# wangheda/youtube-8m

Measured on AMD Instinct MI355X. Metric: training videos/sec, higher is better.
Workload: dtype f32; 1 GPU; BASELINE configs[3]: LstmModel (2 x BasicLSTMCell(1024), dynamic_rnn over F=300) on raw uint8 [B,300,1152] frames + MoeModel head (2 mixtures, V=4716), fp32 training step (fwd+bwd+clip+Adam); per_gpu_batch=128, global_batch=128, frames=300, parallelism=dp1, params=113902808

## Files before the change

### include/yt8m_hip.h

```cpp
#ifndef YT8M_HIP_H
#define YT8M_HIP_H
#include <stdint.h>

#ifdef __cplusplus
extern "C" {
#endif

typedef void* yt8m_stream_t;

enum yt8m_status { YT8M_OK = 0, YT8M_E_BADARG = -1, YT8M_E_SHAPE = -2, YT8M_E_HIP = -3, YT8M_E_RCCL = -4 };
enum yt8m_label_dtype { YT8M_LABEL_U8 = 0, YT8M_LABEL_F32 = 1 };

int yt8m_abi_version(void);
const char* yt8m_last_error(void);
const char* yt8m_built_arch(void);

int yt8m_prof_enable(int on);
int yt8m_prof_reset(void);
int yt8m_prof_get(int family, int64_t* launches, double* total_ms);
int yt8m_prof_get_flops(int family, double* flops);
int yt8m_prof_get_bytes(int family, double* bytes);

int yt8m_probe_mfma_f32(int iters, int blocks, float* sink, yt8m_stream_t stream);
int yt8m_probe_mfma_bf16(int iters, int blocks, int random_operands, float* sink, yt8m_stream_t stream);
// ... 293 lines not shown
int64_t yt8m_wimg_count(void);
int yt8m_wimg_watch(const void* lo, const void* hi, int on);
int yt8m_wimg_note_demand(const float* src, int64_t R, int64_t C, int64_t ld, int trans, int planes, float scale);
int64_t yt8m_wimg_demands(yt8m_wimg_demand* out, int64_t max);
int64_t yt8m_wimg_demand_generation(const void* lo, const void* hi);
typedef struct yt8m_wimg_spec {
  void* plain;
  void* trans;
  int64_t row0, rows;
  float scale;
  int32_t planes;
} yt8m_wimg_spec;
typedef struct yt8m_wimg_job {
  int64_t offset;
  int64_t R, C;
  int32_t tensor;
  int32_t nspec;
  int64_t tile_base;
  yt8m_wimg_spec spec[4];
} yt8m_wimg_job;
int64_t yt8m_wimg_jobs_layout(yt8m_wimg_job* jobs_host, int64_t njobs);
int yt8m_adam_tiles(float* w, float* m, float* v, const float* g, const yt8m_wimg_job* jobs, int64_t njobs, int64_t tile0,
                    int64_t ntiles, const float* l2, float gscale, const float* norms, float clip, float lr_t, float beta1,
                    float beta2, float eps, int do_adam, yt8m_stream_t stream);
int yt8m_adam_multi_ex(float* w, float* m, float* v, const float* g, const int32_t* chunks, int64_t nchunks,
                       const float* l2, float gscale, const float* norms, float clip, float lr_t, float beta1, float beta2,
                       float eps, const uint8_t* skip_tensor, yt8m_stream_t stream);

int yt8m_lstm_gates_fwd(float* z, const float* c_prev, const float* h_prev, float* c_new, float* h_new,
                        float* out, const int32_t* num_frames, int32_t t, int64_t B, int64_t H,
                        float forget_bias, yt8m_stream_t stream);
int yt8m_lstm_gates_bwd(const float* gates, const float* c_prev, const float* c_new, const float* dh,
                        const float* dc, const float* dout, float* dz, float* dc_prev, float* dh_prev,
                        const int32_t* num_frames, int32_t t, int64_t B, int64_t H, yt8m_stream_t stream);

int yt8m_lstm_layer_fwd(float* z, const float* Wh, int64_t ldw, float* cs, float* hs, float* out,
                        const int32_t* num_frames, int64_t F, int64_t B, int64_t H, float forget_bias,
                        void* gemm_workspace, int64_t gemm_workspace_bytes, yt8m_stream_t stream);
int yt8m_lstm_layer_bwd(const float* gates, const float* Wh, int64_t ldw, const float* cs, const float* dout,
                        const float* dc_final, const float* dh_final, float* dz, float* work,
                        const int32_t* num_frames, int64_t F, int64_t B, int64_t H,
                        void* gemm_workspace, int64_t gemm_workspace_bytes, yt8m_stream_t stream);

int yt8m_lstm_persist_supported(int64_t B, int64_t H);
int64_t yt8m_lstm_persist_workspace_bytes(int64_t B, int64_t H);
int64_t yt8m_lstm_persist_workspace_bytes_steps(int64_t B, int64_t H, int64_t T);
int yt8m_lstm_persist_fwd_on_bf16_pipe(int64_t B, int64_t H);
int yt8m_lstm_persist_set_cus(int fwd_cus, int bwd_cus);
int yt8m_lstm_persist_get_cus(int* fwd_cus, int* bwd_cus);
int yt8m_lstm_persist_set_tape_prefetch(int mode);
int yt8m_lstm_persist_tape_prefetch_launches(int64_t* with_prefetch, int64_t* without_prefetch);
int yt8m_lstm_persist_reserve_cus(int cus, int* previous);
int yt8m_lstm_persist_status(const void* workspace, yt8m_stream_t stream);
int yt8m_lstm_persist_debug_fault(void* workspace, yt8m_stream_t stream);
int yt8m_lstm_persist_placement_stats(int64_t* launches, int64_t* workgroups, int64_t* off_xcd, int reset);
int yt8m_lstm_persist_fwd(float* z, const float* Wh, int64_t ldw, float* cs, float* hs, float* out,
                          const int32_t* num_frames, int64_t t0, int64_t T, int64_t B, int64_t H, float forget_bias,
                          void* workspace, int64_t workspace_bytes, yt8m_stream_t stream);
int yt8m_lstm_persist_fwd_bf16(float* z, const float* Wh, int64_t ldw, float* cs, float* hs, float* out,
                               const int32_t* num_frames, int64_t t0, int64_t T, int64_t B, int64_t H, float forget_bias,
                               void* workspace, int64_t workspace_bytes, yt8m_stream_t stream);
int yt8m_lstm_persist_fwd_h2(float* z, const float* Wh, int64_t ldw, float* cs, float* hs, float* out, const int32_t* num_frames,
                             int64_t t0, int64_t T, int64_t B, int64_t H, float forget_bias, const void* wh_absmax, void* workspace,
                             int64_t workspace_bytes, yt8m_stream_t stream);
int yt8m_lstm_persist_bwd_supported(int64_t B, int64_t H);
int yt8m_lstm_persist_bwd(const float* gates, const float* Wh, int64_t ldw, const float* cs, const float* dout, float* dz,
                          float* work, int phase, float* dbias_rows, const int32_t* num_frames, int64_t t0, int64_t T,
                          int64_t B, int64_t H, void* workspace, int64_t workspace_bytes, yt8m_stream_t stream);
int yt8m_lstm_persist_bwd_bf16(const float* gates, const float* Wh, int64_t ldw, const float* cs, const float* dout, float* dz,
                               float* work, int phase, float* dbias_rows, const int32_t* num_frames, int64_t t0, int64_t T,
                               int64_t B, int64_t H, void* workspace, int64_t workspace_bytes, yt8m_stream_t stream);
int yt8m_lstm_persist_bwd_h2(const float* gates, const float* Wh, int64_t ldw, const float* cs, const float* dout, float* dz,
                             float* work, int phase, float* dbias_rows, const int32_t* num_frames, int64_t t0, int64_t T,
                             int64_t B, int64_t H, const void* wh_absmax, void* workspace, int64_t workspace_bytes, yt8m_stream_t stream);
int yt8m_lstm_persist_bwd_on_f16_pipe(int64_t B, int64_t H);
int yt8m_gru_persist_supported(int64_t B, int64_t H);
int64_t yt8m_gru_persist_workspace_bytes(int64_t B, int64_t H, int64_t T);
int yt8m_gru_persist_fwd(float* zg, float* zc, const float* Wg_h, int64_t ldg, const float* Wc_h, int64_t ldc, float* hs, float* rh,
                         float* out, const int32_t* num_frames, int64_t t0, int64_t T, int64_t B, int64_t H, void* workspace,
                         int64_t workspace_bytes, yt8m_stream_t stream);
int yt8m_lstm_persist_bwd_ex(const float* gates, const float* Wh, int64_t ldw, const float* cs, const float* dout, float* dz, float* work,
                             int phase, const int32_t* num_frames, int64_t t0, int64_t T, int64_t B, int64_t H, const void* wh_absmax,
                             void* rowmax, void* partmax, void* workspace, int64_t workspace_bytes, yt8m_stream_t stream);
typedef struct yt8m_persist_bwd_images {
  void* plain;
  void* trans;
  void* trans_scaled;
  const float* rowscale;
  float* colpart;
  float* colpart_scaled;
} yt8m_persist_bwd_images;
int yt8m_lstm_persist_bwd_images_rows(int64_t B, int64_t H);
int yt8m_lstm_persist_bwd_images(const float* gates, const float* Wh, int64_t ldw, const float* cs, const float* dout, float* dz,
                                 float* work, int phase, const int32_t* num_frames, int64_t t0, int64_t T, int64_t B, int64_t H,
                                 void* workspace, int64_t workspace_bytes, const yt8m_persist_bwd_images* images, yt8m_stream_t stream);

typedef struct yt8m_lstm_stack_desc {
  int64_t B, F, D, H;
  int32_t L;
  int32_t input_u8;
  float forget_bias;
  int32_t fwd_chunks;
  int32_t bwd_chunks;
  int32_t need_dx;
  float input_keep_prob;
  int32_t reserved0;
  uint64_t dropout_seed[8];
} yt8m_lstm_stack_desc;
int yt8m_lstm_stack_supported(const yt8m_lstm_stack_desc* desc);
int64_t yt8m_lstm_stack_tape_bytes(const yt8m_lstm_stack_desc* desc);
int64_t yt8m_lstm_stack_scratch_bytes(const yt8m_lstm_stack_desc* desc);
int yt8m_lstm_stack_partition(const yt8m_lstm_stack_desc* desc, int* fwd_chunks, int* bwd_chunks);
int yt8m_lstm_stack_streams(int L, yt8m_stream_t* layer_streams, yt8m_stream_t* wgrad_stream);
int yt8m_lstm_stack_fwd(const yt8m_lstm_stack_desc* desc, const void* x, const int32_t* num_frames, const float* const* W,
                        const float* const* b, void* tape, int64_t tape_bytes, void* scratch, int64_t scratch_bytes,
                        yt8m_stream_t stream);
int yt8m_lstm_stack_view(const yt8m_lstm_stack_desc* desc, void* tape, int layer, int which, float** out);
int yt8m_lstm_stack_bwd(const yt8m_lstm_stack_desc* desc, const void* x, const int32_t* num_frames, const float* const* W, void* tape,
                        int64_t tape_bytes, void* scratch, int64_t scratch_bytes, const float* dout_top,
                        const float* const* dc_final, const float* const* dh_final, float* const* dW, float* const* db,
                        const float* beta_W, const float* beta_b, float* dx, yt8m_stream_t stream);
int yt8m_lstm_stack_status(const yt8m_lstm_stack_desc* desc, void* scratch, yt8m_stream_t stream);
int yt8m_lstm_stack_layer_done_wait(int layer, yt8m_stream_t stream);
int yt8m_lstm_stack_use_streams(int set, int* previous);
typedef void (*yt8m_stream_hook)(void* user, yt8m_stream_t stream);
int yt8m_lstm_stack_set_prep_hook(yt8m_stream_hook hook, void* user);
typedef struct yt8m_opt_ranges {
  float* w;
  float* m;
  float* v;
  const float* g;
  const int32_t* chunks;
  const int32_t* tensor_chunk_start;
  const int32_t* tensor_chunk_start_host;
  const float* l2;
  float* partial;
  float* norms;
  const uint8_t* skip_tensor;
  const yt8m_wimg_job* jobs;
  const int32_t* job_tensor_host;
  const int64_t* job_tile_base_host;
  int32_t njobs;
  int32_t nranges;
  int32_t range_lo[8], range_hi[8];
  float gscale, clip, lr_t, beta1, beta2, eps;
  yt8m_stream_t after_stream;
} yt8m_opt_ranges;
int yt8m_optimizer_ranges(const yt8m_opt_ranges* opt, yt8m_stream_t stream);
int yt8m_lstm_stack_set_early_optimizer(const yt8m_opt_ranges* opt);

int64_t yt8m_lstm_packed_floats(int64_t B, int64_t H);
int yt8m_lstm_pack(const float* Wh, int64_t ldw, int64_t H, float* Wp, float* Wq, yt8m_stream_t stream);
int yt8m_lstm_steps_fwd(float* z, const float* Wh, int64_t ldw, const float* Wp, float* cs, float* hs, float* out,
                        const int32_t* num_frames, int64_t t0, int64_t T, int64_t B, int64_t H, float forget_bias,
                        void* gemm_workspace, int64_t gemm_workspace_bytes, yt8m_stream_t stream);
int yt8m_lstm_steps_bwd(const float* gates, const float* Wh, int64_t ldw, const float* Wq, const float* cs,
                        const float* dout, float* dz, float* work, int phase, const int32_t* num_frames, int64_t t0,
                        int64_t T, int64_t B, int64_t H, void* gemm_workspace, int64_t gemm_workspace_bytes,
                        yt8m_stream_t stream);

int yt8m_graph_cache_stats(int64_t* hits, int64_t* captures, int64_t* fallbacks, int64_t* entries);
int yt8m_graph_cache_clear(void);

int yt8m_reverse_sequence_u8(const uint8_t* x, const int32_t* num_frames, uint8_t* y, int64_t B, int64_t F, int64_t D,
                             yt8m_stream_t stream);
int yt8m_reverse_sequence_f32_tm(const float* x, int64_t ldx, const int32_t* num_frames, float* y, int64_t ldy, int64_t y_col0,
// ... 166 lines not shown
```

### youtube-8m_amd/_lib.py

```python
import ctypes
import os

_HERE = os.path.dirname(os.path.abspath(__file__))
LIB_PATH = os.environ.get("YT8M_LIB", os.path.join(_HERE, "libyt8m_hip.so"))

c_void_p, c_int, c_int64, c_float, c_double = ctypes.c_void_p, ctypes.c_int, ctypes.c_int64, ctypes.c_float, ctypes.c_double
P = c_void_p

class GemmProblem(ctypes.Structure):
    _fields_ = [("M", c_int64), ("N", c_int64), ("K", c_int64), ("A", c_void_p), ("lda", c_int64), ("B", c_void_p),
                ("ldb", c_int64), ("C", c_void_p), ("ldc", c_int64), ("bias", c_void_p), ("beta", c_float)]


STREAM_HOOK = ctypes.CFUNCTYPE(None, ctypes.c_void_p, ctypes.c_void_p)


class PersistBwdImages(ctypes.Structure):
    _fields_ = [("plain", ctypes.c_void_p), ("trans", ctypes.c_void_p), ("trans_scaled", ctypes.c_void_p), ("rowscale", ctypes.c_void_p),
                ("colpart", ctypes.c_void_p), ("colpart_scaled", ctypes.c_void_p)]


class LstmStackDesc(ctypes.Structure):
    _fields_ = [("B", c_int64), ("F", c_int64), ("D", c_int64), ("H", c_int64), ("L", ctypes.c_int32), ("input_u8", ctypes.c_int32),
                ("forget_bias", c_float), ("fwd_chunks", ctypes.c_int32), ("bwd_chunks", ctypes.c_int32), ("need_dx", ctypes.c_int32),
# ... 114 lines not shown
    "yt8m_skinny_fwd_u8": (c_int, [P, c_int64, P, c_int64, P, P, P, P, c_int64, c_int64, c_int64, c_int64, c_float, P]),
    "yt8m_skinny_dw_u8": (c_int, [P, c_int64, P, c_int64, P, P, c_int64, c_int64, c_int64, c_int64, c_float, P, c_int64, P]),
    "yt8m_attn_pool_fwd_u8": (c_int, [P, P, P, P, c_int64, c_int64, c_int64, c_int64, P]),
    "yt8m_attn_pool_dw_u8": (c_int, [P, P, P, P, P, c_int64, c_int64, c_int64, c_int64, P]),
    "yt8m_attn_pool_supported": (c_int, [c_int64, c_int64, c_int64, c_int64]),
    "yt8m_attn_pool_fwd": (c_int, [P, P, P, c_int64, c_int64, c_int64, c_int64, P]),
    "yt8m_attn_pool_bwd": (c_int, [P, P, P, P, P, c_int64, c_int64, c_int64, c_int64, P]),
    "yt8m_gru_layer_fwd": (c_int, [P, P, P, c_int64, P, c_int64, P, P, P, P, c_int64, c_int64, c_int64, P, c_int64, P]),
    "yt8m_gru_layer_bwd": (c_int, [P, P, P, c_int64, P, c_int64, P, P, P, P, P, P, P, c_int64, c_int64, c_int64, P, c_int64, P]),
    "yt8m_lnlstm_layer_fwd": (c_int, [P, P, c_int64, P, P, P, P, P, P, P, c_int64, c_int64, c_int64, c_float, c_float,
                                      ctypes.c_uint64, P, c_int64, P]),
    "yt8m_lnlstm_layer_bwd": (c_int, [P, P, c_int64, P, P, P, P, P, P, P, P, P, P, P, P, c_int64, c_int64, c_int64, c_float,
                                      c_float, ctypes.c_uint64, P, c_int64, P]),
    "yt8m_gate_lstm_supported": (c_int, [c_int64, c_int64]),
    "yt8m_gate_lstm_layer_fwd": (c_int, [P, P, c_int64, P, c_int64, P, P, P, P, P, c_int64, c_int64, c_int64, P, c_int64, P]),
    "yt8m_gate_lstm_layer_bwd": (c_int, [P, P, c_int64, P, c_int64, P, P, P, P, P, P, P, P, P, c_int64, c_int64, c_int64, P, c_int64,
                                         P]),
    "yt8m_glu_lstm_supported": (c_int, [c_int64, c_int64, c_int64]),
    "yt8m_glu_lstm_layer_fwd": (c_int, [P, P, c_int64, P, c_int64, P, c_int64] + [P] * 12 + [c_int64] * 4 + [P, c_int64, P]),
    "yt8m_glu_lstm_layer_bwd": (c_int, [P, P, c_int64, P, c_int64, P, c_int64] + [P] * 14 + [c_int64] + [P] * 4 + [c_int64] * 4 +
                                        [P, c_int64, P]),
    "yt8m_dropout_f32": (c_int, [P, P, c_int64, c_float, ctypes.c_uint64, c_int64, P]),
    "yt8m_add_noise_f32": (c_int, [P, P, c_int64, c_float, ctypes.c_uint64, c_int64, P]),
    "yt8m_moe_mix_bwd_bf16_partial_rows": (c_int64, [c_int64]),
    "yt8m_moe_mix_bwd_bf16": (c_int, [P, P, P, P, c_int, c_int64, c_int64, c_int, c_float, c_float, P, P, c_int64, P, c_int64,
                                      P, c_int64, P, c_int64, P, P]),
    "yt8m_moe_mix_bwd_bf16_images": (c_int, [P, P, P, P, c_int, c_int64, c_int64, c_int, c_float, c_float, P, P, c_int64, P, c_int64,
                                      P, c_int64, P, c_int64, P, P]),
    "yt8m_moe_mix_bwd_bf16_images_z16": (c_int, [P, P, P, P, c_int, c_int64, c_int64, c_int, c_float, c_float, P, P, c_int64, P, c_int64,
                                      P, c_int64, P, c_int64, P, P]),
    "yt8m_moe_mix_fwd_bf16z": (c_int, [P, P, P, c_int64, c_int64, c_int, P]),
    "yt8m_act_fwd_f32": (c_int, [c_int, P, P, c_int64, P]),
    "yt8m_act_bwd_f32": (c_int, [c_int, P, P, P, c_int64, P]),
    "yt8m_chain_link_fwd": (c_int, [c_int, P, P, P, c_int64, c_int64, c_float, c_float, ctypes.c_uint64, c_int64, P]),
    "yt8m_chain_link_bwd": (c_int, [c_int, P, P, P, P, P, c_int64, c_int64, c_float, P]),
    "yt8m_memory_link_fwd": (c_int, [c_int, P, P, c_int, P, P, c_int64, c_float, P]),
    "yt8m_memory_link_bwd": (c_int, [c_int, P, c_int, P, P, P, P, c_int64, c_float, P]),
    "yt8m_frame_pyramid_u8": (c_int, [P, P, c_int64, c_int64, c_int64, c_int, c_int, P, P, P, c_float, P]),
    "yt8m_frame_pyramid_supported": (c_int, [c_int64, c_int, P, c_int]),
    "yt8m_colsum_workspace_bytes": (c_int64, [c_int64, c_int64]),
    "yt8m_colsum_f32": (c_int, [P, c_int64, c_int64, c_int64, P, c_float, P, c_int64, P]),
    "yt8m_rank1_add_rows_f32": (c_int, [P, c_int64, c_int64, c_int64, P, c_float, P]),
    "yt8m_colsum_weighted_f32": (c_int, [P, c_int64, c_int64, c_int64, P, P, c_float, P, P, c_int64, P]),
    "yt8m_xent_workspace_bytes": (c_int64, [c_int64, c_int64]),
    "yt8m_xent_fwd_bwd": (c_int, [P, P, c_int, P, P, P, c_int64, c_int64, c_float, c_float, P, P]),
    "yt8m_xent_bwd": (c_int, [P, P, c_int, P, P, P, c_int64, c_int64, c_float, c_float, P]),
    "yt8m_batch_agreement_workspace_bytes": (c_int64, [c_int64, c_int64]),
    "yt8m_batch_agreement_fwd": (c_int, [P, P, c_int, P, P, c_int64, c_int64, c_float, c_float, c_float, P, P]),
    "yt8m_batch_agreement_bwd": (c_int, [P, P, c_int, P, P, P, c_int64, c_int64, c_float, c_float, P]),
    "yt8m_topk_batch_agreement_fwd": (c_int, [P, P, c_int, P, P, c_int64, c_int64, c_float, c_float, P, P]),
    "yt8m_topk_batch_agreement_bwd": (c_int, [P, P, c_int, P, P, P, c_int64, c_int64, c_float, c_float, c_float, P]),
    "yt8m_pointwise_loss_workspace_bytes": (c_int64, [c_int64, c_int64]),
    "yt8m_pointwise_loss_fwd_bwd": (c_int, [c_int, P, P, c_int, P, P, c_int64, c_int64, c_float, c_float, c_float, c_float, P, P]),
    "yt8m_pointwise_loss_bwd": (c_int, [c_int, P, P, c_int, P, P, c_int64, c_int64, c_float, c_float, c_float, c_float, P]),
    "yt8m_sqnorm_multi": (c_int, [P, P, P, c_int64, P, c_float, P, P, c_int64, c_int64, P, c_int64, P]),
    "yt8m_adam_multi": (c_int, [P, P, P, P, P, c_int64, P, c_float, P, c_float, c_float, c_float, c_float, c_float, P]),
    "yt8m_lstm_gates_fwd": (c_int, [P, P, P, P, P, P, P, ctypes.c_int32, c_int64, c_int64, c_float, P]),
    "yt8m_lstm_gates_bwd": (c_int, [P, P, P, P, P, P, P, P, P, P, ctypes.c_int32, c_int64, c_int64, P]),
    "yt8m_lstm_layer_fwd": (c_int, [P, P, c_int64, P, P, P, P, c_int64, c_int64, c_int64, c_float, P, c_int64, P]),
    "yt8m_graph_cache_stats": (c_int, [ctypes.POINTER(c_int64), ctypes.POINTER(c_int64), ctypes.POINTER(c_int64),
                                       ctypes.POINTER(c_int64)]),
    "yt8m_graph_cache_clear": (c_int, []),
    "yt8m_lstm_persist_supported": (c_int, [c_int64, c_int64]),
    "yt8m_lstm_persist_workspace_bytes": (c_int64, [c_int64, c_int64]),
    "yt8m_lstm_persist_workspace_bytes_steps": (c_int64, [c_int64, c_int64, c_int64]),
    "yt8m_lstm_persist_placement_stats": (c_int, [ctypes.POINTER(c_int64), ctypes.POINTER(c_int64), ctypes.POINTER(c_int64), c_int]),
    "yt8m_lstm_persist_fwd_on_bf16_pipe": (c_int, [c_int64, c_int64]),
    "yt8m_lstm_persist_set_cus": (c_int, [c_int, c_int]),
    "yt8m_lstm_persist_get_cus": (c_int, [ctypes.POINTER(c_int), ctypes.POINTER(c_int)]),
    "yt8m_lstm_persist_set_tape_prefetch": (c_int, [c_int]),
    "yt8m_lstm_persist_tape_prefetch_launches": (c_int, [ctypes.POINTER(c_int64), ctypes.POINTER(c_int64)]),
    "yt8m_lstm_persist_status": (c_int, [P, P]),
    "yt8m_lstm_persist_reserve_cus": (c_int, [c_int, ctypes.POINTER(c_int)]),
    "yt8m_lstm_persist_debug_fault": (c_int, [P, P]),
    "yt8m_lstm_persist_fwd": (c_int, [P, P, c_int64, P, P, P, P, c_int64, c_int64, c_int64, c_int64, c_float, P, c_int64, P]),
    "yt8m_lstm_persist_fwd_bf16": (c_int, [P, P, c_int64, P, P, P, P, c_int64, c_int64, c_int64, c_int64, c_float, P, c_int64, P]),
    "yt8m_lstm_persist_bwd_supported": (c_int, [c_int64, c_int64]),
    "yt8m_lstm_persist_bwd": (c_int, [P, P, c_int64, P, P, P, P, c_int, P, P, c_int64, c_int64, c_int64, c_int64, P, c_int64, P]),
    "yt8m_lstm_persist_bwd_bf16": (c_int, [P, P, c_int64, P, P, P, P, c_int, P, P, c_int64, c_int64, c_int64, c_int64, P, c_int64, P]),
    "yt8m_lstm_persist_fwd_h2": (c_int, [P, P, c_int64, P, P, P, P, c_int64, c_int64, c_int64, c_int64, c_float, P, P, c_int64, P]),
    "yt8m_lstm_persist_bwd_h2": (c_int, [P, P, c_int64, P, P, P, P, c_int, P, P, c_int64, c_int64, c_int64, c_int64, P, P, c_int64, P]),
    "yt8m_lstm_persist_bwd_on_f16_pipe": (c_int, [c_int64, c_int64]),
    "yt8m_lstm_persist_bwd_ex": (c_int, [P, P, c_int64, P, P, P, P, c_int, P, c_int64, c_int64, c_int64, c_int64, P, P, P, P, c_int64, P]),
    "yt8m_h2_split_rowmax": (c_int, [P, c_int64, c_int64, c_int64, P, P, P, P]),
    "yt8m_lstm_persist_bwd_images_rows": (c_int, [c_int64, c_int64]),
    "yt8m_lstm_persist_bwd_images": (c_int, [P, P, c_int64, P, P, P, P, c_int, P, c_int64, c_int64, c_int64, c_int64, P, c_int64, P, P]),
    "yt8m_lstm_packed_floats": (c_int64, [c_int64, c_int64]),
    "yt8m_lstm_pack": (c_int, [P, c_int64, c_int64, P, P, P]),
    "yt8m_lstm_steps_fwd": (c_int, [P, P, c_int64, P, P, P, P, P, c_int64, c_int64, c_int64, c_int64, c_float, P, c_int64, P]),
    "yt8m_lstm_steps_bwd": (c_int, [P, P, c_int64, P, P, P, P, P, c_int, P, c_int64, c_int64, c_int64, c_int64, P, c_int64, P]),
    "yt8m_lstm_layer_bwd": (c_int, [P, P, c_int64, P, P, P, P, P, P, P, c_int64, c_int64, c_int64, P, c_int64, P]),
    "yt8m_attn_softmax_fwd": (c_int, [P, P, P, c_int64, c_int64, c_int64, P]),
    "yt8m_attn_softmax_bwd": (c_int, [P, P, P, P, c_int64, c_int64, c_int64, P]),
    "yt8m_softmax_rows_fwd": (c_int, [P, P, P, c_int64, c_int64, c_int64, P]),
    "yt8m_softmax_rows_bwd": (c_int, [P, P, P, P, c_int64, c_int64, c_int64, P]),
    "yt8m_netvlad_supported": (c_int, [c_int64, c_int64, c_int64, c_int64]),
    "yt8m_netvlad_single_pass": (c_int, [c_int64, c_int64, c_int64, c_int64]),
    "yt8m_netvlad_set_single": (c_int, [c_int]),
    "yt8m_netvlad_workspace_bytes": (c_int64, [c_int64, c_int64, c_int64, c_int64]),
    "yt8m_netvlad_fwd_u8": (c_int, [P, P, P, P, c_int64, c_int64, c_int64, c_int64, c_int, c_float, P, P, P, P, c_int64, P]),
    "yt8m_netvlad_bwd_u8": (c_int, [P, P, P, P, P, c_int64, c_int64, c_int64, c_int64, c_int, c_float, P, c_float, P, c_float,
                                    P, c_int64, P]),
    "yt8m_vlad_finish_fwd": (c_int, [P, P, P, P, P, c_int64, c_int64, c_int64, c_int64, c_float, P]),
    "yt8m_vlad_finish_bwd": (c_int, [P, P, P, P, P, P, P, c_float, c_int64, c_int64, c_int64, c_float, P]),
    "yt8m_vlad_finish_q_supported": (c_int, [c_int64]),
    "yt8m_vlad_finish_q_fwd": (c_int, [P, P, P, P, P, P, c_int64, c_int64, c_int64, c_int64, c_float, P]),
    "yt8m_vlad_finish_q_bwd": (c_int, [P, P, P, P, P, P, P, P, c_float, c_int64, c_int64, c_int64, c_float, P]),
    "yt8m_crc32c": (ctypes.c_uint32, [P, c_int64]),
    "yt8m_crc32c_masked": (ctypes.c_uint32, [P, c_int64]),
    "yt8m_prefetch_open": (c_int, [ctypes.POINTER(ctypes.c_char_p), c_int, c_int, ctypes.POINTER(ctypes.c_char_p),
                                   ctypes.POINTER(ctypes.c_int32), c_int, c_int64, c_int64, c_int64, c_int, c_int, c_int,
                                   ctypes.POINTER(c_void_p)]),
    "yt8m_prefetch_acquire": (c_int, [P, ctypes.POINTER(c_void_p), ctypes.POINTER(c_void_p), ctypes.POINTER(c_void_p),
                                      ctypes.POINTER(c_void_p), ctypes.POINTER(c_int64), ctypes.POINTER(c_int64),
                                      ctypes.POINTER(c_int)]),
    "yt8m_prefetch_close": (c_int, [P]),
    "yt8m_tfrecord_write_predictions": (c_int, [ctypes.c_char_p, c_int64, P, c_int64, P, P, c_int64, ctypes.c_char_p]),
    "yt8m_tfrecord_open": (c_int, [ctypes.c_char_p, c_int, ctypes.POINTER(c_void_p)]),
    "yt8m_tfrecord_close": (c_int, [P]),
    "yt8m_tfrecord_read_frame_batch": (c_int, [P, ctypes.POINTER(ctypes.c_char_p), ctypes.POINTER(ctypes.c_int32), c_int, c_int64,
                                               c_int64, c_int64, P, P, P, P, c_int64, ctypes.POINTER(c_int64)]),
    "yt8m_tfrecord_read_video_batch": (c_int, [P, ctypes.POINTER(ctypes.c_char_p), ctypes.POINTER(ctypes.c_int32), c_int, c_int64,
                                               c_int64, P, P, P, c_int64, ctypes.POINTER(c_int64)]),
    "yt8m_comm_unique_id": (c_int, [P]),
    "yt8m_comm_init": (c_int, [c_int, c_int, P, ctypes.POINTER(c_void_p)]),
    "yt8m_comm_size": (c_int, [P, ctypes.POINTER(c_int), ctypes.POINTER(c_int)]),
    "yt8m_comm_allreduce_f32": (c_int, [P, P, c_int64, c_int, P]),
    "yt8m_comm_allreduce_mean": (c_int, [P, P, c_int64, P]),
    "yt8m_comm_allreduce_rsag_f32": (c_int, [P, P, c_int64, c_int, c_int, P]),
    "yt8m_comm_broadcast_f32": (c_int, [P, P, c_int64, c_int, P]),
    "yt8m_comm_destroy": (c_int, [P]),
    "yt8m_u8_proj_supported": (c_int, [c_int64]),
    "yt8m_u8_frames_to_bf16_tm": (c_int, [P, P, c_int64, c_int64, c_int64, c_float, c_int, P, c_int64, P, P, P]),
    "yt8m_split3_bf16_t": (c_int, [P, c_int64, c_int64, c_int64, c_float, P, c_int64, P]),
    "yt8m_rowscale_bias_f32": (c_int, [P, c_int64, c_int64, c_int64, P, P, c_float, P, P]),
    "yt8m_sample_frames_f32": (c_int, [P, P, c_int64, c_int64, c_int64, c_int64, c_int, ctypes.c_uint64, P, P, P]),
    "yt8m_sample_frames_u8": (c_int, [P, P, c_int64, c_int64, c_int64, c_int64, c_int, ctypes.c_uint64, P, P, P]),
    "yt8m_frame_pool_fwd": (c_int, [P, c_int64, c_int64, c_int64, c_int, P, P]),
    "yt8m_frame_pool_bwd": (c_int, [P, P, P, c_int64, c_int64, c_int64, c_int, P, P]),
    "yt8m_batchnorm_fwd": (c_int, [P, c_int64, c_int64, P, P, P, P, c_int, c_float, c_float, P, P, P, P]),
    "yt8m_batchnorm_workspace_bytes": (c_int64, [c_int64]),
    "yt8m_batchnorm_bwd": (c_int, [P, P, c_int64, c_int64, P, P, P, c_int, P, P, c_float, P, c_float, P, c_int64, P]),
    "yt8m_wimg_register": (c_int, [P, c_int64, c_int64, c_int64, c_int, c_int, c_float, P]),
    "yt8m_wimg_unregister": (c_int64, [P, P]),
    "yt8m_wimg_lookup": (c_void_p, [P, c_int64, c_int64, c_int64, c_int, c_int, c_float]),
    "yt8m_wimg_count": (c_int64, []),
    "yt8m_wimg_watch": (c_int, [P, P, c_int]),
    "yt8m_wimg_note_demand": (c_int, [P, c_int64, c_int64, c_int64, c_int, c_int, c_float]),
    "yt8m_wimg_demands": (c_int64, [ctypes.POINTER(WimgDemand), c_int64]),
    "yt8m_wimg_demand_generation": (c_int64, [P, P]),
    "yt8m_wimg_jobs_layout": (c_int64, [ctypes.POINTER(WimgJob), c_int64]),
    "yt8m_adam_tiles": (c_int, [P, P, P, P, P, c_int64, c_int64, c_int64, P, c_float, P, c_float, c_float, c_float, c_float, c_float,
                                c_int, P]),
    "yt8m_adam_multi_ex": (c_int, [P, P, P, P, P, c_int64, P, c_float, P, c_float, c_float, c_float, c_float, c_float, P, P]),
    "yt8m_optimizer_ranges": (c_int, [ctypes.POINTER(OptRanges), P]),
    "yt8m_lstm_stack_set_early_optimizer": (c_int, [ctypes.POINTER(OptRanges)]),
    "yt8m_h2_split": (c_int, [P, c_int64, c_int64, c_int64, c_float, P, P, P, P, P]),
    "yt8m_h2_absmax": (c_int, [P, c_int64, c_int64, c_int64, P, P]),
    "yt8m_h2_degraded": (c_int, [ctypes.POINTER(ctypes.c_uint64), c_int, P]),
    "yt8m_clip_by_norm_f32": (c_int, [P, P, c_int64, c_float, P, P]),
    "yt8m_gru_persist_supported": (c_int, [c_int64, c_int64]),
    "yt8m_gru_persist_workspace_bytes": (c_int64, [c_int64, c_int64, c_int64]),
    "yt8m_gru_persist_fwd": (c_int, [P, P, P, c_int64, P, c_int64, P, P, P, P, c_int64, c_int64, c_int64, c_int64, P, c_int64, P]),
    "yt8m_h2_split_dropout": (c_int, [P, c_int64, c_int64, c_float, P, P, P, c_float, ctypes.c_uint64, c_int64, P]),
    "yt8m_h2_split_ex": (c_int, [P, c_int64, c_int64, c_int64, c_float, P, P, P, P, P, P, P, P]),
    "yt8m_gemm_h1x2_nt_ex": (c_int, [c_int64, c_int64, c_int64, P, c_int64, P, c_int64, P, c_int64, P, c_float, P, P, P, c_float, c_float, P,
# ... 88 lines not shown
```

### youtube-8m_amd/csrc/lstm_persist.hip

```cpp
#include <algorithm>
#include <atomic>
#include <mutex>
#include "common.h"
#include "x3_image.h"

namespace {

typedef float f32x4 __attribute__((ext_vector_type(4)));
typedef unsigned int u32x4 __attribute__((ext_vector_type(4)));

constexpr int FWD_POLLQ = 2;
constexpr int EPI_PRIO = 3;
constexpr int AUX_STORE = 17, AUX_LOAD = 17;
constexpr long long SPIN_TIMEOUT = 300000000;
constexpr int CTL_HDR = 32;
constexpr int CTL_STICKY = 32;
constexpr int NSH = 8;

struct PersistFwdArgs {
  float* z;
  const float* Wh;
  long long ldw;
  float* cs;
  float* hs;
  float* out;
  const int32_t* nf;
  float* hx;
  unsigned* ctl;
  unsigned* stats;
  int t0, T, B, H;
  float fb;
  int NU, RB, NT16, per, pf;
  int nimg;
  const unsigned* wword;
  unsigned long long* dbg;
};

#ifdef YT8M_PERSIST_TIMING
#define STAMP(slot)                                                                                            \
  do {                                                                                                         \
    if (blockIdx.x == 0 && (w == 0 || w == 8) && lane == 0 && k < 256)                                          \
      a.dbg[((w >> 3) * 256 + k) * 8 + (slot)] = __builtin_readcyclecounter();                                 \
  } while (0)
#else
#define STAMP(slot) do {} while (0)
#endif

__device__ __forceinline__ __amdgpu_buffer_rsrc_t make_rsrc(const void* p, unsigned bytes) {
  return __builtin_amdgcn_make_buffer_rsrc(const_cast<void*>(p), 0, (int)bytes, 0x00020000);
}

__device__ __forceinline__ float4 as_f4(u32x4 v) {
  return make_float4(__uint_as_float(v.x), __uint_as_float(v.y), __uint_as_float(v.z), __uint_as_float(v.w));
}

__device__ __forceinline__ unsigned placement_offset() {
  unsigned xcc;
  asm volatile("s_getreg_b32 %0, hwreg(HW_REG_XCC_ID)" : "=s"(xcc));
  return ((xcc & 7u) - (blockIdx.x & 7u)) & 7u;
}
__device__ __forceinline__ void note_placement(unsigned* ctl) {
  if (threadIdx.x == 0 && blockIdx.x == 0) __hip_atomic_store(ctl + 2, placement_offset() + 1u, __ATOMIC_RELAXED, __HIP_MEMORY_SCOPE_AGENT);
}
__device__ __forceinline__ void check_placement(unsigned* ctl, unsigned* stats) {
  if (!stats) return;
  const unsigned k0 = __hip_atomic_load(ctl + 2, __ATOMIC_RELAXED, __HIP_MEMORY_SCOPE_AGENT);
  if (k0 != 0u && k0 - 1u != placement_offset()) __hip_atomic_fetch_add(stats, 1u, __ATOMIC_RELAXED, __HIP_MEMORY_SCOPE_AGENT);
}

__device__ __forceinline__ void propagate_error(unsigned* ctl) {
  if (__hip_atomic_load(ctl, __ATOMIC_RELAXED, __HIP_MEMORY_SCOPE_AGENT) != 0u)
    __hip_atomic_store(ctl - CTL_STICKY, 1u, __ATOMIC_RELAXED, __HIP_MEMORY_SCOPE_AGENT);
}

__device__ __forceinline__ unsigned shard_sum(unsigned v) {
  unsigned tot = 0;
#pragma unroll
  for (int i = 0; i < NSH; ++i) tot += (unsigned)__builtin_amdgcn_readlane((int)v, i);
  return tot;
}

__device__ __forceinline__ void wait_tile(unsigned* ctl, int tile, unsigned target, int lane) {
  unsigned* c = ctl + CTL_HDR + (tile * NSH + (lane & (NSH - 1))) * 32;
  long long t_start = 0;
  for (unsigned spins = 0;; ++spins) {
    unsigned v = 0;
    if (lane < NSH) v = __hip_atomic_load(c, __ATOMIC_RELAXED, __HIP_MEMORY_SCOPE_AGENT);
    const unsigned tot = shard_sum(v);
    if (tot >= target) return;
    if (spins >= 16) {
      __builtin_amdgcn_s_sleep(1);
      if ((spins & 255) == 16) {
        if (__hip_atomic_load(ctl, __ATOMIC_RELAXED, __HIP_MEMORY_SCOPE_AGENT) != 0u) return;
        const long long now = wall_clock64();
        if (t_start == 0) t_start = now;
        else if (now - t_start > SPIN_TIMEOUT) {
          if (lane == 0) {
            __hip_atomic_store(ctl - CTL_STICKY, 1u, __ATOMIC_RELAXED, __HIP_MEMORY_SCOPE_AGENT);
            __hip_atomic_store(ctl, 1u, __ATOMIC_RELAXED, __HIP_MEMORY_SCOPE_AGENT);
          }
          return;
        }
      }
    }
  }
}

__global__ __launch_bounds__(256) void hx_pack_kernel(const float* __restrict__ h, float* __restrict__ hx, int B, int H, int NT16) {
  const long long n = (long long)NT16 * 16 * H;
  for (long long e = (long long)blockIdx.x * 256 + threadIdx.x; e < n; e += (long long)gridDim.x * 256) {
    const int j = (int)(e & 15), i = (int)((e >> 4) & 15);
    const long long blk = e >> 8;
    const int qg = (int)(blk % (H >> 4)), T = (int)(blk / (H >> 4));
    const int row = T * 16 + i;
    hx[e] = row < B ? h[(long long)row * H + qg * 16 + j] : 0.f;
  }
}

// ... 223 lines not shown
            v.x = __float_as_uint(hn[j]); v.y = __float_as_uint(h1); v.z = __float_as_uint(h2); v.w = __float_as_uint(h3);
            const int erow = 8 * j + (lane >> 3);
            const unsigned off = ((unsigned)(T * QH + (ug >> 1)) * 256u + (unsigned)(erow * 16 + (ug & 1) * 8 + eunit)) * 4u;
            __builtin_amdgcn_raw_buffer_store_b128(v, image(s + 1), (int)off, 0, AUX_STORE);
          }
        }
        STAMP(3);
        asm volatile("s_waitcnt vmcnt(0)" ::: "memory");
        if (lane == 0)
          __hip_atomic_fetch_add(a.ctl + CTL_HDR + (T * NSH + (blockIdx.x & (NSH - 1))) * 32, 1u, __ATOMIC_RELAXED, __HIP_MEMORY_SCOPE_AGENT);
        STAMP(4);
      }
#pragma unroll
      for (int j = 0; j < 2; ++j) {
        if (evalid[j]) {
          const int brow = T * 16 + 8 * j + (lane >> 3);
          const long long idx1 = ((long long)(t + 1) * B + brow) * H + ug * 8 + eunit;
          if (live[j]) {
            float* zr = a.z + ((long long)t * B + brow) * 4 * H + ug * 8 + eunit;
            zr[0] = gi[j]; zr[H] = gj[j]; zr[2 * H] = gf[j]; zr[3 * H] = go[j];
          }
          a.cs[idx1] = cn[j];
          a.hs[idx1] = hn[j];
          if (a.out) a.out[((long long)t * B + brow) * H + ug * 8 + eunit] = live[j] ? hn[j] : 0.f;
        }
      }
    }
  }
  if (ew == 0 && lane == 0) { check_placement(a.ctl, a.stats); propagate_error(a.ctl); }
}

typedef __bf16 bf16x8 __attribute__((ext_vector_type(8)));
typedef _Float16 f16x8 __attribute__((ext_vector_type(8)));
__device__ __forceinline__ u32x4 as_u4(float4 v) {
  u32x4 r;
  r.x = __float_as_uint(v.x); r.y = __float_as_uint(v.y); r.z = __float_as_uint(v.z); r.w = __float_as_uint(v.w);
  return r;
}
template <int N>
__device__ __forceinline__ float row_ror(float v) {
  return __int_as_float(__builtin_amdgcn_update_dpp(0, __float_as_int(v), 0x120 + N, 0xF, 0xF, true));
}

__device__ __forceinline__ unsigned bf16_rn_bits(float x) {
  const unsigned u = __float_as_uint(x);
  return (u + 0x7FFFu + ((u >> 16) & 1u)) >> 16;
}
__device__ __forceinline__ void split3_bits(float x, unsigned& h1, unsigned& h2, unsigned& h3) {
  h1 = bf16_rn_bits(x);
  const float r1 = x - __uint_as_float(h1 << 16);
  h2 = bf16_rn_bits(r1);
  h3 = bf16_rn_bits(r1 - __uint_as_float(h2 << 16));
}
template <int N>
__device__ __forceinline__ unsigned row_shl_u(unsigned v) {
  return (unsigned)__builtin_amdgcn_update_dpp(0, (int)v, 0x100 + N, 0xF, 0xF, true);
}

constexpr float FWD_H2_S = 8192.f;
template <int NP, bool F16 = false>
__global__ __launch_bounds__(256) void hx_pack_x3_kernel(const float* __restrict__ h, u32x4* __restrict__ img, int B, int H, int NT16) {
  const int KBH = H >> 5;
  const long long n = (long long)NT16 * KBH * NP * 64;
  for (long long e = (long long)blockIdx.x * 256 + threadIdx.x; e < n; e += (long long)gridDim.x * 256) {
    const int l = (int)(e & 63), p = (int)((e >> 6) % NP);
    const long long blk = e / (64 * NP);
    const int kbg = (int)(blk % KBH), T = (int)(blk / KBH);
    const int row = T * 16 + (l & 15), k0 = kbg * 32 + (l >> 4) * 8;
    unsigned hb[8];
#pragma unroll
    for (int j = 0; j < 8; ++j) {
      unsigned h1, h2, h3 = 0;
      const float hv = row < B ? h[(long long)row * H + k0 + j] : 0.f;
      if constexpr (F16) yt8m_x3::split_h2(hv * FWD_H2_S, h1, h2);
      else split3_bits(hv, h1, h2, h3);
      hb[j] = p == 0 ? h1 : (p == 1 ? h2 : h3);
    }
    u32x4 v;
    v.x = hb[0] | (hb[1] << 16); v.y = hb[2] | (hb[3] << 16); v.z = hb[4] | (hb[5] << 16); v.w = hb[6] | (hb[7] << 16);
    img[e] = v;
  }
}

template <int NKB, int NP = 3, bool F16 = false>
__global__ __launch_bounds__(768) void lstm_persist_fwd_x3_kernel(PersistFwdArgs a) {
  static_assert(!F16 || NP == 2, "the f16 form has two planes");
  constexpr int NS = 2;
  constexpr int EPW = 2;
  constexpr int NF = NKB * 2 * NP;
  constexpr int NREG = F16 ? NF : (NF < 10 ? NF : 10), NLDS = NF - NREG;
  constexpr int HK = NKB / 2;
  static_assert(NKB % 2 == 0, "half items");
  __shared__ __attribute__((aligned(16))) float red[NS][8][2][4][64];
  __shared__ __attribute__((aligned(16))) u32x4 Wl[8][NLDS > 0 ? NLDS : 1][64];
  __shared__ unsigned lds_cnt[NS], lds_free[NS];
  __shared__ unsigned lds_seen[MAX_LOCAL_TILES];
  __shared__ int lds_nf[MAX_LOCAL_TILES * 16];
  constexpr int CARRY_T = F16 ? 4 : 1;
  __shared__ float lds_ch[F16 ? 4 : 1][CARRY_T][2][2][64];
  const int tid = threadIdx.x, lane = tid & 63;
  const int w = __builtin_amdgcn_readfirstlane(tid >> 6);
  int ug, g;
  {
    const int b = blockIdx.x;
    if (a.per > 0 && (a.NU % (4 * a.per)) == 0) {
      const int x = b & 7, sl = b >> 3;
      g = x / a.per;
      ug = ((sl >> 2) * a.per + (x % a.per)) * 4 + (sl & 3);
    } else if (a.per > 0) { const int x = b & 7; g = x / a.per; ug = (b >> 3) * a.per + (x % a.per); }
    else { g = b / a.NU; ug = b % a.NU; }
  }
  const int H = a.H, B = a.B, NT16 = a.NT16, RB = a.RB;
  const int n_it = (NT16 - g + RB - 1) / RB;
  const int total = n_it * a.T;
  const int KBH = H >> 5;
  const long long img_f = (long long)NT16 * KBH * NP * 256;
  const unsigned img_bytes = (unsigned)(img_f * 4);
  auto image = [&](int s) -> __amdgpu_buffer_rsrc_t { return make_rsrc(a.hx + s * img_f, img_bytes); };
  const unsigned arrivals = (unsigned)a.NU * EPW;
  float f16_sw = 1.f;
  if constexpr (F16) f16_sw = yt8m_x3::pow2_scale_for(__uint_as_float(a.wword[0]), 14);
  const float f16_inv = F16 ? 1.0f / (f16_sw * FWD_H2_S) : 1.0f;
  auto w_frag = [&](int kb, int ct, int p) -> u32x4 {
    const int n16 = lane & 15, kg = lane >> 4;
    const long long k = (long long)(w * NKB + kb) * 32 + kg * 8;
    const long long col = (long long)(n16 & 3) * H + ug * 8 + ct * 4 + (n16 >> 2);
    const float* q = a.Wh + k * a.ldw + col;
    unsigned hb[8];
#pragma unroll
    for (int j = 0; j < 8; ++j) {
      unsigned h1, h2, h3 = 0;
      if constexpr (F16) yt8m_x3::split_h2(q[j * a.ldw] * f16_sw, h1, h2);
      else split3_bits(q[j * a.ldw], h1, h2, h3);
      hb[j] = p == 0 ? h1 : (p == 1 ? h2 : h3);
    }
    u32x4 v;
    v.x = hb[0] | (hb[1] << 16); v.y = hb[2] | (hb[3] << 16); v.z = hb[4] | (hb[5] << 16); v.w = hb[6] | (hb[7] << 16);
    return v;
  };
  note_placement(a.ctl);
  if (tid < NS) { lds_cnt[tid] = 0; lds_free[tid] = 0; }
  for (int i = tid; i < MAX_LOCAL_TILES; i += 768) lds_seen[i] = 0;
  for (int i = tid; i < n_it * 16; i += 768) {
    const int brow = (g + (i >> 4) * RB) * 16 + (i & 15);
    lds_nf[i] = (a.nf && brow < B) ? a.nf[brow] : 0x7fffffff;
  }
  if (w < 8) {
#pragma unroll
    for (int f = NREG; f < NF; ++f) Wl[w][f - NREG][lane] = w_frag(f / (2 * NP), (f / NP) & 1, f % NP);
  }
  __syncthreads();

  if (w < 8) {
    u32x4 Wr[NREG];
#pragma unroll
    for (int f = 0; f < NREG; ++f) Wr[f] = w_frag(f / (2 * NP), (f / NP) & 1, f % NP);
    const unsigned lane_off = (unsigned)lane * 16u + (unsigned)(w * NKB) * (NP * 1024u);
    auto load_half = [&](u32x4 (&Hh)[HK][NP], int s, int T, int half) {
      const __amdgpu_buffer_rsrc_t hxr = image(s);
      const unsigned base = (unsigned)(T * KBH) * (NP * 1024u) + lane_off + (unsigned)(half * HK) * (NP * 1024u);
#pragma unroll
      for (int kbl = 0; kbl < HK; ++kbl)
#pragma unroll
        for (int p = 0; p < NP; ++p)
          Hh[kbl][p] = __builtin_amdgcn_raw_buffer_load_b128(hxr, (int)(base + (unsigned)(kbl * NP + p) * 1024u), 0, 0);
    };
    u32x4 H0[HK][NP], H1[HK][NP], H2[HK][NP];
    load_half(H0, 0, g, 0);
    load_half(H1, 0, g, 1);
    int s_cur = 0, it_cur = 0;
    auto item = [&](u32x4 (&Ha)[HK][NP], u32x4 (&Hb)[HK][NP], u32x4 (&Hc)[HK][NP], int k) {
      const int s = s_cur, T = g + it_cur * RB;
      STAMP(0);
      int sr = s, itr = it_cur + 1;
      if (itr >= n_it) { itr -= n_it; ++sr; }
      const bool have = k + 1 < total;
      const int Tr = have ? g + itr * RB : T;
      itr = have ? itr : it_cur;
      sr = have ? sr : s;
      unsigned pv = 0;
      if (w == 0 && lane < NSH)
        pv = __hip_atomic_load(a.ctl + CTL_HDR + (Tr * NSH + lane) * 32, __ATOMIC_RELAXED, __HIP_MEMORY_SCOPE_AGENT);
      f32x4 acc[2][2] = {{{0.f, 0.f, 0.f, 0.f}, {0.f, 0.f, 0.f, 0.f}}, {{0.f, 0.f, 0.f, 0.f}, {0.f, 0.f, 0.f, 0.f}}};
      u32x4 ls[2][NP];
#pragma unroll
      for (int p = 0; p < NP; ++p)
        if (p >= NREG) ls[0][p] = Wl[w][p >= NREG ? p - NREG : 0][lane];
#pragma unroll
      for (int kb = 0; kb < NKB; ++kb) {
        if (kb == HK) {
          if (w == 0) {
            const unsigned tot = shard_sum(pv);
            if (tot < (unsigned)sr * arrivals) wait_tile(a.ctl, Tr, (unsigned)sr * arrivals, lane);
            if (lane == 0) __hip_atomic_store(&lds_seen[itr], (unsigned)sr * arrivals, __ATOMIC_RELAXED, __HIP_MEMORY_SCOPE_WORKGROUP);
          } else {
            lds_wait_ge(&lds_seen[itr], (unsigned)sr * arrivals, a.ctl);
          }
          STAMP(1);
        }
        u32x4 av[NP];
#pragma unroll
        for (int p = 0; p < NP; ++p) av[p] = kb < HK ? Ha[kb < HK ? kb : 0][p] : Hb[kb >= HK ? kb - HK : 0][p];
#pragma unroll
        for (int ct = 0; ct < 2; ++ct) {
          const int gi = kb * 2 + ct;
          if (kb >= HK) {
            const __amdgpu_buffer_rsrc_t hxr = image(sr);
            const unsigned base = (unsigned)(Tr * KBH) * (NP * 1024u) + lane_off;
#pragma unroll
            for (int j = NP * (gi - NKB); j < NP * (gi - NKB) + NP; ++j) {
              const int kbl = (j % (NP * HK)) / NP, pl = j % NP;
              const u32x4 v = __builtin_amdgcn_raw_buffer_load_b128(hxr, (int)(base + (unsigned)j * 1024u), 0, 0);
              if (j < NP * HK) Hc[kbl][pl] = v; else Ha[kbl][pl] = v;
            }
          }
          if (gi + 1 < 2 * NKB) {
#pragma unroll
            for (int p = 0; p < NP; ++p) {
              const int f = (gi + 1) * NP + p;
              if (f >= NREG) ls[(gi + 1) & 1][p] = Wl[w][f >= NREG ? f - NREG : 0][lane];
            }
          }
          __builtin_amdgcn_sched_barrier(0);
          u32x4 bv[NP];
#pragma unroll
          for (int p = 0; p < NP; ++p) {
            const int f = gi * NP + p;
            bv[p] = f < NREG ? Wr[f < NREG ? f : 0] : ls[gi & 1][p];
          }
          auto mm = [&](const u32x4& x, const u32x4& y, f32x4 c) -> f32x4 {
            if constexpr (F16) return __builtin_amdgcn_mfma_f32_16x16x32_f16(__builtin_bit_cast(f16x8, x), __builtin_bit_cast(f16x8, y), c, 0, 0, 0);
            else return __builtin_amdgcn_mfma_f32_16x16x32_bf16(__builtin_bit_cast(bf16x8, x), __builtin_bit_cast(bf16x8, y), c, 0, 0, 0);
          };
          if constexpr (NP == 3) {
            acc[ct][0] = mm(av[0], bv[0], acc[ct][0]);
            acc[ct][1] = mm(av[0], bv[1], acc[ct][1]);
            acc[ct][0] = mm(av[1], bv[0], acc[ct][0]);
            acc[ct][1] = mm(av[0], bv[2], acc[ct][1]);
            acc[ct][0] = mm(av[1], bv[1], acc[ct][0]);
// ... 93 lines not shown
        hn[j] = live[j] ? h1 : hpre[j];
        if (!evalid[j]) hn[j] = 0.f;
        if (carry) { lds_ch[F16 ? ew : 0][li][0][j][lane] = cn[j]; lds_ch[F16 ? ew : 0][li][1][j][lane] = hn[j]; }
      }
      if (s + 1 < a.T) {
        const __amdgpu_buffer_rsrc_t hxr = image(s + 1);
#pragma unroll
        for (int jj = 0; jj < JP; ++jj) {
          const int j = ew & 1;
          unsigned hb[3];
          if constexpr (F16) yt8m_x3::split_h2(hn[jj] * FWD_H2_S, hb[0], hb[1]);
          else if constexpr (NP == 3) split3_bits(hn[jj], hb[0], hb[1], hb[2]);
          else hb[0] = bf16_rn_bits(hn[jj]);
          const int erow = 8 * j + (lane >> 3);
#pragma unroll
          for (int p = 0; p < NP; ++p) {
            const unsigned d = hb[p] | (row_shl_u<1>(hb[p]) << 16);
            const unsigned d2 = row_shl_u<2>(d), d4 = row_shl_u<4>(d), d6 = row_shl_u<6>(d);
            if (eunit == 0) {
              u32x4 v;
              v.x = d; v.y = d2; v.z = d4; v.w = d6;
              const unsigned off = ((unsigned)((T * KBH + (ug >> 2)) * NP + p) * 256u + (unsigned)(((ug & 3) * 16 + erow) * 4)) * 4u;
              __builtin_amdgcn_raw_buffer_store_b128(v, hxr, (int)off, 0, AUX_STORE);
            }
          }
        }
        STAMP(3);
        asm volatile("s_waitcnt vmcnt(0)" ::: "memory");
        if (lane == 0)
          __hip_atomic_fetch_add(a.ctl + CTL_HDR + (T * NSH + ((blockIdx.x * EPW + (ew & (EPW - 1))) & (NSH - 1))) * 32, 1u,
                                 __ATOMIC_RELAXED, __HIP_MEMORY_SCOPE_AGENT);
        STAMP(4);
      }
#pragma unroll
      for (int jj = 0; jj < JP; ++jj) {
        const int j = ew & 1;
        if (evalid[jj]) {
          const int brow = T * 16 + 8 * j + (lane >> 3);
          const long long idx1 = ((long long)(t + 1) * B + brow) * H + ug * 8 + eunit;
          if (live[jj]) {
            float* zr = a.z + ((long long)t * B + brow) * 4 * H + ug * 8 + eunit;
            zr[0] = gi[jj]; zr[H] = gj[jj]; zr[2 * H] = gf[jj]; zr[3 * H] = go[jj];
          }
          a.cs[idx1] = cn[jj];
          a.hs[idx1] = hn[jj];
          if (a.out) a.out[((long long)t * B + brow) * H + ug * 8 + eunit] = live[jj] ? hn[jj] : 0.f;
        }
      }
    }
  }
  if (ew == 0 && lane == 0) { check_placement(a.ctl, a.stats); propagate_error(a.ctl); }
}

struct PersistBwdArgs {
  const float* gates;
  const float* Wh;
  long long ldw;
  const float* cs;
  const float* dout;
  float* dz;
  float* work;
  float* dbrows;
  const int32_t* nf;
  float* dzx;
  unsigned* ctl;
  unsigned* stats;
  int t0, T, B, H, phase;
  int NUB, RB, NT16, per, pf;
  int nimg;
  int bf;
  int h2;
  const unsigned* wword;
  unsigned* sc;
  unsigned sc_bytes;
  unsigned* rowmax;
  unsigned* partmax;
  unsigned long long* dbg;
  float* img_plain;
  float* img_trans;
  float* img_trans_s;
  const float* rowscale;
  float* colpart;
  float* colpart_s;
};

constexpr int NSLOT_B = 3;

constexpr int PF_DIST = 1;
constexpr int PF_ROWS = 4;
typedef const __attribute__((address_space(4))) unsigned* tape_kptr;
__device__ __forceinline__ unsigned tape_touch(const float* base, unsigned off) {
  const unsigned long long u = reinterpret_cast<unsigned long long>(base);
  const unsigned lo = __builtin_amdgcn_readfirstlane((unsigned)u), hi = __builtin_amdgcn_readfirstlane((unsigned)(u >> 32));
  return *reinterpret_cast<tape_kptr>((((unsigned long long)hi << 32) | lo) + off);
}
__device__ __forceinline__ void tape_discard(unsigned v) { asm volatile("" ::"s"(v)); }

__device__ __forceinline__ unsigned p_bf16_rn_bits(float x) {
  const unsigned u = __float_as_uint(x);
  return (u + 0x7FFFu + ((u >> 16) & 1u)) >> 16;
}
__device__ __forceinline__ void p_split3(float x, unsigned& h1, unsigned& h2, unsigned& h3) {
  h1 = p_bf16_rn_bits(x);
  const float r1 = x - __uint_as_float(h1 << 16);
  h2 = p_bf16_rn_bits(r1);
  const float r2 = r1 - __uint_as_float(h2 << 16);
  h3 = p_bf16_rn_bits(r2);
  if ((__float_as_uint(x) & 0x7F800000u) == 0x7F800000u) {
    h1 = __float_as_uint(x) >> 16;
    h2 = h3 = 0;
  }
}


template <int NQB, bool PF, bool SH, bool ROT, bool IMG = false, bool BF = false, bool H2 = false, bool TPF = false>
__global__ __launch_bounds__(768) void lstm_persist_bwd_kernel(PersistBwdArgs a) {
  static_assert(!TPF || H2, "the tape prefetch belongs to the two-half-plane form");
  static_assert(!IMG || ROT, "the operand images are written by the rotated epilogue");
  static_assert(!BF || (PF && SH && ROT && !IMG && (NQB % 4) == 0), "the bf16-operand form: prefetching, one image per step, rotated epilogue");
  static_assert(!H2 || (PF && SH && ROT && !IMG && !BF && (NQB % 8) == 0), "the two-half-plane form: prefetching, one image per step, rotated epilogue");
  constexpr int HALF = NQB / 2;
  constexpr unsigned EPW = ROT ? 1u : 4u;
  __shared__ __attribute__((aligned(16))) float4 Wl[8][BF ? 1 : HALF][64];
  __shared__ __attribute__((aligned(16))) float red[NSLOT_B][8][4][64];
  __shared__ unsigned lds_cnt[NSLOT_B], lds_free[NSLOT_B];
  __shared__ unsigned lds_seen[MAX_LOCAL_TILES];
  __shared__ int lds_nf[ROT ? MAX_LOCAL_TILES * 16 : 1];
  const int tid = threadIdx.x, lane = tid & 63;
  const int w = __builtin_amdgcn_readfirstlane(tid >> 6);
  int ub, g;
  {
    const int b = blockIdx.x;
    if (a.per > 0 && (a.NUB % (2 * a.per)) == 0) {
      const int x = b & 7, sl = b >> 3;
      g = x / a.per;
      ub = ((sl >> 1) * a.per + (x % a.per)) * 2 + (sl & 1);
    } else if (a.per > 0) { const int x = b & 7; g = x / a.per; ub = (b >> 3) * a.per + (x % a.per); }
    else { g = b / a.NUB; ub = b % a.NUB; }
  }
  const int H = a.H, B = a.B, NT16 = a.NT16, RB = a.RB;
  const int n_it = (NT16 - g + RB - 1) / RB;
  const int total = n_it * a.T;
  const int QH4 = H >> 2;
  const unsigned img_bytes = (unsigned)NT16 * (unsigned)H * (BF ? 32u : 64u) * 4u;
  const long long img_f = (long long)NT16 * H * (BF ? 32 : 64);
  auto image = [&](int s) -> __amdgpu_buffer_rsrc_t { return make_rsrc(a.dzx + (SH ? s : (s & 1)) * img_f, img_bytes); };
  constexpr int AUX_LD = SH ? 0 : AUX_LOAD;
  const unsigned arrivals = (unsigned)a.NUB * EPW;
  const int i16 = lane & 15, kq = lane >> 4;
  note_placement(a.ctl);
  if (tid < NSLOT_B) { lds_cnt[tid] = 0; lds_free[tid] = 0; }
  for (int i = tid; i < MAX_LOCAL_TILES; i += 768) lds_seen[i] = 0;
  if constexpr (ROT) {
    for (int i = tid; i < n_it * 16; i += 768) {
      const int brow = (g + (i >> 4) * RB) * 16 + (i & 15);
      lds_nf[i] = (a.nf && brow < B) ? a.nf[brow] : 0x7fffffff;
    }
  }
  float h2_sw = 1.f;
  if constexpr (H2) h2_sw = yt8m_x3::pow2_scale_for(__uint_as_float(a.wword[0]), 14);
  auto w_frag_h2 = [&](int kbl, u32x4& fhi, u32x4& flo) {
    const int kbp = w * (NQB / 2) + kbl;
    const int urow = ub * 16 + i16;
    const float* q = a.Wh + (long long)urow * a.ldw + 16 * (kbp >> 1) + 8 * (kbp & 1) + 2 * kq;
    unsigned hb[8], lb[8];
#pragma unroll
    for (int j = 0; j < 8; ++j) yt8m_x3::split_h2(q[(long long)(j & 3) * H + (j >> 2)] * h2_sw, hb[j], lb[j]);
    fhi.x = hb[0] | (hb[1] << 16); fhi.y = hb[2] | (hb[3] << 16); fhi.z = hb[4] | (hb[5] << 16); fhi.w = hb[6] | (hb[7] << 16);
    flo.x = lb[0] | (lb[1] << 16); flo.y = lb[2] | (lb[3] << 16); flo.z = lb[4] | (lb[5] << 16); flo.w = lb[6] | (lb[7] << 16);
  };
  if constexpr (H2) {
    if (w < 8) {
#pragma unroll
      for (int kbl = 0; kbl < HALF; ++kbl) {
        u32x4 fhi, flo;
        w_frag_h2(kbl, fhi, flo);
        Wl[w][kbl][lane] = as_f4(flo);
      }
    }
  }
  if (!BF && !H2 && w < 8) {
    const float* wrow = a.Wh + (long long)(ub * 16 + i16) * a.ldw + (long long)(w * NQB) * 16 + kq * 4;
#pragma unroll
    for (int qq = 0; qq < HALF; ++qq) Wl[w][qq][lane] = *reinterpret_cast<const float4*>(wrow + (HALF + qq) * 16);
  }
  __syncthreads();

  if constexpr (BF) {
    if (w < 8) {
      constexpr int KBW = NQB / 2, HB = KBW / 2;
      const float* wrow = a.Wh + (long long)(ub * 16 + i16) * a.ldw + (long long)(w * KBW) * 32 + kq * 8;
      u32x4 Wb[KBW];
#pragma unroll
      for (int kb = 0; kb < KBW; ++kb) {
        const float4 lo = *reinterpret_cast<const float4*>(wrow + kb * 32), hi = *reinterpret_cast<const float4*>(wrow + kb * 32 + 4);
        Wb[kb].x = p_bf16_rn_bits(lo.x) | (p_bf16_rn_bits(lo.y) << 16);
        Wb[kb].y = p_bf16_rn_bits(lo.z) | (p_bf16_rn_bits(lo.w) << 16);
        Wb[kb].z = p_bf16_rn_bits(hi.x) | (p_bf16_rn_bits(hi.y) << 16);
        Wb[kb].w = p_bf16_rn_bits(hi.z) | (p_bf16_rn_bits(hi.w) << 16);
      }
      const int QB = H >> 3;
      const unsigned lane_off = (unsigned)lane * 16u + (unsigned)(w * KBW) * 1024u;
      auto blk = [&](int T) -> unsigned { return (unsigned)(T * QB) * 1024u + lane_off; };
      u32x4 ring[HB];
      int s_cur = 0, it_cur = 0, slot = 0, gen = 0;
      {
        if (w == 0) {
          wait_tile(a.ctl, g, arrivals, lane);
          if (lane == 0) __hip_atomic_store(&lds_seen[0], arrivals, __ATOMIC_RELAXED, __HIP_MEMORY_SCOPE_WORKGROUP);
        } else {
          lds_wait_ge(&lds_seen[0], arrivals, a.ctl);
        }
        const unsigned b0 = blk(g);
        const __amdgpu_buffer_rsrc_t dx0 = image(0);
#pragma unroll
        for (int kb = 0; kb < HB; ++kb) ring[kb] = __builtin_amdgcn_raw_buffer_load_b128(dx0, (int)(b0 + (unsigned)kb * 1024u), 0, 0);
      }
      for (int k = 0; k < total; ++k) {
        const int s = s_cur, T = g + it_cur * RB;
        int s1 = s, it1 = it_cur + 1;
        if (it1 == n_it) { it1 = 0; ++s1; }
        const bool have1 = k + 1 < total;
        const int T1 = have1 ? g + it1 * RB : T;
        s1 = have1 ? s1 : s;
        unsigned pv = 0;
        const unsigned bcur = blk(T);
        const __amdgpu_buffer_rsrc_t dxr = image(s);
        if (w == 0 && lane < NSH)
          pv = __hip_atomic_load(a.ctl + CTL_HDR + (T1 * NSH + lane) * 32, __ATOMIC_RELAXED, __HIP_MEMORY_SCOPE_AGENT);
        f32x4 acc0 = {0.f, 0.f, 0.f, 0.f}, acc1 = {0.f, 0.f, 0.f, 0.f};
#pragma unroll
        for (int kb = 0; kb < HB; ++kb) {
          const bf16x8 av = __builtin_bit_cast(bf16x8, ring[kb]), bv = __builtin_bit_cast(bf16x8, Wb[kb]);
          ring[kb] = __builtin_amdgcn_raw_buffer_load_b128(dxr, (int)(bcur + (unsigned)(HB + kb) * 1024u), 0, 0);
          __builtin_amdgcn_sched_barrier(0);
          if (kb & 1) acc1 = __builtin_amdgcn_mfma_f32_16x16x32_bf16(av, bv, acc1, 0, 0, 0);
          else acc0 = __builtin_amdgcn_mfma_f32_16x16x32_bf16(av, bv, acc0, 0, 0, 0);
          __builtin_amdgcn_sched_barrier(0);
        }
        const int it1l = have1 ? it1 : it_cur;
        if (w == 0) {
          const unsigned tot = shard_sum(pv);
          if (tot < (unsigned)(s1 + 1) * arrivals) wait_tile(a.ctl, T1, (unsigned)(s1 + 1) * arrivals, lane);
          if (lane == 0) __hip_atomic_store(&lds_seen[it1l], (unsigned)(s1 + 1) * arrivals, __ATOMIC_RELAXED, __HIP_MEMORY_SCOPE_WORKGROUP);
        } else {
          lds_wait_ge(&lds_seen[it1l], (unsigned)(s1 + 1) * arrivals, a.ctl);
        }
        const unsigned bnext = blk(T1);
        const __amdgpu_buffer_rsrc_t dxn = image(s1);
#pragma unroll
        for (int kb = 0; kb < HB; ++kb) {
          const bf16x8 av = __builtin_bit_cast(bf16x8, ring[kb]), bv = __builtin_bit_cast(bf16x8, Wb[HB + kb]);
          if (kb & 1) acc1 = __builtin_amdgcn_mfma_f32_16x16x32_bf16(av, bv, acc1, 0, 0, 0);
          else acc0 = __builtin_amdgcn_mfma_f32_16x16x32_bf16(av, bv, acc0, 0, 0, 0);
          if (kb >= 1) {
            __builtin_amdgcn_sched_barrier(0);
            ring[kb - 1] = __builtin_amdgcn_raw_buffer_load_b128(dxn, (int)(bnext + (unsigned)(kb - 1) * 1024u), 0, 0);
            __builtin_amdgcn_sched_barrier(0);
          }
        }
        ring[HB - 1] = __builtin_amdgcn_raw_buffer_load_b128(dxn, (int)(bnext + (unsigned)(HB - 1) * 1024u), 0, 0);
        if (gen > 0) lds_wait_ge(&lds_free[slot], EPW * (unsigned)gen, a.ctl);
        float* rw = &red[slot][w][0][lane];
#pragma unroll
        for (int r = 0; r < 4; ++r) rw[r * 64] = acc0[r] + acc1[r];
        if (lane == 0) __hip_atomic_fetch_add(&lds_cnt[slot], 1u, __ATOMIC_RELAXED, __HIP_MEMORY_SCOPE_WORKGROUP);
        if (++slot == NSLOT_B) { slot = 0; ++gen; }
        if (++it_cur == n_it) { it_cur = 0; ++s_cur; }
      }
      return;
    }
  } else if constexpr (H2) {
    if (w < 8) {
      constexpr int NPW = NQB / 4, PH = NPW / 2;
      u32x4 Wh_[HALF];
#pragma unroll
      for (int kbl = 0; kbl < HALF; ++kbl) { u32x4 flo; w_frag_h2(kbl, Wh_[kbl], flo); }
      const float inv_sw = 1.0f / h2_sw;
      const int lane_off = lane * 16;
      auto blk = [&](int T) -> int { return __builtin_amdgcn_readfirstlane((T * QH4 + w * NQB) * 1024); };
      const __amdgpu_buffer_rsrc_t scr = make_rsrc(a.sc, a.sc_bytes);
      const int kq_off = kq * 4;
      auto sc_off = [&](int s, int T, int pl) -> int { return __builtin_amdgcn_readfirstlane(((s * NT16 + T) * a.NUB + w * NPW + pl) * 16); };
      u32x4 ring[HALF];
      unsigned sc[PH];
      int s_cur = 0, it_cur = 0, slot = 0, gen = 0;
      auto seen_wait = [&](int it, int T, unsigned target) {
        if (w == 0) {
          wait_tile(a.ctl, T, target, lane);
          if (lane == 0) __hip_atomic_store(&lds_seen[it], target, __ATOMIC_RELAXED, __HIP_MEMORY_SCOPE_WORKGROUP);
        } else {
          lds_wait_ge(&lds_seen[it], target, a.ctl);
        }
      };
      {
        seen_wait(0, g, arrivals);
        const int b0 = blk(g);
        const __amdgpu_buffer_rsrc_t dx0 = image(0);
#pragma unroll
        for (int q = 0; q < HALF; ++q) ring[q] = __builtin_amdgcn_raw_buffer_load_b128(dx0, lane_off, b0 + (q) * 1024, 0);
#pragma unroll
        for (int pl = 0; pl < PH; ++pl) sc[pl] = __builtin_amdgcn_raw_buffer_load_b32(scr, kq_off, sc_off(0, g, pl), 0);
      }
      u32x4 wlb[2] = {as_u4(Wl[w][0][lane]), as_u4(Wl[w][1][lane])};
      auto rescale = [&](f32x4& acc, const f32x4& tmp, unsigned e4) {
#pragma unroll
        for (int r = 0; r < 4; ++r) acc[r] = __builtin_fmaf(tmp[r], __uint_as_float(((e4 >> (8 * r)) & 0xFFu) << 23), acc[r]);
        asm volatile("" : "+v"(acc[0]), "+v"(acc[1]), "+v"(acc[2]), "+v"(acc[3]));
      };
      for (int k = 0; k < total; ++k) {
        const int s = s_cur, T = g + it_cur * RB;
        STAMP(0);
        int s1 = s, it1 = it_cur + 1;
        if (it1 == n_it) { it1 = 0; ++s1; }
        const bool have1 = k + 1 < total;
        const int T1 = have1 ? g + it1 * RB : T;
        s1 = have1 ? s1 : s;
        unsigned pv = 0;
        const int bcur = blk(T);
        const __amdgpu_buffer_rsrc_t dxr = image(s);
        if (w == 0 && lane < NSH)
          pv = __hip_atomic_load(a.ctl + CTL_HDR + (T1 * NSH + lane) * 32, __ATOMIC_RELAXED, __HIP_MEMORY_SCOPE_AGENT);
        f32x4 acc = {0.f, 0.f, 0.f, 0.f};
        f32x4 tmp = {0.f, 0.f, 0.f, 0.f};
        unsigned e_cur = 0;
#pragma unroll
        for (int kb = 0; kb < HALF / 2; ++kb) {
          const int pl = kb >> 1;
          const f16x8 ah = __builtin_bit_cast(f16x8, ring[2 * kb]), al = __builtin_bit_cast(f16x8, ring[2 * kb + 1]);
          const f16x8 bh = __builtin_bit_cast(f16x8, Wh_[kb]), bl = __builtin_bit_cast(f16x8, wlb[kb & 1]);
          if ((kb & 1) == 0) e_cur = sc[pl];
          __builtin_amdgcn_sched_barrier(0);
          if ((kb & 1) == 0) tmp = __builtin_amdgcn_mfma_f32_16x16x32_f16(ah, bh, f32x4{0.f, 0.f, 0.f, 0.f}, 0, 0, 0);
          else tmp = __builtin_amdgcn_mfma_f32_16x16x32_f16(ah, bh, tmp, 0, 0, 0);
          tmp = __builtin_amdgcn_mfma_f32_16x16x32_f16(al, bh, tmp, 0, 0, 0);
          tmp = __builtin_amdgcn_mfma_f32_16x16x32_f16(ah, bl, tmp, 0, 0, 0);
          __builtin_amdgcn_sched_barrier(0);
          wlb[kb & 1] = as_u4(Wl[w][kb + 2][lane]);
          ring[2 * kb] = __builtin_amdgcn_raw_buffer_load_b128(dxr, lane_off, bcur + (HALF + 2 * kb) * 1024, 0);
          ring[2 * kb + 1] = __builtin_amdgcn_raw_buffer_load_b128(dxr, lane_off, bcur + (HALF + 2 * kb + 1) * 1024, 0);
          if ((kb & 1) == 0) sc[pl] = __builtin_amdgcn_raw_buffer_load_b32(scr, kq_off, sc_off(s, T, PH + pl), 0);
          if (kb & 1) rescale(acc, tmp, e_cur);
          __builtin_amdgcn_sched_barrier(0);
        }
        {
          const int it1l = have1 ? it1 : it_cur;
          if (w == 0) {
            const unsigned tot = shard_sum(pv);
            if (tot < (unsigned)(s1 + 1) * arrivals) wait_tile(a.ctl, T1, (unsigned)(s1 + 1) * arrivals, lane);
            if (lane == 0) __hip_atomic_store(&lds_seen[it1l], (unsigned)(s1 + 1) * arrivals, __ATOMIC_RELAXED, __HIP_MEMORY_SCOPE_WORKGROUP);
          } else {
            lds_wait_ge(&lds_seen[it1l], (unsigned)(s1 + 1) * arrivals, a.ctl);
          }
          STAMP(1);
        }
        const int bnext = blk(T1);
        const __amdgpu_buffer_rsrc_t dxn = image(s1);
#pragma unroll
        for (int kb = HALF / 2; kb < HALF; ++kb) {
          const int kr = kb - HALF / 2, plr = kr >> 1;
// ... 629 lines not shown
  }
  arrive();
  if (ew == 0 && lane == 0) { check_placement(a.ctl, a.stats); propagate_error(a.ctl); }
}

#include "gru_persist.inl"

struct PersistGate {
  std::mutex mu;
  static constexpr int R = 4;
  hipEvent_t ev[16][R];
  int cus[16][R];
  int head[16];
  bool init[16];
  PersistGate() { memset(cus, 0, sizeof(cus)); memset(head, 0, sizeof(head)); memset(init, 0, sizeof(init)); }
  int admit(int dev, int need, int total, hipStream_t s) {
    static const bool chain_all = getenv("YT8M_PERSIST_CHAIN") != nullptr;
    if (!init[dev]) {
      for (int i = 0; i < R; ++i) YT8M_HIP_CHECK(hipEventCreateWithFlags(&ev[dev][i], hipEventDisableTiming));
      init[dev] = true;
    }
    int room = chain_all ? 0 : total - need;
    for (int i = 0; i < R; ++i) {
      const int k = (head[dev] + R - 1 - i) % R;
      if (cus[dev][k] == 0) continue;
      const bool oldest = i == R - 1;
      if (!oldest && cus[dev][k] <= room) { room -= cus[dev][k]; continue; }
      room = 0;
      YT8M_HIP_CHECK(hipStreamWaitEvent(s, ev[dev][k], 0));
    }
    return YT8M_OK;
  }
  int done(int dev, int used, hipStream_t s) {
    const int k = head[dev];
    YT8M_HIP_CHECK(hipEventRecord(ev[dev][k], s));
    cus[dev][k] = used;
    head[dev] = (k + 1) % R;
    return YT8M_OK;
  }
};
PersistGate g_gate;

unsigned* g_stats[16] = {nullptr};
int64_t g_stat_launches[16] = {0}, g_stat_wgs[16] = {0};
unsigned* stats_ptr(int dev) {
  if (!g_stats[dev]) {
    if (hipMalloc(reinterpret_cast<void**>(&g_stats[dev]), 64) != hipSuccess) return nullptr;
    (void)hipMemset(g_stats[dev], 0, 64);
  }
  return g_stats[dev];
}

int g_cap_fwd = -1, g_cap_bwd = -1;
int g_reserved_cus = getenv("YT8M_PERSIST_RESERVED_CUS") ? atoi(getenv("YT8M_PERSIST_RESERVED_CUS")) : 0;
int persist_cu_budget(int cus, bool bwd = false) {
  static const int cap = getenv("YT8M_PERSIST_CUS") ? atoi(getenv("YT8M_PERSIST_CUS")) : 0;
  static const int cap_b = getenv("YT8M_PERSIST_CUS_BWD") ? atoi(getenv("YT8M_PERSIST_CUS_BWD")) : 128;
  int c = bwd ? cap_b : cap;
  if (bwd && g_cap_bwd >= 0) c = g_cap_bwd;
  if (!bwd && g_cap_fwd >= 0) c = g_cap_fwd;
  return (c > 0 && c < cus) ? c : cus;
}

int device_cus(int* dev_out) {
  static int cus[16] = {0};
  int dev = 0;
  if (hipGetDevice(&dev) != hipSuccess || dev < 0 || dev >= 16) return 0;
  if (!cus[dev]) {
    int n = 0;
    if (hipDeviceGetAttribute(&n, hipDeviceAttributeMultiprocessorCount, dev) != hipSuccess) return 0;
    cus[dev] = n;
  }
  if (dev_out) *dev_out = dev;
  return cus[dev];
}

std::atomic<long long> g_tpf_launches[2] = {{0}, {0}};
thread_local int g_tape_prefetch_mode = 0;
bool tape_prefetch_on() {
  static const bool env_off = getenv("YT8M_PERSIST_TAPE_PREFETCH") != nullptr && atoi(getenv("YT8M_PERSIST_TAPE_PREFETCH")) == 0;
  return g_tape_prefetch_mode == 1 || (g_tape_prefetch_mode == 0 && !env_off);
}

struct Geometry { int NQ, NU, RB, NT16, per, pf; };

bool persist_geometry(int64_t B, int64_t H, Geometry* geo) {
  static const bool off = getenv("YT8M_NO_PERSIST") != nullptr;
  if (off || B < 1 || H < 128 || (H % 128) != 0 || H > 1024) return false;
  const int NQ = (int)(H / 128);
  if (!(NQ == 1 || NQ == 2 || NQ == 4 || NQ == 6 || NQ == 8)) return false;
  int dev = 0;
  const int cus = device_cus(&dev);
  const int NU = (int)(H / 8);
  if (cus < NU) return false;
  const int NT16 = (int)((B + 15) / 16);
  int RB = persist_cu_budget(cus) / NU;
  if (RB > NT16) RB = NT16;
  if (RB > NT16 / 4) RB = NT16 / 4;
  if (RB < 1) RB = 1;
  if ((NT16 + RB - 1) / RB > MAX_LOCAL_TILES) return false;
  const int nit_min = NT16 / RB;
  int per = 0;
  if (RB <= 8 && (8 % RB) == 0 && (NU % (8 / RB)) == 0) per = 8 / RB;
  if (geo) *geo = {NQ, NU, RB, NT16, per, nit_min >= 8 ? 2 : (nit_min >= 2 ? 1 : 0)};
  return true;
}

template <int NQ, bool SH>
int launch_fwd_sh(const PersistFwdArgs& a, unsigned grid, hipStream_t s) {
  if (a.pf >= 2) hipLaunchKernelGGL((lstm_persist_fwd_kernel<NQ, 2, SH>), dim3(grid), dim3(768), 0, s, a);
  else if (a.pf == 1) hipLaunchKernelGGL((lstm_persist_fwd_kernel<NQ, 1, SH>), dim3(grid), dim3(768), 0, s, a);
  else hipLaunchKernelGGL((lstm_persist_fwd_kernel<NQ, 0, SH>), dim3(grid), dim3(768), 0, s, a);
  return yt8m::launch_status("lstm_persist_fwd_kernel");
}
template <int NQ>
int launch_fwd(const PersistFwdArgs& a, unsigned grid, hipStream_t s) {
  return a.nimg >= a.T ? launch_fwd_sh<NQ, true>(a, grid, s) : launch_fwd_sh<NQ, false>(a, grid, s);
}

constexpr int64_t DBG_BYTES = 65536;
constexpr int64_t STICKY_BYTES = CTL_STICKY * 4;
int64_t ctl_bytes(int NT16) { return (int64_t)(CTL_HDR + NT16 * NSH * 32) * 4; }
int64_t ctl_padded(int NT16) { return ((STICKY_BYTES + ctl_bytes(NT16) + 255) / 256) * 256; }
int images_in(int64_t workspace_bytes, int NT16, int64_t width) {
  const int64_t n = (workspace_bytes - ctl_padded(NT16) - DBG_BYTES) / ((int64_t)NT16 * 16 * width * 4);
  return (int)std::min<int64_t>(n, 1 << 20);
}

}

using namespace yt8m;

extern "C" int yt8m_lstm_persist_set_cus(int fwd_cus, int bwd_cus) {
  YT8M_REQUIRE(fwd_cus >= -1 && bwd_cus >= -1, YT8M_E_BADARG, "CU counts must be >= -1");
  g_cap_fwd = fwd_cus;
  g_cap_bwd = bwd_cus;
  return YT8M_OK;
}

extern "C" int yt8m_lstm_persist_get_cus(int* fwd_cus, int* bwd_cus) {
  if (fwd_cus) *fwd_cus = g_cap_fwd;
  if (bwd_cus) *bwd_cus = g_cap_bwd;
  return YT8M_OK;
}

extern "C" int yt8m_lstm_persist_reserve_cus(int cus, int* previous) {
  YT8M_REQUIRE(cus >= 0 && cus <= 4096, YT8M_E_BADARG, "CU count out of range");
  std::lock_guard<std::mutex> lk(g_gate.mu);
  if (previous) *previous = g_reserved_cus;
  g_reserved_cus = cus;
  return YT8M_OK;
}

extern "C" int yt8m_lstm_persist_set_tape_prefetch(int mode) {
  YT8M_REQUIRE(mode >= 0 && mode <= 2, YT8M_E_BADARG, "mode must be 0 (default), 1 (on) or 2 (off)");
  g_tape_prefetch_mode = mode;
  return YT8M_OK;
}

extern "C" int yt8m_lstm_persist_tape_prefetch_launches(int64_t* with_prefetch, int64_t* without_prefetch) {
  if (with_prefetch) *with_prefetch = g_tpf_launches[1].load();
  if (without_prefetch) *without_prefetch = g_tpf_launches[0].load();
  return YT8M_OK;
}

extern "C" int yt8m_lstm_persist_supported(int64_t B, int64_t H) { return persist_geometry(B, H, nullptr) ? 1 : 0; }

namespace {
bool fwd_x3_shape(int64_t H, int pf) {
  static const bool x3_off = getenv("YT8M_PERSIST_X3") != nullptr && atoi(getenv("YT8M_PERSIST_X3")) == 0;
  return !x3_off && (H == 512 || H == 1024) && pf >= 1;
}
}

extern "C" int yt8m_lstm_persist_fwd_on_bf16_pipe(int64_t B, int64_t H) {
  Geometry geo;
  return (persist_geometry(B, H, &geo) && fwd_x3_shape(H, geo.pf)) ? 1 : 0;
}

extern "C" int64_t yt8m_lstm_persist_workspace_bytes(int64_t B, int64_t H) {
  Geometry geo;
  if (!persist_geometry(B, H, &geo)) return 0;
  return ctl_padded(geo.NT16) + (int64_t)2 * geo.NT16 * 16 * 4 * H * 4 + DBG_BYTES;
}

extern "C" int64_t yt8m_lstm_persist_workspace_bytes_steps(int64_t B, int64_t H, int64_t T) {
  Geometry geo;
  if (!persist_geometry(B, H, &geo)) return 0;
  return ctl_padded(geo.NT16) + std::max<int64_t>(T, 2) * geo.NT16 * 16 * 4 * H * 4 + ((std::max<int64_t>(T, 2) * geo.NT16 * (H / 16) * 16 + 255) / 256) * 256 +
         (int64_t)2 * geo.NT16 * (H / 16) * 2048 + DBG_BYTES;
}

extern "C" int yt8m_lstm_persist_placement_stats(int64_t* launches, int64_t* workgroups, int64_t* off_xcd, int reset) {
  int dev = 0;
  device_cus(&dev);
  unsigned v = 0;
  if (g_stats[dev]) YT8M_HIP_CHECK(hipMemcpy(&v, g_stats[dev], 4, hipMemcpyDeviceToHost));
  if (launches) *launches = g_stat_launches[dev];
  if (workgroups) *workgroups = g_stat_wgs[dev];
  if (off_xcd) *off_xcd = v;
  if (reset) {
    if (g_stats[dev]) YT8M_HIP_CHECK(hipMemset(g_stats[dev], 0, 64));
    g_stat_launches[dev] = 0;
    g_stat_wgs[dev] = 0;
  }
  return YT8M_OK;
}

extern "C" int yt8m_lstm_persist_status(const void* workspace, yt8m_stream_t stream) {
  YT8M_REQUIRE(workspace, YT8M_E_BADARG, "null workspace");
  unsigned err = 0;
  YT8M_HIP_CHECK(hipMemcpyAsync(&err, workspace, 4, hipMemcpyDeviceToHost, as_stream(stream)));
  YT8M_HIP_CHECK(hipStreamSynchronize(as_stream(stream)));
  if (err != 0) {
    YT8M_HIP_CHECK(hipMemsetAsync(const_cast<void*>(workspace), 0, 4, as_stream(stream)));
    return fail(YT8M_E_HIP, "a persistent LSTM launch on this workspace timed out waiting for a tile since the last status call%s", "");
  }
  return YT8M_OK;
}

namespace {
__global__ void persist_fault_kernel(unsigned* ctl) {
  __hip_atomic_store(ctl, 1u, __ATOMIC_RELAXED, __HIP_MEMORY_SCOPE_AGENT);
  propagate_error(ctl);
}
}

extern "C" int yt8m_lstm_persist_debug_fault(void* workspace, yt8m_stream_t stream) {
  YT8M_REQUIRE(workspace, YT8M_E_BADARG, "null workspace");
  hipLaunchKernelGGL(persist_fault_kernel, dim3(1), dim3(1), 0, as_stream(stream), static_cast<unsigned*>(workspace) + CTL_STICKY);
  return launch_status("persist_fault_kernel");
}

namespace {
int persist_fwd_impl(float* z, const float* Wh, int64_t ldw, float* cs, float* hs, float* out, const int32_t* num_frames, int64_t t0,
                     int64_t T, int64_t B, int64_t H, float forget_bias, void* workspace, int64_t workspace_bytes, yt8m_stream_t stream,
                     bool bf16, const void* h2_wword = nullptr);
}
extern "C" int yt8m_lstm_persist_fwd_h2(float* z, const float* Wh, int64_t ldw, float* cs, float* hs, float* out,
                                        const int32_t* num_frames, int64_t t0, int64_t T, int64_t B, int64_t H, float forget_bias,
                                        const void* wh_absmax, void* workspace, int64_t workspace_bytes, yt8m_stream_t stream) {
  YT8M_REQUIRE(wh_absmax, YT8M_E_BADARG, "null absmax word");
  static const bool off = getenv("YT8M_PERSIST_FWD_H2") != nullptr && atoi(getenv("YT8M_PERSIST_FWD_H2")) == 0;
  return persist_fwd_impl(z, Wh, ldw, cs, hs, out, num_frames, t0, T, B, H, forget_bias, workspace, workspace_bytes, stream, false,
                          off ? nullptr : wh_absmax);
}
extern "C" int yt8m_lstm_persist_fwd(float* z, const float* Wh, int64_t ldw, float* cs, float* hs, float* out,
                                     const int32_t* num_frames, int64_t t0, int64_t T, int64_t B, int64_t H, float forget_bias,
                                     void* workspace, int64_t workspace_bytes, yt8m_stream_t stream) {
  return persist_fwd_impl(z, Wh, ldw, cs, hs, out, num_frames, t0, T, B, H, forget_bias, workspace, workspace_bytes, stream, false);
}
extern "C" int yt8m_lstm_persist_fwd_bf16(float* z, const float* Wh, int64_t ldw, float* cs, float* hs, float* out,
                                          const int32_t* num_frames, int64_t t0, int64_t T, int64_t B, int64_t H, float forget_bias,
                                          void* workspace, int64_t workspace_bytes, yt8m_stream_t stream) {
  return persist_fwd_impl(z, Wh, ldw, cs, hs, out, num_frames, t0, T, B, H, forget_bias, workspace, workspace_bytes, stream, true);
}
namespace {
int persist_fwd_impl(float* z, const float* Wh, int64_t ldw, float* cs, float* hs, float* out, const int32_t* num_frames, int64_t t0,
                     int64_t T, int64_t B, int64_t H, float forget_bias, void* workspace, int64_t workspace_bytes, yt8m_stream_t stream,
                     bool bf16, const void* h2_wword) {
  using namespace yt8m;
  YT8M_REQUIRE(t0 >= 0 && T >= 0 && B >= 0 && H >= 0, YT8M_E_SHAPE, "negative dimension");
  if (T * B * H == 0) return YT8M_OK;
  YT8M_REQUIRE(z && Wh && cs && hs && workspace, YT8M_E_BADARG, "null operand");
  YT8M_REQUIRE(ldw >= 4 * H, YT8M_E_SHAPE, "ldw < 4H");
  Geometry geo;
  YT8M_REQUIRE(persist_geometry(B, H, &geo), YT8M_E_SHAPE, "shape not supported by the persistent recurrence (see yt8m_lstm_persist_supported)");
  YT8M_REQUIRE(workspace_bytes >= yt8m_lstm_persist_workspace_bytes(B, H), YT8M_E_SHAPE, "workspace too small");
  YT8M_REQUIRE(T < (1 << 20), YT8M_E_SHAPE, "T too large");
  hipStream_t s = as_stream(stream);
  const int64_t cb = ctl_padded(geo.NT16);
  PersistFwdArgs a;
  a.z = z; a.Wh = Wh; a.ldw = ldw; a.cs = cs; a.hs = hs; a.out = out; a.nf = num_frames;
  a.ctl = static_cast<unsigned*>(workspace) + CTL_STICKY;
  a.hx = reinterpret_cast<float*>(static_cast<char*>(workspace) + cb);
  a.t0 = (int)t0; a.T = (int)T; a.B = (int)B; a.H = (int)H; a.fb = forget_bias;
  a.NU = geo.NU; a.RB = geo.RB; a.NT16 = geo.NT16; a.per = geo.per; a.pf = geo.pf;
  a.nimg = images_in(workspace_bytes, geo.NT16, H);
  a.dbg = reinterpret_cast<unsigned long long*>(static_cast<char*>(workspace) + workspace_bytes - DBG_BYTES);
  const unsigned grid = (unsigned)(geo.NU * geo.RB);
  int dev = 0;
  device_cus(&dev);
  a.stats = stats_ptr(dev);
  ++g_stat_launches[dev];
  g_stat_wgs[dev] += grid;
  ProfScope prof(F_LSTM, s, 2.0 * (double)T * (double)B * (double)H * 4.0 * (double)H);
  std::lock_guard<std::mutex> lk(g_gate.mu);
  const int total_cus = device_cus(nullptr);
  int grc = g_gate.admit(dev, (int)grid, std::max(0, total_cus - g_reserved_cus), s);
  if (grc != YT8M_OK) return grc;
  YT8M_HIP_CHECK(hipMemsetAsync(a.ctl, 0, (size_t)ctl_bytes(geo.NT16), s));
  const bool x3 = fwd_x3_shape(H, geo.pf) && images_in(workspace_bytes, geo.NT16, H + H / 2) >= T;
  int rc;
  a.wword = static_cast<const unsigned*>(h2_wword);
  if (x3 && !bf16 && h2_wword) {
    hipLaunchKernelGGL((hx_pack_x3_kernel<2, true>), dim3(256), dim3(256), 0, s, hs + t0 * B * H, reinterpret_cast<u32x4*>(a.hx), (int)B, (int)H,
                       geo.NT16);
    rc = launch_status("hx_pack_x3_kernel");
    if (rc != YT8M_OK) return rc;
    if (H == 1024) hipLaunchKernelGGL((lstm_persist_fwd_x3_kernel<4, 2, true>), dim3(grid), dim3(768), 0, s, a);
    else hipLaunchKernelGGL((lstm_persist_fwd_x3_kernel<2, 2, true>), dim3(grid), dim3(768), 0, s, a);
    rc = launch_status("lstm_persist_fwd_x3_kernel");
  } else if (x3 && bf16) {
    hipLaunchKernelGGL(hx_pack_x3_kernel<1>, dim3(256), dim3(256), 0, s, hs + t0 * B * H, reinterpret_cast<u32x4*>(a.hx), (int)B, (int)H,
                       geo.NT16);
    rc = launch_status("hx_pack_x3_kernel");
    if (rc != YT8M_OK) return rc;
    if (H == 1024) hipLaunchKernelGGL((lstm_persist_fwd_x3_kernel<4, 1>), dim3(grid), dim3(768), 0, s, a);
    else hipLaunchKernelGGL((lstm_persist_fwd_x3_kernel<2, 1>), dim3(grid), dim3(768), 0, s, a);
    rc = launch_status("lstm_persist_fwd_x3_kernel");
  } else if (x3) {
    hipLaunchKernelGGL(hx_pack_x3_kernel<3>, dim3(256), dim3(256), 0, s, hs + t0 * B * H, reinterpret_cast<u32x4*>(a.hx), (int)B, (int)H,
                       geo.NT16);
    rc = launch_status("hx_pack_x3_kernel");
    if (rc != YT8M_OK) return rc;
    if (H == 1024) hipLaunchKernelGGL((lstm_persist_fwd_x3_kernel<4>), dim3(grid), dim3(768), 0, s, a);
    else hipLaunchKernelGGL((lstm_persist_fwd_x3_kernel<2>), dim3(grid), dim3(768), 0, s, a);
    rc = launch_status("lstm_persist_fwd_x3_kernel");
  } else {
    hipLaunchKernelGGL(hx_pack_kernel, dim3(256), dim3(256), 0, s, hs + t0 * B * H, a.hx, (int)B, (int)H, geo.NT16);
    rc = launch_status("hx_pack_kernel");
    if (rc != YT8M_OK) return rc;
    switch (geo.NQ) {
      case 1: rc = launch_fwd<1>(a, grid, s); break;
      case 2: rc = launch_fwd<2>(a, grid, s); break;
      case 4: rc = launch_fwd<4>(a, grid, s); break;
      case 6: rc = launch_fwd<6>(a, grid, s); break;
      default: rc = launch_fwd<8>(a, grid, s); break;
    }
  }
  if (rc != YT8M_OK) return rc;
  return g_gate.done(dev, (int)grid, s);
}
}

namespace {
struct GeometryB { int NQB, NUB, RB, NT16, per, pf; };

bool persist_geometry_bwd(int64_t B, int64_t H, GeometryB* geo) {
  static const bool off = getenv("YT8M_NO_PERSIST") != nullptr || getenv("YT8M_NO_PERSIST_BWD") != nullptr;
  if (off || B < 1 || H > 1024 || !(H == 128 || (H >= 256 && (H % 256) == 0))) return false;
  const int NQB = (int)(H / 32);
  if (!(NQB == 4 || NQB == 8 || NQB == 16 || NQB == 24 || NQB == 32)) return false;
  int dev = 0;
  const int cus = device_cus(&dev);
  const int NUB = (int)(H / 16);
  if (cus < NUB) return false;
  const int NT16 = (int)((B + 15) / 16);
  int RB = persist_cu_budget(cus, true) / NUB;
  if (RB > NT16 / 2) RB = NT16 / 2;
  if (RB < 1) RB = 1;
  if ((NT16 + RB - 1) / RB > MAX_LOCAL_TILES) return false;
  const int nit_min = NT16 / RB;
  int per = 0;
  if (RB <= 8 && (8 % RB) == 0 && (NUB % (8 / RB)) == 0) per = 8 / RB;
  if (geo) *geo = {NQB, NUB, RB, NT16, per, nit_min >= 2 ? 1 : 0};
  return true;
}

bool bwd_rot_off() {
  static const bool off = getenv("YT8M_BWD_ROT") != nullptr && atoi(getenv("YT8M_BWD_ROT")) == 0;
  return off;
}
bool bwd_rot(int pf, int NT16, int RB) { return !bwd_rot_off() && pf && (NT16 % (4 * RB)) == 0; }

template <int NQB, bool SH>
int launch_bwd_sh(const PersistBwdArgs& a, unsigned grid, hipStream_t s) {
  const bool rot = bwd_rot(a.pf, a.NT16, a.RB);
  const bool img = a.img_plain || a.img_trans || a.img_trans_s || a.colpart || a.colpart_s;
  if (img) {
    if constexpr (SH) {
      if (!rot) return yt8m::fail(YT8M_E_SHAPE, "operand images need the rotated backward epilogue%s", "");
      hipLaunchKernelGGL((lstm_persist_bwd_kernel<NQB, true, true, true, true>), dim3(grid), dim3(768), 0, s, a);
      return yt8m::launch_status("lstm_persist_bwd_kernel");
    } else {
      return yt8m::fail(YT8M_E_SHAPE, "operand images need one exchange image per step%s", "");
    }
  }
  if constexpr (SH && (NQB == 16 || NQB == 32)) {
    if (a.bf && rot) {
      hipLaunchKernelGGL((lstm_persist_bwd_kernel<NQB, true, true, true, false, true>), dim3(grid), dim3(768), 0, s, a);
      return yt8m::launch_status("lstm_persist_bwd_kernel");
    }
  }
  if constexpr (SH && (NQB == 16 || NQB == 32)) {
    if (a.h2 && rot) {
      const bool tpf = tape_prefetch_on();
      ++g_tpf_launches[tpf ? 1 : 0];
      if (tpf) hipLaunchKernelGGL((lstm_persist_bwd_kernel<NQB, true, true, true, false, false, true, true>), dim3(grid), dim3(768), 0, s, a);
      else hipLaunchKernelGGL((lstm_persist_bwd_kernel<NQB, true, true, true, false, false, true>), dim3(grid), dim3(768), 0, s, a);
      return yt8m::launch_status("lstm_persist_bwd_kernel");
    }
  }
  if (rot) hipLaunchKernelGGL((lstm_persist_bwd_kernel<NQB, true, SH, true>), dim3(grid), dim3(768), 0, s, a);
  else if (a.pf) hipLaunchKernelGGL((lstm_persist_bwd_kernel<NQB, true, SH, false>), dim3(grid), dim3(768), 0, s, a);
  else hipLaunchKernelGGL((lstm_persist_bwd_kernel<NQB, false, SH, false>), dim3(grid), dim3(768), 0, s, a);
  return yt8m::launch_status("lstm_persist_bwd_kernel");
}
template <int NQB>
int launch_bwd(const PersistBwdArgs& a, unsigned grid, hipStream_t s) {
  return a.nimg >= a.T ? launch_bwd_sh<NQB, true>(a, grid, s) : launch_bwd_sh<NQB, false>(a, grid, s);
}
}

extern "C" int yt8m_lstm_persist_bwd_supported(int64_t B, int64_t H) {
  return (persist_geometry(B, H, nullptr) && persist_geometry_bwd(B, H, nullptr)) ? 1 : 0;
}

extern "C" int yt8m_lstm_persist_bwd_images_rows(int64_t B, int64_t H) {
  GeometryB geo;
  if (!persist_geometry(B, H, nullptr) || !persist_geometry_bwd(B, H, &geo)) return 0;
  if ((B % 16) != 0 || !bwd_rot(geo.pf, geo.NT16, geo.RB)) return 0;
  return 4 * geo.RB;
}

namespace {
int persist_bwd_impl(const float* gates, const float* Wh, int64_t ldw, const float* cs, const float* dout, float* dz,
                     float* work, int phase, float* dbias_rows, const int32_t* num_frames, int64_t t0, int64_t T,
                     int64_t B, int64_t H, void* workspace, int64_t workspace_bytes, const yt8m_persist_bwd_images* img,
                     yt8m_stream_t stream, bool bf16 = false, const void* h2_wword = nullptr, void* rowmax = nullptr, void* partmax = nullptr);
int64_t h2_scale_bytes(int NT16, int64_t H, int64_t T) { return ((T * NT16 * (H / 16) * 16 + 255) / 256) * 256; }
}

extern "C" int yt8m_lstm_persist_bwd(const float* gates, const float* Wh, int64_t ldw, const float* cs, const float* dout, float* dz,
                                     float* work, int phase, float* dbias_rows, const int32_t* num_frames, int64_t t0, int64_t T,
                                     int64_t B, int64_t H, void* workspace, int64_t workspace_bytes, yt8m_stream_t stream) {
  return persist_bwd_impl(gates, Wh, ldw, cs, dout, dz, work, phase, dbias_rows, num_frames, t0, T, B, H, workspace, workspace_bytes,
                          nullptr, stream);
}

extern "C" int yt8m_lstm_persist_bwd_bf16(const float* gates, const float* Wh, int64_t ldw, const float* cs, const float* dout, float* dz,
                                          float* work, int phase, float* dbias_rows, const int32_t* num_frames, int64_t t0, int64_t T,
                                          int64_t B, int64_t H, void* workspace, int64_t workspace_bytes, yt8m_stream_t stream) {
  return persist_bwd_impl(gates, Wh, ldw, cs, dout, dz, work, phase, dbias_rows, num_frames, t0, T, B, H, workspace, workspace_bytes,
                          nullptr, stream, true);
}

extern "C" int yt8m_lstm_persist_bwd_h2(const float* gates, const float* Wh, int64_t ldw, const float* cs, const float* dout, float* dz,
                                        float* work, int phase, float* dbias_rows, const int32_t* num_frames, int64_t t0, int64_t T,
                                        int64_t B, int64_t H, const void* wh_absmax, void* workspace, int64_t workspace_bytes,
                                        yt8m_stream_t stream) {
  YT8M_REQUIRE(wh_absmax, YT8M_E_BADARG, "null absmax word");
  static const bool off = getenv("YT8M_PERSIST_BWD_H2") != nullptr && atoi(getenv("YT8M_PERSIST_BWD_H2")) == 0;
  return persist_bwd_impl(gates, Wh, ldw, cs, dout, dz, work, phase, dbias_rows, num_frames, t0, T, B, H, workspace, workspace_bytes,
                          nullptr, stream, false, off ? nullptr : wh_absmax);
}
extern "C" int yt8m_lstm_persist_bwd_ex(const float* gates, const float* Wh, int64_t ldw, const float* cs, const float* dout, float* dz,
                                        float* work, int phase, const int32_t* num_frames, int64_t t0, int64_t T, int64_t B, int64_t H,
                                        const void* wh_absmax, void* rowmax, void* partmax, void* workspace, int64_t workspace_bytes,
                                        yt8m_stream_t stream) {
  static const bool off = getenv("YT8M_PERSIST_BWD_H2") != nullptr && atoi(getenv("YT8M_PERSIST_BWD_H2")) == 0;
  return persist_bwd_impl(gates, Wh, ldw, cs, dout, dz, work, phase, nullptr, num_frames, t0, T, B, H, workspace, workspace_bytes,
                          nullptr, stream, false, off ? nullptr : wh_absmax, rowmax, partmax);
}
extern "C" int yt8m_lstm_persist_bwd_on_f16_pipe(int64_t B, int64_t H) {
  GeometryB geo;
  if (!persist_geometry(B, H, nullptr) || !persist_geometry_bwd(B, H, &geo)) return 0;
  return ((H == 512 || H == 1024) && bwd_rot(geo.pf, geo.NT16, geo.RB)) ? 1 : 0;
}

extern "C" int yt8m_lstm_persist_bwd_images(const float* gates, const float* Wh, int64_t ldw, const float* cs, const float* dout, float* dz,
                                            float* work, int phase, const int32_t* num_frames, int64_t t0, int64_t T, int64_t B,
                                            int64_t H, void* workspace, int64_t workspace_bytes, const yt8m_persist_bwd_images* images,
                                            yt8m_stream_t stream) {
  YT8M_REQUIRE(images, YT8M_E_BADARG, "null image description");
  YT8M_REQUIRE(yt8m_lstm_persist_bwd_images_rows(B, H) > 0, YT8M_E_SHAPE, "shape cannot take the operand images (yt8m_lstm_persist_bwd_images_rows)");
  YT8M_REQUIRE((images->rowscale != nullptr) == (images->trans_scaled != nullptr || images->colpart_scaled != nullptr), YT8M_E_BADARG,
               "rowscale comes with trans_scaled / colpart_scaled");
  YT8M_REQUIRE((((uintptr_t)images->plain | (uintptr_t)images->trans | (uintptr_t)images->trans_scaled) & 15) == 0, YT8M_E_BADARG,
               "images must be 16-byte aligned");
  return persist_bwd_impl(gates, Wh, ldw, cs, dout, dz, work, phase, nullptr, num_frames, t0, T, B, H, workspace, workspace_bytes, images,
                          stream);
}

namespace {
int persist_bwd_impl(const float* gates, const float* Wh, int64_t ldw, const float* cs, const float* dout, float* dz,
                     float* work, int phase, float* dbias_rows, const int32_t* num_frames, int64_t t0, int64_t T,
                     int64_t B, int64_t H, void* workspace, int64_t workspace_bytes, const yt8m_persist_bwd_images* img,
                     yt8m_stream_t stream, bool bf16, const void* h2_wword, void* rowmax, void* partmax) {
  using namespace yt8m;
  YT8M_REQUIRE(t0 >= 0 && T >= 0 && B >= 0 && H >= 0, YT8M_E_SHAPE, "negative dimension");
  YT8M_REQUIRE(phase == 0 || phase == 1, YT8M_E_BADARG, "phase must be 0 or 1");
  if (T * B * H == 0) return YT8M_OK;
  YT8M_REQUIRE(gates && Wh && cs && dz && work && workspace, YT8M_E_BADARG, "null operand");
  YT8M_REQUIRE(ldw >= 4 * H && (ldw % 4) == 0 && (reinterpret_cast<uintptr_t>(Wh) & 15) == 0, YT8M_E_SHAPE,
               "W_h rows must be 16-byte aligned (ldw % 4 == 0)");
  GeometryB geo;
  YT8M_REQUIRE(persist_geometry(B, H, nullptr) && persist_geometry_bwd(B, H, &geo), YT8M_E_SHAPE,
               "shape not supported by the persistent backward recurrence (see yt8m_lstm_persist_bwd_supported)");
  YT8M_REQUIRE(workspace_bytes >= yt8m_lstm_persist_workspace_bytes(B, H), YT8M_E_SHAPE, "workspace too small");
  YT8M_REQUIRE(T < (1 << 20), YT8M_E_SHAPE, "T too large");
  hipStream_t s = as_stream(stream);
  const int64_t cb = ctl_padded(geo.NT16);
  PersistBwdArgs a;
  a.gates = gates; a.Wh = Wh; a.ldw = ldw; a.cs = cs; a.dout = dout; a.dz = dz; a.work = work; a.nf = num_frames;
  a.dbrows = dbias_rows;
  a.img_plain = img ? static_cast<float*>(img->plain) : nullptr;
  a.img_trans = img ? static_cast<float*>(img->trans) : nullptr;
  a.img_trans_s = img ? static_cast<float*>(img->trans_scaled) : nullptr;
  a.rowscale = img ? img->rowscale : nullptr;
  a.colpart = img ? img->colpart : nullptr;
  a.colpart_s = img ? img->colpart_scaled : nullptr;
  a.ctl = static_cast<unsigned*>(workspace) + CTL_STICKY;
  a.dzx = reinterpret_cast<float*>(static_cast<char*>(workspace) + cb);
  a.t0 = (int)t0; a.T = (int)T; a.B = (int)B; a.H = (int)H; a.phase = phase;
  a.NUB = geo.NUB; a.RB = geo.RB; a.NT16 = geo.NT16; a.per = geo.per; a.pf = geo.pf;
  a.nimg = images_in(workspace_bytes, geo.NT16, 4 * H);
  a.bf = (bf16 && !img) ? 1 : 0;
  a.dbg = reinterpret_cast<unsigned long long*>(static_cast<char*>(workspace) + workspace_bytes - DBG_BYTES);
  a.rowmax = static_cast<unsigned*>(rowmax);
  a.partmax = static_cast<unsigned*>(partmax);
  YT8M_REQUIRE(!(rowmax || partmax) || (!img && images_in(workspace_bytes, geo.NT16, 4 * H) >= T && bwd_rot(geo.pf, geo.NT16, geo.RB)), YT8M_E_SHAPE,
               "row / launch maxima need the rotated backward epilogue on a per-step workspace (yt8m_lstm_persist_bwd_images_rows)");
  a.h2 = 0; a.wword = nullptr; a.sc = nullptr; a.sc_bytes = 0;
  if (h2_wword && !img && !bf16 && (H == 512 || H == 1024)) {
    const int64_t scb = h2_scale_bytes(geo.NT16, H, T);
    if (scb < (1LL << 31) && images_in(workspace_bytes - scb, geo.NT16, 4 * H) >= T) {
      a.h2 = 1;
      a.wword = static_cast<const unsigned*>(h2_wword);
      a.sc = reinterpret_cast<unsigned*>(static_cast<char*>(workspace) + workspace_bytes - DBG_BYTES - scb);
      a.sc_bytes = (unsigned)scb;
    }
  }
  const unsigned grid = (unsigned)(geo.NUB * geo.RB);
  int dev = 0;
  device_cus(&dev);
  a.stats = stats_ptr(dev);
  ++g_stat_launches[dev];
  g_stat_wgs[dev] += grid;
  ProfScope prof(F_LSTM_BWD, s, 2.0 * (double)T * (double)B * (double)H * 4.0 * (double)H);
  std::lock_guard<std::mutex> lk(g_gate.mu);
  const int total_cus = device_cus(nullptr);
  int grc = g_gate.admit(dev, (int)grid, std::max(0, total_cus - g_reserved_cus), s);
  if (grc != YT8M_OK) return grc;
  YT8M_HIP_CHECK(hipMemsetAsync(a.ctl, 0, (size_t)ctl_bytes(geo.NT16), s));
  int rc;
  switch (geo.NQB) {
    case 4: rc = launch_bwd<4>(a, grid, s); break;
    case 8: rc = launch_bwd<8>(a, grid, s); break;
    case 16: rc = launch_bwd<16>(a, grid, s); break;
    case 24: rc = launch_bwd<24>(a, grid, s); break;
    default: rc = launch_bwd<32>(a, grid, s); break;
  }
  if (rc != YT8M_OK) return rc;
  return g_gate.done(dev, (int)grid, s);
}
}


extern "C" int yt8m_gru_persist_supported(int64_t B, int64_t H) {
  static const bool off = getenv("YT8M_GRU_PERSIST") != nullptr && atoi(getenv("YT8M_GRU_PERSIST")) == 0;
  Geometry geo;
  return (!off && persist_geometry(B, H, &geo) && geo.NQ >= 2) ? 1 : 0;
}

extern "C" int64_t yt8m_gru_persist_workspace_bytes(int64_t B, int64_t H, int64_t T) {
  Geometry geo;
  if (!persist_geometry(B, H, &geo)) return 0;
  return ctl_padded(geo.NT16) + (3 * std::max<int64_t>(T, 1) + 3) * geo.NT16 * 16 * H * 4 + DBG_BYTES;
}

namespace {
template <int NQ>
int launch_gru_fwd(const GruFwdArgs& a, unsigned grid, hipStream_t s) {
  if (a.pf >= 2) hipLaunchKernelGGL((gru_persist_fwd_kernel<NQ, 2>), dim3(grid), dim3(768), 0, s, a);
  else if (a.pf == 1) hipLaunchKernelGGL((gru_persist_fwd_kernel<NQ, 1>), dim3(grid), dim3(768), 0, s, a);
  else hipLaunchKernelGGL((gru_persist_fwd_kernel<NQ, 0>), dim3(grid), dim3(768), 0, s, a);
  return yt8m::launch_status("gru_persist_fwd_kernel");
}
}

extern "C" int yt8m_gru_persist_fwd(float* zg, float* zc, const float* Wg_h, int64_t ldg, const float* Wc_h, int64_t ldc, float* hs,
                                    float* rh, float* out, const int32_t* num_frames, int64_t t0, int64_t T, int64_t B, int64_t H,
                                    void* workspace, int64_t workspace_bytes, yt8m_stream_t stream) {
  using namespace yt8m;
  YT8M_REQUIRE(t0 >= 0 && T >= 0 && B >= 0 && H >= 0, YT8M_E_SHAPE, "negative dimension");
  if (T * B * H == 0) return YT8M_OK;
  YT8M_REQUIRE(zg && zc && Wg_h && Wc_h && hs && rh && workspace, YT8M_E_BADARG, "null operand");
  YT8M_REQUIRE(ldg >= 2 * H && ldc >= H, YT8M_E_SHAPE, "leading dimension too small");
  Geometry geo;
  YT8M_REQUIRE(yt8m_gru_persist_supported(B, H) && persist_geometry(B, H, &geo), YT8M_E_SHAPE,
               "shape not supported by the persistent GRU recurrence (see yt8m_gru_persist_supported)");
  YT8M_REQUIRE(workspace_bytes >= yt8m_gru_persist_workspace_bytes(B, H, T), YT8M_E_SHAPE, "workspace too small");
  YT8M_REQUIRE(T < (1 << 19), YT8M_E_SHAPE, "T too large");
  hipStream_t s = as_stream(stream);
  GruFwdArgs a;
  a.zg = zg; a.zc = zc; a.Wg = Wg_h; a.Wc = Wc_h; a.ldg = ldg; a.ldc = ldc; a.hs = hs; a.rh = rh; a.out = out; a.nf = num_frames;
  a.ctl = static_cast<unsigned*>(workspace) + CTL_STICKY;
  a.hx = reinterpret_cast<float*>(static_cast<char*>(workspace) + ctl_padded(geo.NT16));
  a.t0 = (int)t0; a.T = (int)T; a.B = (int)B; a.H = (int)H;
  a.NU = geo.NU; a.RB = geo.RB; a.NT16 = geo.NT16; a.per = geo.per; a.pf = geo.pf;
  const unsigned grid = (unsigned)(geo.NU * geo.RB);
  int dev = 0;
  device_cus(&dev);
  a.stats = stats_ptr(dev);
  ++g_stat_launches[dev];
  g_stat_wgs[dev] += grid;
  ProfScope prof(F_LSTM, s, 2.0 * (double)T * (double)B * (double)H * 3.0 * (double)H);
  std::lock_guard<std::mutex> lk(g_gate.mu);
  const int total_cus = device_cus(nullptr);
  int grc = g_gate.admit(dev, (int)grid, std::max(0, total_cus - g_reserved_cus), s);
  if (grc != YT8M_OK) return grc;
  YT8M_HIP_CHECK(hipMemsetAsync(a.ctl, 0, (size_t)ctl_bytes(geo.NT16), s));
  hipLaunchKernelGGL(hx_pack_kernel, dim3(256), dim3(256), 0, s, hs + t0 * B * H, a.hx, (int)B, (int)H, geo.NT16);
// ... 12 lines not shown
```

### youtube-8m_amd/csrc/lstm_stack.hip

```cpp
#include <stdlib.h>
#include <algorithm>
#include <mutex>
#include <vector>
#include "common.h"

using namespace yt8m;

namespace {

constexpr int MAXL = 8, MAXP = 64;
constexpr int MAXBP = 62;
constexpr float U8_ALPHA = 4.0f / 255.0f;
constexpr float U8_BETA = 128.0f * (4.0f / 255.0f) + (4.0f / 512.0f - 2.0f);
constexpr int64_t X3_MIN_ROWS = 1024;
constexpr int64_t STEP_IMAGES_MAX_BYTES = 8LL << 30;
constexpr float H2_S = 8192.0f;

int64_t up256(int64_t v) { return (v + 255) / 256 * 256; }

int knob(const char* name, int dflt) { const char* v = getenv(name); return v ? atoi(v) : dflt; }

struct Part { int64_t t0, T; };
int chunks(int64_t F, int n, Part* out) {
  if (n < 1) n = 1;
  if (n > F) n = (int)F;
  if (n > MAXP) n = MAXP;
  const int64_t step = (F + n - 1) / n;
  int k = 0;
  for (int64_t t0 = 0; t0 < F; t0 += step) out[k++] = {t0, std::min(step, F - t0)};
  return k;
}

struct Plan {
  int64_t B, F, D, H, FB;
  int L, u8, need_dx;
  int bf16;
  int nf, nb;
  Part fp[MAXP], bp[MAXP];
  int64_t z[MAXL], cs[MAXL], hs[MAXL], out[MAXL], rrow, tape_bytes;
  int64_t pws[MAXL], pws_bytes;
  int64_t gws[MAXL + 1], gws_bytes;
  int64_t gwx[MAXL], gws2;
  int64_t qimg, w3t, wcs, wxt3[MAXL], xi[MAXL];
  int64_t dz[MAXL], dbuf[MAXL], work[MAXL];
  int64_t dz3[MAXL], wx3[MAXL], dzT3[MAXL], dzT3s, csr, dbdummy;
  int64_t xT[MAXL], hT[MAXL];
  int64_t cpart[MAXL], cparts;
  bool colparts;
  int img_rows;
  int h2;
  int64_t hsc;
  int64_t hx0;
  int64_t hrow, hrow_stride;
  float keep;
  uint64_t seed[MAXL];
  int emit_max;
  int64_t rmax, rmax_stride;
  int64_t cimg[MAXL], cimgs;
  int64_t scratch_bytes;
};

int64_t x3_bytes(int64_t rows, int64_t K) { return yt8m_x3_image_bytes(rows, K); }
int64_t x1_bytes(int64_t rows, int64_t K) { return ((rows + 31) / 32) * ((K + 15) / 16) * 1024; }

const char* plan(const yt8m_lstm_stack_desc* d, Plan* P) {
  if (!d) return "null description";
  if (d->L < 1 || d->L > MAXL) return "1..8 layers";
  if (d->B < 1 || d->F < 1 || d->D < 1 || d->H < 1) return "empty dimension";
  Plan& p = *P;
  p.B = d->B; p.F = d->F; p.D = d->D; p.H = d->H; p.L = d->L; p.u8 = (d->input_u8 & 1) != 0; p.need_dx = d->need_dx != 0;
  p.bf16 = (d->input_u8 & 2) != 0;
  p.FB = p.F * p.B;
  if (p.FB >= (1LL << 31) - 64) return "too many frame rows";
  if (!yt8m_lstm_persist_supported(p.B, p.H) || !yt8m_lstm_persist_bwd_supported(p.B, p.H))
    return "shape not covered by the persistent recurrence kernels";
  if (p.FB < X3_MIN_ROWS || p.H < 128) return "too small for the bf16-pipe products";
  if (p.u8 && (p.D % 16 != 0 || p.D > 2048)) return "uint8 input needs D % 16 == 0 and D <= 2048";
  if (p.u8 && p.need_dx) return "no gradient with respect to uint8 frames";
  if (p.FB % 16 != 0) return "F * B must be a multiple of 16 (K ranges of the transposed operand images)";
  p.nf = chunks(p.F, d->fwd_chunks > 0 ? d->fwd_chunks : 1, p.fp);
  p.nb = chunks(p.F, std::min(d->bwd_chunks > 0 ? d->bwd_chunks : 3, MAXBP), p.bp);
  static const char* dflt_parts = "2,2,1,1";
  const char* spec = getenv("YT8M_STACK_BWD_PARTS");
  if (!spec && d->bwd_chunks <= 0 && p.F >= 12) spec = dflt_parts;
  if (spec) {
    double w[MAXP], tot = 0;
    int n = 0;
    for (const char* q = spec; *q && n < MAXBP;) { w[n] = atof(q); tot += w[n++]; while (*q && *q != ',') ++q; if (*q) ++q; }
    if (n >= 1 && tot > 0) {
      int64_t t0 = 0; double acc = 0; int k = 0;
      Part pp[MAXP];
      for (int i = 0; i < n; ++i) {
        acc += w[i];
        int64_t t1 = i + 1 == n ? p.F : (int64_t)(p.F * acc / tot + 0.5);
        if (t1 > t0) { pp[k++] = {t0, t1 - t0}; t0 = t1; }
      }
      bool ok = k >= 1;
      for (int i = 0; i < k; ++i) ok = ok && (pp[i].t0 * p.B) % 16 == 0 && (pp[i].T * p.B) % 16 == 0;
      if (ok) { p.nb = k; for (int i = 0; i < k; ++i) p.bp[i] = pp[i]; }
    }
  }
  int64_t tmax = 0;
  for (int c = 0; c < p.nf; ++c) {
    if (p.u8 && (p.fp[c].t0 * p.B) % 32 != 0) return "a forward chunk does not start on a 32-row group of the frame image";
    tmax = std::max(tmax, p.fp[c].T);
  }
  for (int c = 0; c < p.nb; ++c) {
    if ((p.bp[c].t0 * p.B) % 16 != 0 || (p.bp[c].T * p.B) % 16 != 0) return "a backward part is not a multiple of 16 frame rows";
    tmax = std::max(tmax, p.bp[c].T);
  }
  const int64_t BH = p.B * p.H, FBH = p.FB * p.H;
  int64_t o = 0;
  for (int l = 0; l < p.L; ++l) {
    p.z[l] = o; o += up256(FBH * 4 * 4);
    p.cs[l] = o; o += up256((FBH + BH) * 4);
    p.hs[l] = o; o += up256((FBH + BH) * 4);
    p.out[l] = o; o += up256(FBH * 4);
  }
  p.rrow = o; o += up256(p.FB * 4);
  p.tape_bytes = o;
  int64_t pb = yt8m_lstm_persist_workspace_bytes_steps(p.B, p.H, tmax);
  const bool per_step = pb <= STEP_IMAGES_MAX_BYTES;
  if (!per_step) pb = yt8m_lstm_persist_workspace_bytes(p.B, p.H);
  p.pws_bytes = up256(pb);
  o = 0;
  for (int l = 0; l < p.L; ++l) { p.pws[l] = o; o += p.pws_bytes; }
  p.gws_bytes = up256(yt8m_gemm_workspace_bytes());
  for (int l = 0; l <= p.L; ++l) { p.gws[l] = o; o += p.gws_bytes; }
  for (int l = 0; l < p.L; ++l) { p.gwx[l] = o; o += p.gws_bytes; }
  p.gws2 = o; o += p.gws_bytes;
  auto ib = [&](int64_t rows, int64_t K) { return p.bf16 ? x1_bytes(rows, K) : x3_bytes(rows, K); };
  const int64_t H4 = 4 * p.H;
  p.qimg = o; o += p.u8 ? up256(x1_bytes(p.FB, p.D)) : 0;
  p.w3t = o; o += p.u8 ? up256(ib(H4, p.D)) : 0;
  p.wcs = o; o += up256(H4 * 4);
  int64_t fmax = 0, bmax = 0;
  for (int c = 0; c < p.nf; ++c) fmax = std::max(fmax, p.fp[c].T * p.B);
  for (int c = 0; c < p.nb; ++c) bmax = std::max(bmax, p.bp[c].T * p.B);
  for (int l = 0; l < p.L; ++l) {
    const int64_t Din = l ? p.H : p.D;
    const bool x1 = l == 0 && p.u8;
    p.wxt3[l] = o; o += x1 ? 0 : up256(ib(H4, Din));
    p.xi[l] = o; o += x1 ? 0 : up256(ib(fmax, Din));
    p.dz[l] = o; o += up256(FBH * 4 * 4);
    p.dbuf[l] = o; o += l + 1 < p.L ? up256(FBH * 4) : 0;
    p.work[l] = o; o += up256(4 * BH * 4);
    const bool dxl = l > 0 || p.need_dx;
    p.dz3[l] = o; o += dxl ? up256(ib(bmax, H4)) : 0;
    p.wx3[l] = o; o += dxl ? up256(ib(Din, H4)) : 0;
    p.xT[l] = o; o += x1 ? up256(x1_bytes(p.D, p.FB)) : up256(ib(Din, p.FB));
    p.hT[l] = o; o += up256(ib(p.H, p.FB));
  }
  p.h2 = (knob("YT8M_STACK_H2", 1) && !p.bf16) ? 1 : 0;
  p.keep = (d->input_keep_prob > 0.f && d->input_keep_prob < 1.f) ? d->input_keep_prob : 0.f;
  for (int l = 0; l < MAXL; ++l) p.seed[l] = d->dropout_seed[l];
  if (d->input_keep_prob < 0.f || d->input_keep_prob > 1.f) return "input_keep_prob must be in [0, 1]";
  if (p.keep > 0.f && (p.u8 || !p.h2 || p.keep < 0.3f || (p.D % 4) != 0 || (p.H % 4) != 0))
    return "input dropout: float input, f16 product forms (YT8M_STACK_H2), keep_prob >= 0.3, D % 4 == 0";
  p.img_rows = (knob("YT8M_STACK_FUSED_IMAGES", 0) && !p.bf16 && !p.h2) ? yt8m_lstm_persist_bwd_images_rows(p.B, p.H) : 0;
  const int64_t trows = p.img_rows ? p.FB : bmax;
  for (int l = 0; l < p.L; ++l) { p.dzT3[l] = o; o += up256(ib(H4, trows)); }
  p.dzT3s = o; o += p.u8 ? up256(ib(H4, trows)) : 0;
  const int64_t ci = p.img_rows ? up256((int64_t)p.img_rows * MAXP * 2 * H4 * 4) : 0;
  for (int l = 0; l < p.L; ++l) { p.cimg[l] = o; o += ci; }
  p.cimgs = o; o += p.u8 ? ci : 0;
  p.csr = o; o += up256(H4 * 4);
  p.dbdummy = o; o += up256(H4 * 4);
  p.hsc = o; o += 256 * MAXL;
  p.hx0 = o; o += 256;
  p.hrow_stride = up256(bmax * 4);
  p.hrow = o; o += p.h2 ? p.hrow_stride * 2 * MAXL : 0;
  p.emit_max = (p.h2 && knob("YT8M_STACK_DZ_MAXIMA", 1) && yt8m_lstm_persist_bwd_images_rows(p.B, p.H) > 0 && per_step && p.nb <= 61) ? 1 : 0;
  p.rmax_stride = up256(p.FB * 4);
  p.rmax = o; o += p.emit_max ? p.rmax_stride * p.L : 0;
  p.colparts = knob("YT8M_STACK_COLPARTS", 1) != 0;
  for (int c = 0; c < p.nb; ++c) p.colparts = p.colparts && (p.bp[c].t0 * p.B) % 64 == 0 && (p.bp[c].T * p.B) % 64 == 0;
  const int64_t cp = p.colparts ? up256(((p.FB + 63) / 64) * H4 * 4) : 0;
  for (int l = 0; l < p.L; ++l) { p.cpart[l] = o; o += cp; }
  p.cparts = o; o += p.u8 ? cp : 0;
  p.scratch_bytes = o;
  return nullptr;
}

struct DevState {
  hipStream_t rs[MAXL] = {nullptr};
  hipStream_t dxs[MAXL] = {nullptr};
  hipStream_t sw = nullptr, sw2 = nullptr;
  int prio = 0;
  bool prio_known = false;
  std::vector<hipEvent_t> ev[2];
  size_t used[2] = {0, 0};
  hipEvent_t layer_done[MAXL] = {nullptr};
  int layers_done = 0;
};
std::mutex g_mu;
constexpr int NSETS = 2;
DevState g_dev[NSETS][16];
thread_local int g_set = 0;
thread_local yt8m_stream_hook g_prep_hook = nullptr;
thread_local void* g_prep_user = nullptr;
struct EarlyOpt {
  bool set = false;
  yt8m_opt_ranges o;
  std::vector<int32_t> tcs, job_tensor;
  std::vector<int64_t> tile_base;
};
thread_local EarlyOpt g_early;

int high_stream(DevState& S, hipStream_t* s) {
  if (*s) return YT8M_OK;
  if (!S.prio_known) {
    int least = 0, greatest = 0;
    YT8M_HIP_CHECK(hipDeviceGetStreamPriorityRange(&least, &greatest));
    S.prio = greatest;
    S.prio_known = true;
  }
  YT8M_HIP_CHECK(hipStreamCreateWithPriority(s, hipStreamNonBlocking, S.prio));
  return YT8M_OK;
}
int plain_stream(hipStream_t* s) {
  if (*s) return YT8M_OK;
  YT8M_HIP_CHECK(hipStreamCreateWithFlags(s, hipStreamNonBlocking));
  return YT8M_OK;
}

int dev_state(int L, DevState** out) {
  int dev = 0;
  YT8M_HIP_CHECK(hipGetDevice(&dev));
  YT8M_REQUIRE(dev >= 0 && dev < 16, YT8M_E_BADARG, "device index out of range");
  DevState& S = g_dev[g_set][dev];
  for (int l = 0; l < L; ++l) { int rc = high_stream(S, &S.rs[l]); if (rc != YT8M_OK) return rc; }
  { int rc = plain_stream(&S.sw); if (rc != YT8M_OK) return rc; }
  if (knob("YT8M_STACK_DX_STREAM", 0))
    for (int l = 0; l < L; ++l) { int rc = high_stream(S, &S.dxs[l]); if (rc != YT8M_OK) return rc; }
  if (knob("YT8M_STACK_SW2", 0)) { int rc = plain_stream(&S.sw2); if (rc != YT8M_OK) return rc; }
  *out = &S;
  return YT8M_OK;
}

struct Ev {
  DevState& S;
  int dir;
  int rc = YT8M_OK;
  Ev(DevState& s, int d) : S(s), dir(d) { S.used[d] = 0; }
  hipEvent_t record(hipStream_t st) {
    if (S.used[dir] == S.ev[dir].size()) {
      hipEvent_t e;
      if (hipEventCreateWithFlags(&e, hipEventDisableTiming) != hipSuccess) { rc = fail(YT8M_E_HIP, "hipEventCreate failed%s", ""); return nullptr; }
      S.ev[dir].push_back(e);
    }
    hipEvent_t e = S.ev[dir][S.used[dir]++];
    if (hipEventRecord(e, st) != hipSuccess) rc = fail(YT8M_E_HIP, "hipEventRecord failed%s", "");
    return e;
  }
  void wait(hipStream_t st, hipEvent_t e) {
    if (e && hipStreamWaitEvent(st, e, 0) != hipSuccess) rc = fail(YT8M_E_HIP, "hipStreamWaitEvent failed%s", "");
  }
};

#define RC(expr) do { int _rc = (expr); if (_rc != YT8M_OK) return _rc; } while (0)

template <typename T> T* at(void* base, int64_t off) { return reinterpret_cast<T*>(static_cast<char*>(base) + off); }

}

extern "C" int yt8m_lstm_stack_supported(const yt8m_lstm_stack_desc* desc) {
  Plan P;
  const char* why = plan(desc, &P);
  if (why) { snprintf(g_err, sizeof(g_err), "yt8m_lstm_stack: %s", why); return 0; }
  return 1;
}
extern "C" int64_t yt8m_lstm_stack_tape_bytes(const yt8m_lstm_stack_desc* desc) {
  Plan P;
  return plan(desc, &P) ? 0 : P.tape_bytes;
}
extern "C" int64_t yt8m_lstm_stack_scratch_bytes(const yt8m_lstm_stack_desc* desc) {
  Plan P;
  return plan(desc, &P) ? 0 : P.scratch_bytes;
// ... 38 lines not shown
  }
  return YT8M_OK;
}

extern "C" int yt8m_lstm_stack_layer_done_wait(int layer, yt8m_stream_t stream) {
  int dev = 0;
  YT8M_HIP_CHECK(hipGetDevice(&dev));
  YT8M_REQUIRE(dev >= 0 && dev < 16, YT8M_E_BADARG, "device index out of range");
  std::lock_guard<std::mutex> lk(g_mu);
  DevState& S = g_dev[g_set][dev];
  YT8M_REQUIRE(layer >= 0 && layer < S.layers_done && S.layer_done[layer], YT8M_E_BADARG,
               "no backward call on this device has recorded that layer");
  YT8M_HIP_CHECK(hipStreamWaitEvent(as_stream(stream), S.layer_done[layer], 0));
  return YT8M_OK;
}

extern "C" int yt8m_lstm_stack_status(const yt8m_lstm_stack_desc* desc, void* scratch, yt8m_stream_t stream) {
  Plan P;
  const char* why = plan(desc, &P);
  YT8M_REQUIRE(!why, YT8M_E_SHAPE, why ? why : "");
  YT8M_REQUIRE(scratch, YT8M_E_BADARG, "null scratch");
  int rc = YT8M_OK;
  for (int l = 0; l < P.L; ++l) {
    const int r = yt8m_lstm_persist_status(at<char>(scratch, P.pws[l]), stream);
    if (r != YT8M_OK) rc = r;
  }
  return rc;
}

extern "C" int yt8m_lstm_stack_set_prep_hook(yt8m_stream_hook hook, void* user) {
  g_prep_hook = hook;
  g_prep_user = user;
  return YT8M_OK;
}

extern "C" int yt8m_lstm_stack_set_early_optimizer(const yt8m_opt_ranges* opt) {
  g_early.set = false;
  if (!opt) return YT8M_OK;
  YT8M_REQUIRE(opt->nranges >= 1 && opt->nranges <= 8 && opt->tensor_chunk_start_host, YT8M_E_BADARG, "1..8 ranges + the host chunk starts");
  int hi = 0;
  for (int r = 0; r < opt->nranges; ++r) {
    YT8M_REQUIRE(opt->range_lo[r] >= 0 && opt->range_hi[r] >= opt->range_lo[r], YT8M_E_BADARG, "bad tensor range");
    hi = std::max(hi, (int)opt->range_hi[r]);
  }
  YT8M_REQUIRE(opt->njobs >= 0 && (opt->njobs == 0 || (opt->job_tensor_host && opt->job_tile_base_host)), YT8M_E_BADARG, "job tables");
  g_early.o = *opt;
  g_early.tcs.assign(opt->tensor_chunk_start_host, opt->tensor_chunk_start_host + hi + 1);
  g_early.o.tensor_chunk_start_host = g_early.tcs.data();
  g_early.job_tensor.clear();
  g_early.tile_base.clear();
  if (opt->njobs) {
    g_early.job_tensor.assign(opt->job_tensor_host, opt->job_tensor_host + opt->njobs);
    g_early.tile_base.assign(opt->job_tile_base_host, opt->job_tile_base_host + opt->njobs + 1);
    g_early.o.job_tensor_host = g_early.job_tensor.data();
    g_early.o.job_tile_base_host = g_early.tile_base.data();
  }
  g_early.set = true;
  return YT8M_OK;
}

extern "C" int yt8m_lstm_stack_fwd(const yt8m_lstm_stack_desc* desc, const void* x, const int32_t* num_frames, const float* const* W,
                                   const float* const* b, void* tape, int64_t tape_bytes, void* scratch, int64_t scratch_bytes,
                                   yt8m_stream_t stream) {
  Plan P;
  const char* why = plan(desc, &P);
  YT8M_REQUIRE(!why, YT8M_E_SHAPE, why ? why : "");
  YT8M_REQUIRE(x && W && b && tape && scratch, YT8M_E_BADARG, "null operand");
  YT8M_REQUIRE(tape_bytes >= P.tape_bytes && scratch_bytes >= P.scratch_bytes, YT8M_E_BADARG, "tape / scratch too small");
  YT8M_REQUIRE(((reinterpret_cast<uintptr_t>(tape) | reinterpret_cast<uintptr_t>(scratch)) & 255) == 0, YT8M_E_BADARG,
               "tape and scratch must be 256-byte aligned");
  for (int l = 0; l < P.L; ++l) YT8M_REQUIRE(W[l] && b[l], YT8M_E_BADARG, "null weights");
  std::lock_guard<std::mutex> lk(g_mu);
  DevState* S = nullptr;
  RC(dev_state(P.L, &S));
  Ev ev(*S, 0);
  hipStream_t main = as_stream(stream);
  const int64_t B = P.B, D = P.D, H = P.H, H4 = 4 * H, BH = B * H;
  const bool bf = P.bf16 != 0;
  auto split = [&](const float* src, int64_t R, int64_t C, int64_t ld, float scale, void* plain, void* trans, hipStream_t st) {
    return bf ? yt8m_bf16_image(src, R, C, ld, scale, plain, trans, (yt8m_stream_t)st) : yt8m_x3_split(src, R, C, ld, scale, plain, trans, (yt8m_stream_t)st);
  };
  hipEvent_t start = ev.record(main);
  for (int l = 0; l < P.L; ++l) ev.wait(S->rs[l], start);
  const void* wxt_img[MAXL] = {nullptr};
  for (int l = 0; l < P.L; ++l) {
    hipStream_t s = S->rs[l];
    const int64_t Din = l ? H : D;
    YT8M_HIP_CHECK(hipMemsetAsync(at<char>(tape, P.cs[l]), 0, (size_t)BH * 4, s));
    YT8M_HIP_CHECK(hipMemsetAsync(at<char>(tape, P.hs[l]), 0, (size_t)BH * 4, s));
    if (!bf) {
      YT8M_HIP_CHECK(hipMemsetAsync(at<char>(scratch, P.hsc + 256 * l + 252), 0, 4, s));
      RC(yt8m_h2_absmax(W[l] + Din * H4, H, H4, H4, at<char>(scratch, P.hsc + 256 * l + 252), (yt8m_stream_t)s));
    }
    if (l == 0 && P.u8) {
      if (P.h2) {
        RC(yt8m_u8_frames_image_f16(static_cast<const uint8_t*>(x), num_frames, B, P.F, D, 1e-12f, at<char>(scratch, P.qimg), nullptr,
                                    at<float>(tape, P.rrow), s));
        float* word = at<float>(scratch, P.hsc);
        YT8M_HIP_CHECK(hipMemsetAsync(word, 0, 4, s));
        RC(yt8m_h2_absmax(W[0], D, H4, H4, word, (yt8m_stream_t)s));
        RC(yt8m_h2_split(W[0], D, H4, H4, U8_ALPHA, word, nullptr, at<char>(scratch, P.w3t), nullptr, (yt8m_stream_t)s));
        wxt_img[0] = at<char>(scratch, P.w3t);
      } else {
      RC(yt8m_u8_frames_image(static_cast<const uint8_t*>(x), num_frames, B, P.F, D, 1e-12f, at<char>(scratch, P.qimg), nullptr,
                              at<float>(tape, P.rrow), s));
      wxt_img[0] = yt8m_wimg_lookup(W[0], D, H4, H4, 1, bf ? 1 : 3, U8_ALPHA);
      if (!wxt_img[0]) {
        RC(split(W[0], D, H4, H4, U8_ALPHA, nullptr, at<char>(scratch, P.w3t), s));
        wxt_img[0] = at<char>(scratch, P.w3t);
      }
      }
      RC(yt8m_colsum_f32(W[0], D, H4, H4, at<float>(scratch, P.wcs), 0.f, at<char>(scratch, P.gws[0]), P.gws_bytes, s));
    } else {
      if (P.h2) {
        float* word = at<float>(scratch, P.hsc + 256 * l);
        YT8M_HIP_CHECK(hipMemsetAsync(word, 0, 4, s));
        RC(yt8m_h2_absmax(W[l], Din, H4, H4, word, (yt8m_stream_t)s));
        RC(yt8m_h2_split(W[l], Din, H4, H4, 1.0f, word, nullptr, at<char>(scratch, P.wxt3[l]), nullptr, (yt8m_stream_t)s));
        wxt_img[l] = at<char>(scratch, P.wxt3[l]);
        if (l == 0) {
          YT8M_HIP_CHECK(hipMemsetAsync(at<char>(scratch, P.hx0), 0, 4, s));
          RC(yt8m_h2_absmax(static_cast<const float*>(x), P.FB, D, D, at<char>(scratch, P.hx0), (yt8m_stream_t)s));
        }
        continue;
      }
      wxt_img[l] = yt8m_wimg_lookup(W[l], Din, H4, H4, 1, bf ? 1 : 3, 1.0f);
      if (!wxt_img[l]) {
        RC(split(W[l], Din, H4, H4, 1.0f, nullptr, at<char>(scratch, P.wxt3[l]), s));
        wxt_img[l] = at<char>(scratch, P.wxt3[l]);
      }
    }
  }
  std::vector<hipEvent_t> done((size_t)P.L * P.nf, nullptr);
  static const int fwd_half = knob("YT8M_STACK_FWD_HALF", 0);
  struct CapGuard {
    bool on;
    int fwd = -1, bwd = -1;
    explicit CapGuard(bool o) : on(o) {
      if (!on) return;
      yt8m_lstm_persist_get_cus(&fwd, &bwd);
      yt8m_lstm_persist_set_cus(fwd > 0 ? std::min(fwd, 128) : 128, bwd);
    }
    ~CapGuard() { if (on) yt8m_lstm_persist_set_cus(fwd, bwd); }
  } cap_guard(fwd_half != 0 && P.L >= 2 && P.nf >= 2);
  for (int c = 0; c < P.nf; ++c) {
    const int64_t t0 = P.fp[c].t0, T = P.fp[c].T, M = T * B;
    for (int l = 0; l < P.L; ++l) {
      hipStream_t s = S->rs[l];
      const int64_t Din = l ? H : D;
      if (l > 0) ev.wait(s, done[(size_t)(l - 1) * P.nf + c]);
      float* zc = at<float>(tape, P.z[l]) + t0 * B * H4;
      void* gw = at<char>(scratch, P.gws[l]);
      static const int chain_combine = knob("YT8M_STACK_CHAIN_COMBINE", 0);
      if (chain_combine) yt8m_x3_set_combine(1);
      if (l == 0 && P.u8) {
        const char* qi = at<char>(scratch, P.qimg) + (t0 * B / 32) * (D / 16) * 1024;
        const int prc = P.h2 ? yt8m_gemm_h1x2_nt_ex(M, H4, D, qi, 0, wxt_img[0], 0, zc, H4, b[0], 1.0f, at<float>(scratch, P.hsc),
                                                    at<float>(tape, P.rrow) + t0 * B, at<float>(scratch, P.wcs), U8_BETA, 0.f, gw, P.gws_bytes, s)
                           : bf ? yt8m_gemm_b1_nt_ex(M, H4, D, qi, 0, wxt_img[0], 0, zc, H4, b[0], 1.0f, at<float>(tape, P.rrow) + t0 * B,
                                                at<float>(scratch, P.wcs), U8_BETA, 0.f, gw, P.gws_bytes, s)
                           : yt8m_gemm_x1x3_nt(M, H4, D, qi, wxt_img[0], zc, H4, b[0], at<float>(tape, P.rrow) + t0 * B,
                                               at<float>(scratch, P.wcs), U8_BETA, gw, P.gws_bytes, s);
        yt8m_x3_set_combine(0);
        RC(prc);
      } else {
        const float* src = l ? at<float>(tape, P.out[l - 1]) + t0 * B * H : static_cast<const float*>(x) + t0 * B * D;
        yt8m_gemm_problem pr = {M, H4, Din, at<char>(scratch, P.xi[l]), 0, wxt_img[l], 0, zc, H4, b[l], 0.0f};
        int grc;
        if (P.h2 && l >= 1) {
          if (P.keep > 0.f)
            RC(yt8m_h2_split_dropout(src, M, Din, H2_S, nullptr, at<char>(scratch, P.xi[l]), nullptr, P.keep, P.seed[l], t0 * B * Din, (yt8m_stream_t)s));
          else
          RC(yt8m_h2_split(src, M, Din, Din, H2_S, nullptr, at<char>(scratch, P.xi[l]), nullptr, nullptr, (yt8m_stream_t)s));
          const float alpha = 1.0f / H2_S;
          const float* dsb = at<float>(scratch, P.hsc + 256 * l);
          grc = yt8m_gemm_h2_nt_grouped(1, &pr, &alpha, nullptr, &dsb, gw, P.gws_bytes, (yt8m_stream_t)s);
        } else if (P.h2) {
          const float* dsa = at<float>(scratch, P.hx0);
          const float* dsb = at<float>(scratch, P.hsc);
          if (P.keep > 0.f)
            RC(yt8m_h2_split_dropout(src, M, Din, 1.0f, dsa, at<char>(scratch, P.xi[0]), nullptr, P.keep, P.seed[0], t0 * B * Din, (yt8m_stream_t)s));
          else
          RC(yt8m_h2_split(src, M, Din, Din, 1.0f, dsa, at<char>(scratch, P.xi[0]), nullptr, nullptr, (yt8m_stream_t)s));
          const float alpha = 1.0f;
          grc = yt8m_gemm_h2_nt_grouped(1, &pr, &alpha, &dsa, &dsb, gw, P.gws_bytes, (yt8m_stream_t)s);
        } else {
          RC(split(src, M, Din, Din, 1.0f, at<char>(scratch, P.xi[l]), nullptr, s));
          grc = bf ? yt8m_gemm_b1_nt_grouped(1, &pr, gw, P.gws_bytes, s) : yt8m_gemm_x3_nt_grouped(1, &pr, gw, P.gws_bytes, s);
        }
        yt8m_x3_set_combine(0);
        RC(grc);
      }
      static const int bf_recur_f = knob("YT8M_STACK_BF16_RECUR", 1);
      static const int h2_recur_f_env = knob("YT8M_STACK_H2_RECUR_FWD", -1);
      const int h2_recur_f = h2_recur_f_env >= 0 ? h2_recur_f_env : P.h2;
      if (!bf && h2_recur_f)
        RC(yt8m_lstm_persist_fwd_h2(at<float>(tape, P.z[l]), W[l] + Din * H4, H4, at<float>(tape, P.cs[l]), at<float>(tape, P.hs[l]),
                                    at<float>(tape, P.out[l]), num_frames, t0, T, B, H, desc->forget_bias,
                                    at<char>(scratch, P.hsc + 256 * l + 252), at<char>(scratch, P.pws[l]), P.pws_bytes, s));
      else
      RC((bf && bf_recur_f ? yt8m_lstm_persist_fwd_bf16 : yt8m_lstm_persist_fwd)(
          at<float>(tape, P.z[l]), W[l] + Din * H4, H4, at<float>(tape, P.cs[l]), at<float>(tape, P.hs[l]), at<float>(tape, P.out[l]),
          num_frames, t0, T, B, H, desc->forget_bias, at<char>(scratch, P.pws[l]), P.pws_bytes, s));
      done[(size_t)l * P.nf + c] = ev.record(s);
    }
  }
  for (int l = 0; l < P.L; ++l) ev.wait(main, done[(size_t)l * P.nf + P.nf - 1]);
  return ev.rc;
}

extern "C" int yt8m_lstm_stack_bwd(const yt8m_lstm_stack_desc* desc, const void* x, const int32_t* num_frames, const float* const* W,
                                   void* tape, int64_t tape_bytes, void* scratch, int64_t scratch_bytes, const float* dout_top,
                                   const float* const* dc_final, const float* const* dh_final, float* const* dW, float* const* db,
                                   const float* beta_W, const float* beta_b, float* dx, yt8m_stream_t stream) {
  Plan P;
  const char* why = plan(desc, &P);
  YT8M_REQUIRE(!why, YT8M_E_SHAPE, why ? why : "");
  YT8M_REQUIRE(x && W && tape && scratch && dW && db, YT8M_E_BADARG, "null operand");
  YT8M_REQUIRE(tape_bytes >= P.tape_bytes && scratch_bytes >= P.scratch_bytes, YT8M_E_BADARG, "tape / scratch too small");
  YT8M_REQUIRE(!P.need_dx || dx, YT8M_E_BADARG, "need_dx is set but dx is NULL");
  for (int l = 0; l < P.L; ++l) {
    YT8M_REQUIRE(W[l], YT8M_E_BADARG, "null weights");
    YT8M_REQUIRE(!beta_W || beta_W[l] == 0.f || beta_W[l] == 1.f, YT8M_E_BADARG, "beta must be 0 or 1");
    YT8M_REQUIRE(!beta_b || beta_b[l] == 0.f || beta_b[l] == 1.f, YT8M_E_BADARG, "beta must be 0 or 1");
  }
  std::lock_guard<std::mutex> lk(g_mu);
  DevState* S = nullptr;
  RC(dev_state(P.L, &S));
  Ev ev(*S, 1);
  hipStream_t main = as_stream(stream), sw = S->sw;
  static const int dx_stream = knob("YT8M_STACK_DX_STREAM", 0), two_sw = knob("YT8M_STACK_SW2", 0);
  const int fuse_dz = P.h2 ? 0 : knob("YT8M_STACK_FUSE_DZ_SPLIT", 0);
  const int64_t B = P.B, D = P.D, H = P.H, H4 = 4 * H, BH = B * H, FB = P.FB;
  const int64_t KBtot = FB / 16;
  const bool bf = P.bf16 != 0;
  const int64_t KBB = bf ? 1024 : 3072;
  auto split = [&](const float* src, int64_t R, int64_t C, int64_t ld, float scale, void* plain, void* trans, hipStream_t st) {
    return bf ? yt8m_bf16_image(src, R, C, ld, scale, plain, trans, (yt8m_stream_t)st) : yt8m_x3_split(src, R, C, ld, scale, plain, trans, (yt8m_stream_t)st);
  };
  auto gemm = [&](int n, const yt8m_gemm_problem* pr, void* ws, int64_t wsb, hipStream_t st) {
    return bf ? yt8m_gemm_b1_nt_grouped(n, pr, ws, wsb, (yt8m_stream_t)st) : yt8m_gemm_x3_nt_grouped(n, pr, ws, wsb, (yt8m_stream_t)st);
  };
  hipEvent_t start = ev.record(main);
  ev.wait(sw, start);
  if (two_sw) ev.wait(S->sw2, start);
  for (int l = 0; l < P.L; ++l) { ev.wait(S->rs[l], start); if (dx_stream) ev.wait(S->dxs[l], start); }
  if (P.h2)
    for (int l = 0; l < P.L; ++l) {
      YT8M_HIP_CHECK(hipMemsetAsync(at<char>(scratch, P.hsc + 256 * l + 4), 0, 248, S->rs[l]));
      if (P.emit_max && l >= 1) YT8M_HIP_CHECK(hipMemsetAsync(at<char>(scratch, P.rmax + l * P.rmax_stride), 0, (size_t)FB * 4, S->rs[l]));
    }
  for (int l = 0; l < P.L; ++l) {
    if (!dW[l]) continue;
    if (l == 0 && P.u8) {
      if (P.h2) RC(yt8m_u8_frames_image_t_f16(static_cast<const uint8_t*>(x), num_frames, B, P.F, D, at<char>(scratch, P.xT[0]), sw));
      else RC(yt8m_u8_frames_image_t(static_cast<const uint8_t*>(x), num_frames, B, P.F, D, at<char>(scratch, P.xT[0]), sw));
    } else {
      const float* src = l ? at<float>(tape, P.out[l - 1]) : static_cast<const float*>(x);
      const int64_t Din = l ? H : D;
      if (P.h2 && P.keep > 0.f)
        RC(yt8m_h2_split_dropout(src, FB, Din, l ? H2_S : 1.0f, l ? nullptr : at<float>(scratch, P.hx0), nullptr, at<char>(scratch, P.xT[l]),
                                 P.keep, P.seed[l], 0, (yt8m_stream_t)sw));
      else if (P.h2 && l >= 1) RC(yt8m_h2_split(src, FB, Din, Din, H2_S, nullptr, nullptr, at<char>(scratch, P.xT[l]), nullptr, (yt8m_stream_t)sw));
      else if (P.h2) RC(yt8m_h2_split(src, FB, Din, Din, 1.0f, at<float>(scratch, P.hx0), nullptr, at<char>(scratch, P.xT[0]), nullptr, (yt8m_stream_t)sw));
      else RC(split(src, FB, Din, Din, 1.0f, nullptr, at<char>(scratch, P.xT[l]), sw));
    }
    if (P.h2) RC(yt8m_h2_split(at<float>(tape, P.hs[l]), FB, H, H, H2_S, nullptr, nullptr, at<char>(scratch, P.hT[l]), nullptr, (yt8m_stream_t)sw));
    else RC(split(at<float>(tape, P.hs[l]), FB, H, H, 1.0f, nullptr, at<char>(scratch, P.hT[l]), sw));
  }
  yt8m_stream_hook hook = g_prep_hook;
  void* hook_user = g_prep_user;
  g_prep_hook = nullptr;
  g_prep_user = nullptr;
  bool early = g_early.set;
  g_early.set = false;
  if (two_sw) ev.wait(S->sw2, ev.record(sw));
  int phase[MAXL];
  bool wx3_done[MAXL];
  const void* wx_img[MAXL] = {nullptr};
  hipEvent_t dzT_free[MAXL] = {nullptr};
  const bool fused_img = P.img_rows > 0 && !dx_stream && !fuse_dz;
  int64_t img_done_rows[MAXL] = {0};
  int img_launches[MAXL] = {0};
  for (int l = 0; l < P.L; ++l) {
    hipStream_t s = S->rs[l];
    float* work = at<float>(scratch, P.work[l]);
    const float* dh = dh_final ? dh_final[l] : nullptr;
    const float* dc = dc_final ? dc_final[l] : nullptr;
    if (dh) YT8M_HIP_CHECK(hipMemcpyAsync(work, dh, (size_t)BH * 4, hipMemcpyDeviceToDevice, s));
    else YT8M_HIP_CHECK(hipMemsetAsync(work, 0, (size_t)BH * 4, s));
    if (dc) YT8M_HIP_CHECK(hipMemcpyAsync(work + BH, dc, (size_t)BH * 4, hipMemcpyDeviceToDevice, s));
    else YT8M_HIP_CHECK(hipMemsetAsync(work + BH, 0, (size_t)BH * 4, s));
    phase[l] = 0;
    wx3_done[l] = false;
  }
  std::vector<hipEvent_t> last;
  int sub0[MAXP];
  for (int c = 0; c < P.nb; ++c) sub0[c] = (c == 0 && P.L > 1 && P.nb > 1 && !getenv("YT8M_STACK_SUB0")) ? std::max(1, knob("YT8M_STACK_SUB0_LAST", 1)) : 1;
  if (const char* spec = getenv("YT8M_STACK_SUB0")) {
    int n = 0;
    for (const char* q = spec; *q && n < P.nb;) { sub0[n++] = std::max(1, atoi(q)); while (*q && *q != ',') ++q; if (*q) ++q; }
  }
  for (int c = P.nb - 1; c >= 0; --c) {
    hipEvent_t dx_ev = nullptr;
    for (int l = P.L - 1; l >= 0; --l) {
     Part sp[MAXP];
     int nsub = (l == 0 && P.L > 1 && !P.emit_max) ? std::min(sub0[c], MAXP) : 1;
     if (nsub > 1) {
       const int64_t step = (P.bp[c].T + nsub - 1) / nsub;
       int k = 0;
       bool ok = (step * B) % (P.colparts ? 64 : 16) == 0;
       for (int64_t u = 0; ok && u < P.bp[c].T; u += step) sp[k++] = {P.bp[c].t0 + u, std::min(step, P.bp[c].T - u)};
       nsub = ok ? k : 1;
     }
     if (nsub == 1) sp[0] = P.bp[c];
     for (int j = nsub - 1; j >= 0; --j) {
      const int64_t t0 = sp[j].t0, T = sp[j].T, M = T * B;
      const int64_t kb0 = t0 * B / 16;
      const bool first = c == P.nb - 1 && j == nsub - 1;
      hipStream_t s = S->rs[l];
      const int64_t Din = l ? H : D;
      if (dx_ev && j == nsub - 1) ev.wait(s, dx_ev);
      const float* dout = l == P.L - 1 ? dout_top : at<float>(scratch, P.dbuf[l]);
      float* dz = at<float>(scratch, P.dz[l]);
      const int64_t toff = fused_img ? (H4 / 32) * (img_done_rows[l] / 16) * 3072 : 0;
      char* dzT_img = at<char>(scratch, P.dzT3[l]) + toff;
      char* dzTs_img = at<char>(scratch, P.dzT3s) + toff;
      if (fused_img && img_launches[l] < 2 * MAXP) {
        const bool dxl = l > 0 || P.need_dx;
        yt8m_persist_bwd_images im;
        im.plain = dxl ? at<char>(scratch, P.dz3[l]) : nullptr;
        im.trans = dW[l] ? dzT_img : nullptr;
        const bool sc = dW[l] && l == 0 && P.u8;
        im.trans_scaled = sc ? dzTs_img : nullptr;
        im.rowscale = sc ? at<float>(tape, P.rrow) : nullptr;
        im.colpart = at<float>(scratch, P.cimg[l]) + (int64_t)img_launches[l] * P.img_rows * H4;
        im.colpart_scaled = sc ? at<float>(scratch, P.cimgs) + (int64_t)img_launches[l] * P.img_rows * H4 : nullptr;
        RC(yt8m_lstm_persist_bwd_images(at<float>(tape, P.z[l]), W[l] + Din * H4, H4, at<float>(tape, P.cs[l]), dout, dz,
                                        at<float>(scratch, P.work[l]), phase[l], num_frames, t0, T, B, H, at<char>(scratch, P.pws[l]),
                                        P.pws_bytes, &im, s));
        img_done_rows[l] += M;
        ++img_launches[l];
      } else {
        YT8M_REQUIRE(!fused_img, YT8M_E_SHAPE, "YT8M_STACK_FUSED_IMAGES: more backward launches per layer than image slots (YT8M_STACK_SUB0)");
        static const int bf_recur = knob("YT8M_STACK_BF16_RECUR", 1);
        static const int h2_recur = knob("YT8M_STACK_H2_RECUR", 1);
        static const int h2_dx_rows = knob("YT8M_STACK_H2_DX", 1);
        if (P.emit_max)
          RC(yt8m_lstm_persist_bwd_ex(at<float>(tape, P.z[l]), W[l] + Din * H4, H4, at<float>(tape, P.cs[l]), dout, dz,
                                      at<float>(scratch, P.work[l]), phase[l], num_frames, t0, T, B, H,
                                      h2_recur ? at<char>(scratch, P.hsc + 256 * l + 252) : nullptr,
                                      (l >= 1 && h2_dx_rows) ? at<char>(scratch, P.rmax + l * P.rmax_stride) : nullptr,
                                      at<char>(scratch, P.hsc + 256 * l + 4 * (1 + c)), at<char>(scratch, P.pws[l]), P.pws_bytes, s));
        else if (!bf && h2_recur)
          RC(yt8m_lstm_persist_bwd_h2(at<float>(tape, P.z[l]), W[l] + Din * H4, H4, at<float>(tape, P.cs[l]), dout, dz,
                                      at<float>(scratch, P.work[l]), phase[l], nullptr, num_frames, t0, T, B, H,
                                      at<char>(scratch, P.hsc + 256 * l + 252), at<char>(scratch, P.pws[l]), P.pws_bytes, s));
        else
        RC((bf && bf_recur ? yt8m_lstm_persist_bwd_bf16 : yt8m_lstm_persist_bwd)(
            at<float>(tape, P.z[l]), W[l] + Din * H4, H4, at<float>(tape, P.cs[l]), dout, dz, at<float>(scratch, P.work[l]), phase[l],
            nullptr, num_frames, t0, T, B, H, at<char>(scratch, P.pws[l]), P.pws_bytes, s));
      }
      phase[l] = (int)((phase[l] + T) % 2);
      hipEvent_t rb = ev.record(s);
      if (hook) {
        hook(hook_user, (yt8m_stream_t)S->sw);
        hook = nullptr;
      }
      if (early) {
        early = false;
        RC(yt8m_optimizer_ranges(&g_early.o, (yt8m_stream_t)S->sw));
      }
      bool fused_t = false;
      const float* dzc = dz + t0 * B * H4;
      if (j == nsub - 1) dx_ev = nullptr;
      if (l > 0 || P.need_dx) {
        hipStream_t sx = dx_stream ? S->dxs[l] : s;
        if (dx_stream) ev.wait(sx, rb);
        fused_t = fuse_dz && dW[l] && !(l == 0 && P.u8);
        if (fused_t && dzT_free[l]) ev.wait(sx, dzT_free[l]);
        static const int h2_dx_knob = knob("YT8M_STACK_H2_DX", 1);
        const bool dx_h2 = P.h2 && l >= 1 && h2_dx_knob;
        if (dx_h2) {
          float* rS = at<float>(scratch, P.hrow + 2 * l * P.hrow_stride);
          float* rI = at<float>(scratch, P.hrow + (2 * l + 1) * P.hrow_stride);
          if (P.emit_max) {
            RC(yt8m_h2_split_rowmax(dzc, M, H4, H4, at<char>(scratch, P.rmax + l * P.rmax_stride + t0 * B * 4), rI, at<char>(scratch, P.dz3[l]),
                                    (yt8m_stream_t)sx));
          } else {
            RC(yt8m_h2_rowscales(dzc, M, H4, H4, rS, rI, (yt8m_stream_t)sx));
            RC(yt8m_h2_split_rows(dzc, M, H4, H4, rS, at<char>(scratch, P.dz3[l]), (yt8m_stream_t)sx));
          }
          const float* wword = at<float>(scratch, P.hsc + 256 * l);
          if (!wx3_done[l]) {
            RC(yt8m_h2_split(W[l], Din, H4, H4, 1.0f, wword, at<char>(scratch, P.wx3[l]), nullptr, nullptr, (yt8m_stream_t)sx));
            wx3_done[l] = true;
          }
          float* dst = at<float>(scratch, P.dbuf[l - 1]) + t0 * B * H;
          RC(yt8m_gemm_h2_nt_ex(M, Din, H4, at<char>(scratch, P.dz3[l]), 0, at<char>(scratch, P.wx3[l]), 0, dst, Din, nullptr, 1.0f, nullptr,
                                wword, rI, 0.0f, at<char>(scratch, dx_stream ? P.gwx[l] : P.gws[l]), P.gws_bytes, (yt8m_stream_t)sx));
          if (P.keep > 0.f)
            RC(yt8m_dropout_f32(dst, dst, M * Din, P.keep, P.seed[l], t0 * B * Din, (yt8m_stream_t)sx));
          dx_ev = ev.record(sx);
          if (c == 0 && j == 0) last.push_back(dx_ev);
        } else {
        if (!fused_img)
          RC(split(dzc, M, H4, H4, 1.0f, at<char>(scratch, P.dz3[l]), fused_t ? at<char>(scratch, P.dzT3[l]) : nullptr, sx));
        if (fused_t) rb = ev.record(sx);
        if (!wx3_done[l]) {
          wx_img[l] = yt8m_wimg_lookup(W[l], Din, H4, H4, 0, bf ? 1 : 3, 1.0f);
          if (!wx_img[l]) {
            RC(split(W[l], Din, H4, H4, 1.0f, at<char>(scratch, P.wx3[l]), nullptr, sx));
            wx_img[l] = at<char>(scratch, P.wx3[l]);
          }
          wx3_done[l] = true;
        }
        float* dst = l ? at<float>(scratch, P.dbuf[l - 1]) + t0 * B * H : dx + t0 * B * D;
        yt8m_gemm_problem pr = {M, Din, H4, at<char>(scratch, P.dz3[l]), 0, wx_img[l], 0, dst, Din, nullptr, 0.0f};
        static const int chain_combine_b = knob("YT8M_STACK_CHAIN_COMBINE", 0);
        if (chain_combine_b) yt8m_x3_set_combine(1);
        const int grc = gemm(1, &pr, at<char>(scratch, dx_stream ? P.gwx[l] : P.gws[l]), P.gws_bytes, sx);
        yt8m_x3_set_combine(0);
        RC(grc);
        if (P.keep > 0.f) RC(yt8m_dropout_f32(dst, dst, M * Din, P.keep, P.seed[l], t0 * B * Din, (yt8m_stream_t)sx));
        dx_ev = ev.record(sx);
        if (c == 0 && j == 0) last.push_back(dx_ev);
        }
      }
      hipStream_t sw = (two_sw && l == 0) ? S->sw2 : S->sw;
      ev.wait(sw, rb);
      void* gw = at<char>(scratch, (two_sw && l == 0) ? P.gws2 : P.gws[P.L]);
      const float bW = first ? (beta_W ? beta_W[l] : 0.f) : 1.f;
      const bool lastpart = c == 0 && j == 0;
      if (dW[l]) {
        if (l == 0 && P.u8 && P.h2) {
          const float* rr = at<float>(tape, P.rrow) + t0 * B;
          float* word = at<float>(scratch, P.hsc) + 1 + c;
          if (!P.emit_max) RC(yt8m_h2_absmax(dzc, M, H4, H4, word, (yt8m_stream_t)sw));
          float* cp = P.colparts ? at<float>(scratch, P.cpart[l]) + (t0 * B / 64) * H4 : nullptr;
          float* cps = P.colparts ? at<float>(scratch, P.cparts) + (t0 * B / 64) * H4 : nullptr;
// ... 93 lines not shown
```

Measured before the change: 8305 videos/s.

## Precompute split-f16 recurrent weight fragment images for persistent LSTM kernels

Adds kernels that convert the recurrent weight matrix into pre-scaled, split-half f16 MFMA fragment images once per step, one for forward and one for backward. The persistent forward and backward kernels then load their register and LDS weight fragments directly from these images instead of gathering and splitting fp32 weights inside each persistent block. The stack driver allocates the image scratch, builds the forward image on a neighbouring stream alongside the absmax pass, and builds the backward image after the forward recurrence. Event tracking keyed by buffer address orders image reuse. This adds extra conversion launches and scratch memory and makes the cross-stream synchronisation more complex.

```diff
diff --git a/include/yt8m_hip.h b/include/yt8m_hip.h
--- a/include/yt8m_hip.h
+++ b/include/yt8m_hip.h
@@ -399,6 +399,18 @@
 int yt8m_lstm_persist_bwd_ex(const float* gates, const float* Wh, int64_t ldw, const float* cs, const float* dout, float* dz, float* work,
                              int phase, const int32_t* num_frames, int64_t t0, int64_t T, int64_t B, int64_t H, const void* wh_absmax,
                              void* rowmax, void* partmax, void* workspace, int64_t workspace_bytes, yt8m_stream_t stream);
+int64_t yt8m_lstm_persist_wh_image_bytes(int64_t H, int direction);
+int yt8m_lstm_persist_wh_image(const float* Wh, int64_t ldw, int64_t H, const void* wh_absmax, int direction, void* image, yt8m_stream_t stream);
+int yt8m_lstm_persist_fwd_h2_img(float* z, const float* Wh, int64_t ldw, float* cs, float* hs, float* out, const int32_t* num_frames,
+                                 int64_t t0, int64_t T, int64_t B, int64_t H, float forget_bias, const void* wh_absmax, const void* wh_image,
+                                 void* workspace, int64_t workspace_bytes, yt8m_stream_t stream);
+int yt8m_lstm_persist_bwd_ex_img(const float* gates, const float* Wh, int64_t ldw, const float* cs, const float* dout, float* dz, float* work,
+                                 int phase, const int32_t* num_frames, int64_t t0, int64_t T, int64_t B, int64_t H, const void* wh_absmax,
+                                 const void* wh_image, void* rowmax, void* partmax, void* workspace, int64_t workspace_bytes,
+                                 yt8m_stream_t stream);
+int yt8m_lstm_persist_set_wh_image(int mode);
+int yt8m_lstm_persist_wh_image_on(void);
+int yt8m_lstm_persist_wh_image_launches(int64_t* fwd_with, int64_t* fwd_without, int64_t* bwd_with, int64_t* bwd_without);
 typedef struct yt8m_persist_bwd_images {
   void* plain;
   void* trans;
diff --git a/youtube-8m_amd/_lib.py b/youtube-8m_amd/_lib.py
--- a/youtube-8m_amd/_lib.py
+++ b/youtube-8m_amd/_lib.py
@@ -220,6 +220,13 @@
     "yt8m_lstm_persist_bwd_h2": (c_int, [P, P, c_int64, P, P, P, P, c_int, P, P, c_int64, c_int64, c_int64, c_int64, P, P, c_int64, P]),
     "yt8m_lstm_persist_bwd_on_f16_pipe": (c_int, [c_int64, c_int64]),
     "yt8m_lstm_persist_bwd_ex": (c_int, [P, P, c_int64, P, P, P, P, c_int, P, c_int64, c_int64, c_int64, c_int64, P, P, P, P, c_int64, P]),
+    "yt8m_lstm_persist_wh_image_bytes": (c_int64, [c_int64, c_int]),
+    "yt8m_lstm_persist_wh_image": (c_int, [P, c_int64, c_int64, P, c_int, P, P]),
+    "yt8m_lstm_persist_fwd_h2_img": (c_int, [P, P, c_int64, P, P, P, P, c_int64, c_int64, c_int64, c_int64, c_float, P, P, P, c_int64, P]),
+    "yt8m_lstm_persist_bwd_ex_img": (c_int, [P, P, c_int64, P, P, P, P, c_int, P, c_int64, c_int64, c_int64, c_int64, P, P, P, P, P, c_int64, P]),
+    "yt8m_lstm_persist_set_wh_image": (c_int, [c_int]),
+    "yt8m_lstm_persist_wh_image_on": (c_int, []),
+    "yt8m_lstm_persist_wh_image_launches": (c_int, [ctypes.POINTER(c_int64)] * 4),
     "yt8m_h2_split_rowmax": (c_int, [P, c_int64, c_int64, c_int64, P, P, P, P]),
     "yt8m_lstm_persist_bwd_images_rows": (c_int, [c_int64, c_int64]),
     "yt8m_lstm_persist_bwd_images": (c_int, [P, P, c_int64, P, P, P, P, c_int, P, c_int64, c_int64, c_int64, c_int64, P, c_int64, P, P]),
diff --git a/youtube-8m_amd/csrc/lstm_persist.hip b/youtube-8m_amd/csrc/lstm_persist.hip
--- a/youtube-8m_amd/csrc/lstm_persist.hip
+++ b/youtube-8m_amd/csrc/lstm_persist.hip
@@ -34,6 +34,7 @@
   int nimg;
   const unsigned* wword;
   unsigned long long* dbg;
+  const void* wimg;
 };
 
 #ifdef YT8M_PERSIST_TIMING
@@ -423,9 +424,10 @@
   }
 }
 
-template <int NKB, int NP = 3, bool F16 = false>
+template <int NKB, int NP = 3, bool F16 = false, bool WIMG = false>
 __global__ __launch_bounds__(768) void lstm_persist_fwd_x3_kernel(PersistFwdArgs a) {
   static_assert(!F16 || NP == 2, "the f16 form has two planes");
+  static_assert(!WIMG || F16, "the fragment image belongs to the f16 form");
   constexpr int NS = 2;
   constexpr int EPW = 2;
   constexpr int NF = NKB * 2 * NP;
@@ -494,8 +496,14 @@
 
   if (w < 8) {
     u32x4 Wr[NREG];
-#pragma unroll
-    for (int f = 0; f < NREG; ++f) Wr[f] = w_frag(f / (2 * NP), (f / NP) & 1, f % NP);
+    if constexpr (WIMG) {
+      const u32x4* wi = static_cast<const u32x4*>(a.wimg) + ((long long)(ug * 8 + w) * NF) * 64 + lane;
+#pragma unroll
+      for (int f = 0; f < NREG; ++f) Wr[f] = wi[f * 64];
+    } else {
+#pragma unroll
+      for (int f = 0; f < NREG; ++f) Wr[f] = w_frag(f / (2 * NP), (f / NP) & 1, f % NP);
+    }
     const unsigned lane_off = (unsigned)lane * 16u + (unsigned)(w * NKB) * (NP * 1024u);
     auto load_half = [&](u32x4 (&Hh)[HK][NP], int s, int T, int half) {
       const __amdgpu_buffer_rsrc_t hxr = image(s);
@@ -755,6 +763,7 @@
   const float* rowscale;
   float* colpart;
   float* colpart_s;
+  const void* wimg;
 };
 
 constexpr int NSLOT_B = 3;
@@ -786,9 +795,10 @@
 }
 
 
-template <int NQB, bool PF, bool SH, bool ROT, bool IMG = false, bool BF = false, bool H2 = false, bool TPF = false>
+template <int NQB, bool PF, bool SH, bool ROT, bool IMG = false, bool BF = false, bool H2 = false, bool TPF = false, bool WIMG = false>
 __global__ __launch_bounds__(768) void lstm_persist_bwd_kernel(PersistBwdArgs a) {
   static_assert(!TPF || H2, "the tape prefetch belongs to the two-half-plane form");
+  static_assert(!WIMG || H2, "the fragment image belongs to the two-half-plane form");
   static_assert(!IMG || ROT, "the operand images are written by the rotated epilogue");
   static_assert(!BF || (PF && SH && ROT && !IMG && (NQB % 4) == 0), "the bf16-operand form: prefetching, one image per step, rotated epilogue");
   static_assert(!H2 || (PF && SH && ROT && !IMG && !BF && (NQB % 8) == 0), "the two-half-plane form: prefetching, one image per step, rotated epilogue");
@@ -842,13 +852,19 @@
     fhi.x = hb[0] | (hb[1] << 16); fhi.y = hb[2] | (hb[3] << 16); fhi.z = hb[4] | (hb[5] << 16); fhi.w = hb[6] | (hb[7] << 16);
     flo.x = lb[0] | (lb[1] << 16); flo.y = lb[2] | (lb[3] << 16); flo.z = lb[4] | (lb[5] << 16); flo.w = lb[6] | (lb[7] << 16);
   };
+  const u32x4* wimg_w = WIMG ? static_cast<const u32x4*>(a.wimg) + ((long long)(ub * 8 + (w & 7)) * 2 * HALF) * 64 + lane : nullptr;
   if constexpr (H2) {
     if (w < 8) {
+      if constexpr (WIMG) {
+#pragma unroll
+        for (int kbl = 0; kbl < HALF; ++kbl) Wl[w][kbl][lane] = as_f4(wimg_w[(HALF + kbl) * 64]);
+      } else {
 #pragma unroll
       for (int kbl = 0; kbl < HALF; ++kbl) {
         u32x4 fhi, flo;
         w_frag_h2(kbl, fhi, flo);
         Wl[w][kbl][lane] = as_f4(flo);
+      }
       }
     }
   }
@@ -947,8 +963,13 @@
     if (w < 8) {
       constexpr int NPW = NQB / 4, PH = NPW / 2;
       u32x4 Wh_[HALF];
-#pragma unroll
-      for (int kbl = 0; kbl < HALF; ++kbl) { u32x4 flo; w_frag_h2(kbl, Wh_[kbl], flo); }
+      if constexpr (WIMG) {
+#pragma unroll
+        for (int kbl = 0; kbl < HALF; ++kbl) Wh_[kbl] = wimg_w[kbl * 64];
+      } else {
+#pragma unroll
+        for (int kbl = 0; kbl < HALF; ++kbl) { u32x4 flo; w_frag_h2(kbl, Wh_[kbl], flo); }
+      }
       const float inv_sw = 1.0f / h2_sw;
       const int lane_off = lane * 16;
       auto blk = [&](int T) -> int { return __builtin_amdgcn_readfirstlane((T * QH4 + w * NQB) * 1024); };
@@ -1744,6 +1765,75 @@
   return g_tape_prefetch_mode == 1 || (g_tape_prefetch_mode == 0 && !env_off);
 }
 
+std::atomic<long long> g_whimg_launches[2][2] = {{{0}, {0}}, {{0}, {0}}};
+thread_local int g_wh_image_mode = 0;
+bool wh_image_on() {
+  static const bool env_off = getenv("YT8M_PERSIST_WH_IMAGE") != nullptr && atoi(getenv("YT8M_PERSIST_WH_IMAGE")) == 0;
+  return g_wh_image_mode == 1 || (g_wh_image_mode == 0 && !env_off);
+}
+
+constexpr int FWD_UNITS = 8, BWD_UNITS = 16;
+bool h2_form_width(int64_t H) { return H == 512 || H == 1024; }
+int fwd_h2_nkb(int64_t H) { return (int)(H / 256); }
+int bwd_nqb(int64_t H) { return (int)(H / 32); }
+
+__device__ __forceinline__ u32x4 pack_halves(const unsigned (&hb)[8]) {
+  u32x4 v;
+  v.x = hb[0] | (hb[1] << 16); v.y = hb[2] | (hb[3] << 16); v.z = hb[4] | (hb[5] << 16); v.w = hb[6] | (hb[7] << 16);
+  return v;
+}
+template <int NKB>
+__global__ __launch_bounds__(256) void wh_image_fwd_kernel(const float* __restrict__ Wh, long long ldw, int H, const unsigned* __restrict__ wword,
+                                                           u32x4* __restrict__ img) {
+  __shared__ float tile[32][4][33];
+  const int kb = blockIdx.x % NKB, w = (blockIdx.x / NKB) & 7, ugq = blockIdx.x / (NKB * 8);
+  const long long k0 = (long long)(w * NKB + kb) * 32;
+  for (int e = threadIdx.x; e < 32 * 4 * 32; e += 256) {
+    const int c = e & 31, g4 = (e >> 5) & 3, r = e >> 7;
+    tile[r][g4][c] = Wh[(k0 + r) * ldw + (long long)g4 * H + ugq * 32 + c];
+  }
+  __syncthreads();
+  const float sw = yt8m_x3::pow2_scale_for(__uint_as_float(wword[0]), 14);
+  for (int o = threadIdx.x; o < 4 * 4 * 64; o += 256) {
+    const int lane = o & 63, p = (o >> 6) & 1, ct = (o >> 7) & 1, ugl = o >> 8;
+    const int n16 = lane & 15, kg = lane >> 4;
+    unsigned hb[8];
+#pragma unroll
+    for (int j = 0; j < 8; ++j) {
+      unsigned h1, h2;
+      yt8m_x3::split_h2(tile[kg * 8 + j][n16 & 3][ugl * 8 + ct * 4 + (n16 >> 2)] * sw, h1, h2);
+      hb[j] = p == 0 ? h1 : h2;
+    }
+    const int ug = ugq * 4 + ugl, f = kb * 4 + ct * 2 + p;
+    img[((long long)(ug * 8 + w) * (NKB * 4) + f) * 64 + lane] = pack_halves(hb);
+  }
+}
+template <int HALF>
+__global__ __launch_bounds__(256) void wh_image_bwd_kernel(const float* __restrict__ Wh, long long ldw, int H, const unsigned* __restrict__ wword,
+                                                           u32x4* __restrict__ img) {
+  constexpr int C = 8 * HALF;
+  __shared__ float tile[16][4][C + 1];
+  const int w = blockIdx.x & 7, ub = blockIdx.x >> 3;
+  for (int e = threadIdx.x; e < 16 * 4 * C; e += 256) {
+    const int c = e % C, g4 = (e / C) & 3, r = e / (4 * C);
+    tile[r][g4][c] = Wh[(long long)(ub * 16 + r) * ldw + (long long)g4 * H + w * C + c];
+  }
+  __syncthreads();
+  const float sw = yt8m_x3::pow2_scale_for(__uint_as_float(wword[0]), 14);
+  for (int o = threadIdx.x; o < 2 * HALF * 64; o += 256) {
+    const int lane = o & 63, kbl = (o >> 6) % HALF, pl = o / (64 * HALF);
+    const int i16 = lane & 15, kq = lane >> 4;
+    unsigned hb[8];
+#pragma unroll
+    for (int j = 0; j < 8; ++j) {
+      unsigned h1, h2;
+      yt8m_x3::split_h2(tile[i16][j & 3][8 * kbl + 2 * kq + (j >> 2)] * sw, h1, h2);
+      hb[j] = pl == 0 ? h1 : h2;
+    }
+    img[((long long)(ub * 8 + w) * 2 * HALF) * 64 + o] = pack_halves(hb);
+  }
+}
+
 struct Geometry { int NQ, NU, RB, NT16, per, pf; };
 
 bool persist_geometry(int64_t B, int64_t H, Geometry* geo) {
@@ -1753,7 +1843,7 @@
   if (!(NQ == 1 || NQ == 2 || NQ == 4 || NQ == 6 || NQ == 8)) return false;
   int dev = 0;
   const int cus = device_cus(&dev);
-  const int NU = (int)(H / 8);
+  const int NU = (int)(H / FWD_UNITS);
   if (cus < NU) return false;
   const int NT16 = (int)((B + 15) / 16);
   int RB = persist_cu_budget(cus) / NU;
@@ -1826,12 +1916,55 @@
   return YT8M_OK;
 }
 
+extern "C" int yt8m_lstm_persist_set_wh_image(int mode) {
+  YT8M_REQUIRE(mode >= 0 && mode <= 2, YT8M_E_BADARG, "mode must be 0 (default), 1 (on) or 2 (off)");
+  g_wh_image_mode = mode;
+  return YT8M_OK;
+}
+
+extern "C" int yt8m_lstm_persist_wh_image_on(void) { return wh_image_on() ? 1 : 0; }
+
+extern "C" int yt8m_lstm_persist_wh_image_launches(int64_t* fwd_with, int64_t* fwd_without, int64_t* bwd_with, int64_t* bwd_without) {
+  if (fwd_with) *fwd_with = g_whimg_launches[0][1].load();
+  if (fwd_without) *fwd_without = g_whimg_launches[0][0].load();
+  if (bwd_with) *bwd_with = g_whimg_launches[1][1].load();
+  if (bwd_without) *bwd_without = g_whimg_launches[1][0].load();
+  return YT8M_OK;
+}
+
+extern "C" int64_t yt8m_lstm_persist_wh_image_bytes(int64_t H, int direction) {
+  if ((direction != 0 && direction != 1) || !h2_form_width(H)) return 0;
+  return direction == 0 ? (H / FWD_UNITS) * 8 * (int64_t)(fwd_h2_nkb(H) * 4) * 1024 : (H / BWD_UNITS) * 8 * (int64_t)bwd_nqb(H) * 1024;
+}
+
+extern "C" int yt8m_lstm_persist_wh_image(const float* Wh, int64_t ldw, int64_t H, const void* wh_absmax, int direction, void* image,
+                                          yt8m_stream_t stream) {
+  YT8M_REQUIRE(Wh && wh_absmax && image, YT8M_E_BADARG, "null operand");
+  YT8M_REQUIRE(direction == 0 || direction == 1, YT8M_E_BADARG, "direction must be 0 (forward) or 1 (backward)");
+  YT8M_REQUIRE(yt8m_lstm_persist_wh_image_bytes(H, direction) > 0, YT8M_E_SHAPE, "no f16 form of the recurrence at this width");
+  YT8M_REQUIRE(ldw >= 4 * H, YT8M_E_SHAPE, "ldw < 4H");
+  YT8M_REQUIRE((reinterpret_cast<uintptr_t>(image) & 15) == 0, YT8M_E_BADARG, "the image must be 16-byte aligned");
+  hipStream_t s = as_stream(stream);
+  const unsigned* word = static_cast<const unsigned*>(wh_absmax);
+  u32x4* img = static_cast<u32x4*>(image);
+  if (direction == 0) {
+    const unsigned grid = (unsigned)((H / FWD_UNITS / 4) * 8 * fwd_h2_nkb(H));
+    if (fwd_h2_nkb(H) == 4) hipLaunchKernelGGL(wh_image_fwd_kernel<4>, dim3(grid), dim3(256), 0, s, Wh, (long long)ldw, (int)H, word, img);
+    else hipLaunchKernelGGL(wh_image_fwd_kernel<2>, dim3(grid), dim3(256), 0, s, Wh, (long long)ldw, (int)H, word, img);
+    return launch_status("wh_image_fwd_kernel");
+  }
+  const unsigned grid = (unsigned)((H / BWD_UNITS) * 8);
+  if (bwd_nqb(H) == 32) hipLaunchKernelGGL(wh_image_bwd_kernel<16>, dim3(grid), dim3(256), 0, s, Wh, (long long)ldw, (int)H, word, img);
+  else hipLaunchKernelGGL(wh_image_bwd_kernel<8>, dim3(grid), dim3(256), 0, s, Wh, (long long)ldw, (int)H, word, img);
+  return launch_status("wh_image_bwd_kernel");
+}
+
 extern "C" int yt8m_lstm_persist_supported(int64_t B, int64_t H) { return persist_geometry(B, H, nullptr) ? 1 : 0; }
 
 namespace {
 bool fwd_x3_shape(int64_t H, int pf) {
   static const bool x3_off = getenv("YT8M_PERSIST_X3") != nullptr && atoi(getenv("YT8M_PERSIST_X3")) == 0;
-  return !x3_off && (H == 512 || H == 1024) && pf >= 1;
+  return !x3_off && h2_form_width(H) && pf >= 1;
 }
 }
 
@@ -1897,7 +2030,7 @@
 namespace {
 int persist_fwd_impl(float* z, const float* Wh, int64_t ldw, float* cs, float* hs, float* out, const int32_t* num_frames, int64_t t0,
                      int64_t T, int64_t B, int64_t H, float forget_bias, void* workspace, int64_t workspace_bytes, yt8m_stream_t stream,
-                     bool bf16, const void* h2_wword = nullptr);
+                     bool bf16, const void* h2_wword = nullptr, const void* wimg = nullptr);
 }
 extern "C" int yt8m_lstm_persist_fwd_h2(float* z, const float* Wh, int64_t ldw, float* cs, float* hs, float* out,
                                         const int32_t* num_frames, int64_t t0, int64_t T, int64_t B, int64_t H, float forget_bias,
@@ -1907,6 +2040,16 @@
   return persist_fwd_impl(z, Wh, ldw, cs, hs, out, num_frames, t0, T, B, H, forget_bias, workspace, workspace_bytes, stream, false,
                           off ? nullptr : wh_absmax);
 }
+extern "C" int yt8m_lstm_persist_fwd_h2_img(float* z, const float* Wh, int64_t ldw, float* cs, float* hs, float* out,
+                                            const int32_t* num_frames, int64_t t0, int64_t T, int64_t B, int64_t H, float forget_bias,
+                                            const void* wh_absmax, const void* wh_image, void* workspace, int64_t workspace_bytes,
+                                            yt8m_stream_t stream) {
+  YT8M_REQUIRE(wh_absmax, YT8M_E_BADARG, "null absmax word");
+  YT8M_REQUIRE((reinterpret_cast<uintptr_t>(wh_image) & 15) == 0, YT8M_E_BADARG, "the image must be 16-byte aligned");
+  static const bool off = getenv("YT8M_PERSIST_FWD_H2") != nullptr && atoi(getenv("YT8M_PERSIST_FWD_H2")) == 0;
+  return persist_fwd_impl(z, Wh, ldw, cs, hs, out, num_frames, t0, T, B, H, forget_bias, workspace, workspace_bytes, stream, false,
+                          off ? nullptr : wh_absmax, wh_image);
+}
 extern "C" int yt8m_lstm_persist_fwd(float* z, const float* Wh, int64_t ldw, float* cs, float* hs, float* out,
                                      const int32_t* num_frames, int64_t t0, int64_t T, int64_t B, int64_t H, float forget_bias,
                                      void* workspace, int64_t workspace_bytes, yt8m_stream_t stream) {
@@ -1920,7 +2063,7 @@
 namespace {
 int persist_fwd_impl(float* z, const float* Wh, int64_t ldw, float* cs, float* hs, float* out, const int32_t* num_frames, int64_t t0,
                      int64_t T, int64_t B, int64_t H, float forget_bias, void* workspace, int64_t workspace_bytes, yt8m_stream_t stream,
-                     bool bf16, const void* h2_wword) {
+                     bool bf16, const void* h2_wword, const void* wimg) {
   using namespace yt8m;
   YT8M_REQUIRE(t0 >= 0 && T >= 0 && B >= 0 && H >= 0, YT8M_E_SHAPE, "negative dimension");
   if (T * B * H == 0) return YT8M_OK;
@@ -1955,12 +2098,18 @@
   const bool x3 = fwd_x3_shape(H, geo.pf) && images_in(workspace_bytes, geo.NT16, H + H / 2) >= T;
   int rc;
   a.wword = static_cast<const unsigned*>(h2_wword);
+  a.wimg = nullptr;
   if (x3 && !bf16 && h2_wword) {
     hipLaunchKernelGGL((hx_pack_x3_kernel<2, true>), dim3(256), dim3(256), 0, s, hs + t0 * B * H, reinterpret_cast<u32x4*>(a.hx), (int)B, (int)H,
                        geo.NT16);
     rc = launch_status("hx_pack_x3_kernel");
     if (rc != YT8M_OK) return rc;
-    if (H == 1024) hipLaunchKernelGGL((lstm_persist_fwd_x3_kernel<4, 2, true>), dim3(grid), dim3(768), 0, s, a);
+    a.wimg = wh_image_on() ? wimg : nullptr;
+    ++g_whimg_launches[0][a.wimg ? 1 : 0];
+    const int nkb = fwd_h2_nkb(H);
+    if (a.wimg && nkb == 4) hipLaunchKernelGGL((lstm_persist_fwd_x3_kernel<4, 2, true, true>), dim3(grid), dim3(768), 0, s, a);
+    else if (a.wimg) hipLaunchKernelGGL((lstm_persist_fwd_x3_kernel<2, 2, true, true>), dim3(grid), dim3(768), 0, s, a);
+    else if (nkb == 4) hipLaunchKernelGGL((lstm_persist_fwd_x3_kernel<4, 2, true>), dim3(grid), dim3(768), 0, s, a);
     else hipLaunchKernelGGL((lstm_persist_fwd_x3_kernel<2, 2, true>), dim3(grid), dim3(768), 0, s, a);
     rc = launch_status("lstm_persist_fwd_x3_kernel");
   } else if (x3 && bf16) {
@@ -2002,11 +2151,11 @@
 bool persist_geometry_bwd(int64_t B, int64_t H, GeometryB* geo) {
   static const bool off = getenv("YT8M_NO_PERSIST") != nullptr || getenv("YT8M_NO_PERSIST_BWD") != nullptr;
   if (off || B < 1 || H > 1024 || !(H == 128 || (H >= 256 && (H % 256) == 0))) return false;
-  const int NQB = (int)(H / 32);
+  const int NQB = bwd_nqb(H);
   if (!(NQB == 4 || NQB == 8 || NQB == 16 || NQB == 24 || NQB == 32)) return false;
   int dev = 0;
   const int cus = device_cus(&dev);
-  const int NUB = (int)(H / 16);
+  const int NUB = (int)(H / BWD_UNITS);
   if (cus < NUB) return false;
   const int NT16 = (int)((B + 15) / 16);
   int RB = persist_cu_budget(cus, true) / NUB;
@@ -2049,7 +2198,10 @@
     if (a.h2 && rot) {
       const bool tpf = tape_prefetch_on();
       ++g_tpf_launches[tpf ? 1 : 0];
-      if (tpf) hipLaunchKernelGGL((lstm_persist_bwd_kernel<NQB, true, true, true, false, false, true, true>), dim3(grid), dim3(768), 0, s, a);
+      ++g_whimg_launches[1][a.wimg ? 1 : 0];
+      if (a.wimg && tpf) hipLaunchKernelGGL((lstm_persist_bwd_kernel<NQB, true, true, true, false, false, true, true, true>), dim3(grid), dim3(768), 0, s, a);
+      else if (a.wimg) hipLaunchKernelGGL((lstm_persist_bwd_kernel<NQB, true, true, true, false, false, true, false, true>), dim3(grid), dim3(768), 0, s, a);
+      else if (tpf) hipLaunchKernelGGL((lstm_persist_bwd_kernel<NQB, true, true, true, false, false, true, true>), dim3(grid), dim3(768), 0, s, a);
       else hipLaunchKernelGGL((lstm_persist_bwd_kernel<NQB, true, true, true, false, false, true>), dim3(grid), dim3(768), 0, s, a);
       return yt8m::launch_status("lstm_persist_bwd_kernel");
     }
@@ -2080,7 +2232,8 @@
 int persist_bwd_impl(const float* gates, const float* Wh, int64_t ldw, const float* cs, const float* dout, float* dz,
                      float* work, int phase, float* dbias_rows, const int32_t* num_frames, int64_t t0, int64_t T,
                      int64_t B, int64_t H, void* workspace, int64_t workspace_bytes, const yt8m_persist_bwd_images* img,
-                     yt8m_stream_t stream, bool bf16 = false, const void* h2_wword = nullptr, void* rowmax = nullptr, void* partmax = nullptr);
+                     yt8m_stream_t stream, bool bf16 = false, const void* h2_wword = nullptr, void* rowmax = nullptr, void* partmax = nullptr,
+                     const void* wimg = nullptr);
 int64_t h2_scale_bytes(int NT16, int64_t H, int64_t T) { return ((T * NT16 * (H / 16) * 16 + 255) / 256) * 256; }
 }
 
@@ -2115,10 +2268,19 @@
   return persist_bwd_impl(gates, Wh, ldw, cs, dout, dz, work, phase, nullptr, num_frames, t0, T, B, H, workspace, workspace_bytes,
                           nullptr, stream, false, off ? nullptr : wh_absmax, rowmax, partmax);
 }
+extern "C" int yt8m_lstm_persist_bwd_ex_img(const float* gates, const float* Wh, int64_t ldw, const float* cs, const float* dout, float* dz,
+                                            float* work, int phase, const int32_t* num_frames, int64_t t0, int64_t T, int64_t B, int64_t H,
+                                            const void* wh_absmax, const void* wh_image, void* rowmax, void* partmax, void* workspace,
+                                            int64_t workspace_bytes, yt8m_stream_t stream) {
+  YT8M_REQUIRE((reinterpret_cast<uintptr_t>(wh_image) & 15) == 0, YT8M_E_BADARG, "the image must be 16-byte aligned");
+  static const bool off = getenv("YT8M_PERSIST_BWD_H2") != nullptr && atoi(getenv("YT8M_PERSIST_BWD_H2")) == 0;
+  return persist_bwd_impl(gates, Wh, ldw, cs, dout, dz, work, phase, nullptr, num_frames, t0, T, B, H, workspace, workspace_bytes,
+                          nullptr, stream, false, off ? nullptr : wh_absmax, rowmax, partmax, wh_image);
+}
 extern "C" int yt8m_lstm_persist_bwd_on_f16_pipe(int64_t B, int64_t H) {
   GeometryB geo;
   if (!persist_geometry(B, H, nullptr) || !persist_geometry_bwd(B, H, &geo)) return 0;
-  return ((H == 512 || H == 1024) && bwd_rot(geo.pf, geo.NT16, geo.RB)) ? 1 : 0;
+  return (h2_form_width(H) && bwd_rot(geo.pf, geo.NT16, geo.RB)) ? 1 : 0;
 }
 
 extern "C" int yt8m_lstm_persist_bwd_images(const float* gates, const float* Wh, int64_t ldw, const float* cs, const float* dout, float* dz,
@@ -2139,7 +2301,7 @@
 int persist_bwd_impl(const float* gates, const float* Wh, int64_t ldw, const float* cs, const float* dout, float* dz,
                      float* work, int phase, float* dbias_rows, const int32_t* num_frames, int64_t t0, int64_t T,
                      int64_t B, int64_t H, void* workspace, int64_t workspace_bytes, const yt8m_persist_bwd_images* img,
-                     yt8m_stream_t stream, bool bf16, const void* h2_wword, void* rowmax, void* partmax) {
+                     yt8m_stream_t stream, bool bf16, const void* h2_wword, void* rowmax, void* partmax, const void* wimg) {
   using namespace yt8m;
   YT8M_REQUIRE(t0 >= 0 && T >= 0 && B >= 0 && H >= 0, YT8M_E_SHAPE, "negative dimension");
   YT8M_REQUIRE(phase == 0 || phase == 1, YT8M_E_BADARG, "phase must be 0 or 1");
@@ -2174,14 +2336,15 @@
   a.partmax = static_cast<unsigned*>(partmax);
   YT8M_REQUIRE(!(rowmax || partmax) || (!img && images_in(workspace_bytes, geo.NT16, 4 * H) >= T && bwd_rot(geo.pf, geo.NT16, geo.RB)), YT8M_E_SHAPE,
                "row / launch maxima need the rotated backward epilogue on a per-step workspace (yt8m_lstm_persist_bwd_images_rows)");
-  a.h2 = 0; a.wword = nullptr; a.sc = nullptr; a.sc_bytes = 0;
-  if (h2_wword && !img && !bf16 && (H == 512 || H == 1024)) {
+  a.h2 = 0; a.wword = nullptr; a.sc = nullptr; a.sc_bytes = 0; a.wimg = nullptr;
+  if (h2_wword && !img && !bf16 && h2_form_width(H)) {
     const int64_t scb = h2_scale_bytes(geo.NT16, H, T);
     if (scb < (1LL << 31) && images_in(workspace_bytes - scb, geo.NT16, 4 * H) >= T) {
       a.h2 = 1;
       a.wword = static_cast<const unsigned*>(h2_wword);
       a.sc = reinterpret_cast<unsigned*>(static_cast<char*>(workspace) + workspace_bytes - DBG_BYTES - scb);
       a.sc_bytes = (unsigned)scb;
+      a.wimg = wh_image_on() ? wimg : nullptr;
     }
   }
   const unsigned grid = (unsigned)(geo.NUB * geo.RB);
diff --git a/youtube-8m_amd/csrc/lstm_stack.hip b/youtube-8m_amd/csrc/lstm_stack.hip
--- a/youtube-8m_amd/csrc/lstm_stack.hip
+++ b/youtube-8m_amd/csrc/lstm_stack.hip
@@ -1,5 +1,6 @@
 #include <stdlib.h>
 #include <algorithm>
+#include <map>
 #include <mutex>
 #include <vector>
 #include "common.h"
@@ -57,6 +58,7 @@
   int emit_max;
   int64_t rmax, rmax_stride;
   int64_t cimg[MAXL], cimgs;
+  int64_t whimg[MAXL][2], whimg_bytes[2];
   int64_t scratch_bytes;
 };
 
@@ -178,6 +180,10 @@
   const int64_t cp = p.colparts ? up256(((p.FB + 63) / 64) * H4 * 4) : 0;
   for (int l = 0; l < p.L; ++l) { p.cpart[l] = o; o += cp; }
   p.cparts = o; o += p.u8 ? cp : 0;
+  p.whimg_bytes[0] = (!p.bf16 && per_step && yt8m_lstm_persist_fwd_on_bf16_pipe(p.B, p.H)) ? yt8m_lstm_persist_wh_image_bytes(p.H, 0) : 0;
+  p.whimg_bytes[1] = (!p.bf16 && per_step && yt8m_lstm_persist_bwd_on_f16_pipe(p.B, p.H)) ? yt8m_lstm_persist_wh_image_bytes(p.H, 1) : 0;
+  for (int l = 0; l < p.L; ++l)
+    for (int dir = 0; dir < 2; ++dir) { p.whimg[l][dir] = o; o += up256(p.whimg_bytes[dir]); }
   p.scratch_bytes = o;
   return nullptr;
 }
@@ -194,6 +200,8 @@
   int layers_done = 0;
 };
 std::mutex g_mu;
+struct WhImage { hipEvent_t ready = nullptr; bool valid = false; };
+std::map<const void*, WhImage> g_whimg;
 constexpr int NSETS = 2;
 DevState g_dev[NSETS][16];
 thread_local int g_set = 0;
@@ -398,15 +406,26 @@
   };
   hipEvent_t start = ev.record(main);
   for (int l = 0; l < P.L; ++l) ev.wait(S->rs[l], start);
+  const bool wh_img = yt8m_lstm_persist_wh_image_on() != 0;
   const void* wxt_img[MAXL] = {nullptr};
+  hipEvent_t wh_ready0 = nullptr;
   for (int l = 0; l < P.L; ++l) {
     hipStream_t s = S->rs[l];
     const int64_t Din = l ? H : D;
     YT8M_HIP_CHECK(hipMemsetAsync(at<char>(tape, P.cs[l]), 0, (size_t)BH * 4, s));
     YT8M_HIP_CHECK(hipMemsetAsync(at<char>(tape, P.hs[l]), 0, (size_t)BH * 4, s));
     if (!bf) {
-      YT8M_HIP_CHECK(hipMemsetAsync(at<char>(scratch, P.hsc + 256 * l + 252), 0, 4, s));
-      RC(yt8m_h2_absmax(W[l] + Din * H4, H, H4, H4, at<char>(scratch, P.hsc + 256 * l + 252), (yt8m_stream_t)s));
+      hipStream_t sp = (l == 0 && P.L >= 2) ? S->rs[1] : s;
+      if (sp != s && P.whimg_bytes[1]) {
+        const auto it = g_whimg.find(at<char>(scratch, P.whimg[l][1]));
+        if (it != g_whimg.end()) ev.wait(sp, it->second.ready);
+      }
+      YT8M_HIP_CHECK(hipMemsetAsync(at<char>(scratch, P.hsc + 256 * l + 252), 0, 4, sp));
+      RC(yt8m_h2_absmax(W[l] + Din * H4, H, H4, H4, at<char>(scratch, P.hsc + 256 * l + 252), (yt8m_stream_t)sp));
+      if (wh_img && P.whimg_bytes[0])
+        RC(yt8m_lstm_persist_wh_image(W[l] + Din * H4, H4, H, at<char>(scratch, P.hsc + 256 * l + 252), 0, at<char>(scratch, P.whimg[l][0]),
+                                      (yt8m_stream_t)sp));
+      if (sp != s) wh_ready0 = ev.record(sp);
     }
     if (l == 0 && P.u8) {
       if (P.h2) {
@@ -508,17 +527,31 @@
         RC(grc);
       }
       static const int bf_recur_f = knob("YT8M_STACK_BF16_RECUR", 1);
+      if (l == 0 && c == 0) ev.wait(s, wh_ready0);
       static const int h2_recur_f_env = knob("YT8M_STACK_H2_RECUR_FWD", -1);
       const int h2_recur_f = h2_recur_f_env >= 0 ? h2_recur_f_env : P.h2;
       if (!bf && h2_recur_f)
-        RC(yt8m_lstm_persist_fwd_h2(at<float>(tape, P.z[l]), W[l] + Din * H4, H4, at<float>(tape, P.cs[l]), at<float>(tape, P.hs[l]),
-                                    at<float>(tape, P.out[l]), num_frames, t0, T, B, H, desc->forget_bias,
-                                    at<char>(scratch, P.hsc + 256 * l + 252), at<char>(scratch, P.pws[l]), P.pws_bytes, s));
+        RC(yt8m_lstm_persist_fwd_h2_img(at<float>(tape, P.z[l]), W[l] + Din * H4, H4, at<float>(tape, P.cs[l]), at<float>(tape, P.hs[l]),
+                                        at<float>(tape, P.out[l]), num_frames, t0, T, B, H, desc->forget_bias,
+                                        at<char>(scratch, P.hsc + 256 * l + 252),
+                                        (wh_img && P.whimg_bytes[0]) ? at<char>(scratch, P.whimg[l][0]) : nullptr,
+                                        at<char>(scratch, P.pws[l]), P.pws_bytes, s));
       else
       RC((bf && bf_recur_f ? yt8m_lstm_persist_fwd_bf16 : yt8m_lstm_persist_fwd)(
           at<float>(tape, P.z[l]), W[l] + Din * H4, H4, at<float>(tape, P.cs[l]), at<float>(tape, P.hs[l]), at<float>(tape, P.out[l]),
           num_frames, t0, T, B, H, desc->forget_bias, at<char>(scratch, P.pws[l]), P.pws_bytes, s));
       done[(size_t)l * P.nf + c] = ev.record(s);
+      if (c == P.nf - 1 && !bf && P.whimg_bytes[1]) {
+        WhImage& wi = g_whimg[at<char>(scratch, P.whimg[l][1])];
+        wi.valid = false;
+        if (wh_img) {
+          RC(yt8m_lstm_persist_wh_image(W[l] + Din * H4, H4, H, at<char>(scratch, P.hsc + 256 * l + 252), 1, at<char>(scratch, P.whimg[l][1]),
+                                        (yt8m_stream_t)s));
+          if (!wi.ready) YT8M_HIP_CHECK(hipEventCreateWithFlags(&wi.ready, hipEventDisableTiming));
+          YT8M_HIP_CHECK(hipEventRecord(wi.ready, s));
+          wi.valid = true;
+        }
+      }
     }
   }
   for (int l = 0; l < P.L; ++l) ev.wait(main, done[(size_t)l * P.nf + P.nf - 1]);
@@ -594,6 +627,7 @@
   int phase[MAXL];
   bool wx3_done[MAXL];
   const void* wx_img[MAXL] = {nullptr};
+  const void* wh_img[MAXL] = {nullptr};
   hipEvent_t dzT_free[MAXL] = {nullptr};
   const bool fused_img = P.img_rows > 0 && !dx_stream && !fuse_dz;
   int64_t img_done_rows[MAXL] = {0};
@@ -609,6 +643,13 @@
     else YT8M_HIP_CHECK(hipMemsetAsync(work + BH, 0, (size_t)BH * 4, s));
     phase[l] = 0;
     wx3_done[l] = false;
+    if (!bf && P.whimg_bytes[1] && yt8m_lstm_persist_wh_image_on()) {
+      const auto it = g_whimg.find(at<char>(scratch, P.whimg[l][1]));
+      if (it != g_whimg.end() && it->second.valid) {
+        ev.wait(s, it->second.ready);
+        wh_img[l] = at<char>(scratch, P.whimg[l][1]);
+      }
+    }
   }
   std::vector<hipEvent_t> last;
   int sub0[MAXP];
@@ -663,15 +704,16 @@
         static const int h2_recur = knob("YT8M_STACK_H2_RECUR", 1);
         static const int h2_dx_rows = knob("YT8M_STACK_H2_DX", 1);
         if (P.emit_max)
-          RC(yt8m_lstm_persist_bwd_ex(at<float>(tape, P.z[l]), W[l] + Din * H4, H4, at<float>(tape, P.cs[l]), dout, dz,
-                                      at<float>(scratch, P.work[l]), phase[l], num_frames, t0, T, B, H,
-                                      h2_recur ? at<char>(scratch, P.hsc + 256 * l + 252) : nullptr,
-                                      (l >= 1 && h2_dx_rows) ? at<char>(scratch, P.rmax + l * P.rmax_stride) : nullptr,
-                                      at<char>(scratch, P.hsc + 256 * l + 4 * (1 + c)), at<char>(scratch, P.pws[l]), P.pws_bytes, s));
+          RC(yt8m_lstm_persist_bwd_ex_img(at<float>(tape, P.z[l]), W[l] + Din * H4, H4, at<float>(tape, P.cs[l]), dout, dz,
+                                          at<float>(scratch, P.work[l]), phase[l], num_frames, t0, T, B, H,
+                                          h2_recur ? at<char>(scratch, P.hsc + 256 * l + 252) : nullptr, wh_img[l],
+                                          (l >= 1 && h2_dx_rows) ? at<char>(scratch, P.rmax + l * P.rmax_stride) : nullptr,
+                                          at<char>(scratch, P.hsc + 256 * l + 4 * (1 + c)), at<char>(scratch, P.pws[l]), P.pws_bytes, s));
         else if (!bf && h2_recur)
-          RC(yt8m_lstm_persist_bwd_h2(at<float>(tape, P.z[l]), W[l] + Din * H4, H4, at<float>(tape, P.cs[l]), dout, dz,
-                                      at<float>(scratch, P.work[l]), phase[l], nullptr, num_frames, t0, T, B, H,
-                                      at<char>(scratch, P.hsc + 256 * l + 252), at<char>(scratch, P.pws[l]), P.pws_bytes, s));
+          RC(yt8m_lstm_persist_bwd_ex_img(at<float>(tape, P.z[l]), W[l] + Din * H4, H4, at<float>(tape, P.cs[l]), dout, dz,
+                                          at<float>(scratch, P.work[l]), phase[l], num_frames, t0, T, B, H,
+                                          at<char>(scratch, P.hsc + 256 * l + 252), wh_img[l], nullptr, nullptr,
+                                          at<char>(scratch, P.pws[l]), P.pws_bytes, s));
         else
         RC((bf && bf_recur ? yt8m_lstm_persist_bwd_bf16 : yt8m_lstm_persist_bwd)(
             at<float>(tape, P.z[l]), W[l] + Din * H4, H4, at<float>(tape, P.cs[l]), dout, dz, at<float>(scratch, P.work[l]), phase[l],
```

Result: no change. 8381 videos/s, median of 6 (+0.9%).
